# neggles/neurosis

Measured on AMD Instinct MI355X. Metric: train images/sec (node) SDXL 1024^2, higher is better.
Workload: dtype bf16

## Files before the change

include/neurosis_hip.h:

```cpp
#ifndef NEUROSIS_HIP_H
#define NEUROSIS_HIP_H

#ifdef __cplusplus
extern "C" {
#endif

const char* nk_last_error(void);
int nk_abi_version(void);

int nk_linear_fwd(const void* x, const void* w, const float* bias, const void* residual, void* y,
                  int M, int N, int K, long ldx, long ldw, long ldr, long ldy, float alpha, void* stream);
int nk_linear_dgrad(const void* dy, const void* w, const void* dx_add, void* dx, int M, int N, int K,
                    long lddy, long ldw, long ldadd, long lddx, void* stream);
long nk_linear_fwd_geglu_ok(int M, int I, int K);
int nk_linear_fwd_geglu(const void* x, const void* w, const float* bias, void* u, void* h, int M, int I, int K, long ldx, long ldw, long ldu,
                        long ldh, void* stream);
int nk_linear_dgrad_geglu(const void* dy, const void* w, const void* u, void* du, int M, int N, int I, long lddy, long ldw, long ldu,
                          long lddu, void* stream);
int nk_linear_fwd_geglu_s(const void* x, const void* w, const float* bias, void* s, void* h, int M, int I, int K, long ldx, long ldw, long lds,
                          long ldh, void* stream);
int nk_linear_dgrad_geglu_s(const void* dy, const void* w, const void* s, void* du, int M, int N, int I, long lddy, long ldw, long lds,
                            long lddu, void* stream);
int nk_linear_wgrad(const void* dy, const void* x, float* dw, int M, int N, int K, long lddy, long ldx,
                    long lddw, int accumulate, void* stream);
int nk_linear_wgrad_bias(const void* dy, const void* x, float* dw, float* dbias, int M, int N, int K, long lddy, long ldx, long lddw,
                         int accumulate, void* stream);

int nk_gemm_sk_status(void);

int nk_health_status(void);
int nk_health_clear(void);
int nk_health_export(int* dst, void* stream);
int nk_health_import(const int* src, void* stream);
int nk_debug_raise_health(void* stream);
int nk_debug_stamp(unsigned long long* dst, void* stream);
int nk_debug_launch_log(int mode);
long nk_debug_launch_names(char* buf, long cap);

int nk_colsum_batched(const void* dy, float* out, float* ws, long M, int N, long ld, int nbatch, int accumulate, void* stream);

int nk_linear_fwd_batched(const void* const* x, const void* const* w, void* const* y, int count, int M, int N, int K,
                          long ldx, long ldw, long ldy, void* stream);

int nk_linear_wgrad_batched(const void* const* dy, const void* const* x, float* const* dw, float* const* dbias, int count, int M, int N,
                            int K, long lddy, long ldx, long lddw, int accumulate, void* stream);

typedef struct NkConvDesc {
  int N, H, W, Cin;
  int Cout, KH, KW;
  int stride;
  int pad_t, pad_l;
  int Ho, Wo;
  int upsample;
} NkConvDesc;
int nk_conv2d_fwd(const NkConvDesc* d, const void* x, const void* w, const float* bias, const void* rowvec,
                  const void* residual, void* y, void* stream);
long nk_conv2d_stats_tiles(const NkConvDesc* d, int stats_groups);
int nk_conv2d_fwd_stats(const NkConvDesc* d, const void* x, const void* w, const float* bias, const void* rowvec, const void* residual,
                        void* y, float* stats_part, int stats_groups, void* stream);
int nk_conv3x3_few_channels_fwd(const void* x, const void* w, const float* bias, void* y, int N, int H, int W, int Cout, int cin_real,
                                void* stream);
int nk_conv_weight_flip(const void* w, void* wt, int Cout, int Cin, int taps, void* stream);
long nk_conv2d_dgrad_flipped_ok(const NkConvDesc* d);
int nk_conv2d_dgrad_flipped(const NkConvDesc* d, const void* dy, const void* wt, void* dx, void* stream);
int nk_conv2d_dgrad(const NkConvDesc* d, const void* dy, const void* w, void* dx, void* stream);
int nk_conv2d_wgrad(const NkConvDesc* d, const void* dy, const void* x, float* dw, int accumulate, void* stream);
int nk_conv2d_wgrad_bias(const NkConvDesc* d, const void* dy, const void* x, float* dw, float* dbias, int accumulate, void* stream);

typedef struct NkAttnDesc {
  int B, H, Lq, Lk, D;
  long sq, sk, sv, so;
  long bq, bk, bv, bo;
  long sdq, sdk, sdv, sdo;
  long bdq, bdk, bdv, bdo;
  float scale;
  int causal;
} NkAttnDesc;
int nk_attention_fwd(const NkAttnDesc* d, const void* q, const void* k, const void* v, void* o, float* lse,
                     void* stream);
long nk_attention_bwd_ws_floats(const NkAttnDesc* d);
int nk_attention_bwd(const NkAttnDesc* d, const void* q, const void* k, const void* v, const void* o,
                     const float* lse, const void* d_o, void* dq, void* dk, void* dv, float* delta_ws, void* stream);
int nk_attention_bwd_causal(const NkAttnDesc* d, const void* q, const void* k, const void* v, const void* o,
                            const float* lse, const void* d_o, void* dq, void* dk, void* dv, void* stream);
int nk_softmax_rows(void* s, long M, int L, void* stream);

long nk_groupnorm_ws_floats(int N, int HW, int C, int G);
int nk_groupnorm_fwd(const void* x, const float* gamma, const float* beta, void* y, float* mean, float* rstd,
                     float* ws, int N, int HW, int C, int G, float eps, int silu, void* stream);
int nk_groupnorm_sums(const void* x, float* sums, float* ws, int N, int HW, int C, int G, void* stream);
long nk_groupnorm_sums_ws_floats(int N, int nparts, int G);
int nk_groupnorm_sums_from_parts(const float* part, float* sums, float* ws, int N, int nparts, int G, void* stream);
int nk_groupnorm_apply(const void* x, const float* sums, const float* gamma, const float* beta, void* y, float* mean, float* rstd,
                       int N, int HW, int C, int G, float eps, int silu, void* stream);
int nk_groupnorm_bwd(const void* dy, const void* x, const float* gamma, const float* beta, const float* mean,
                     const float* rstd, const void* dx_add, void* dx, float* dgamma, float* dbeta, float* ws,
                     int N, int HW, int C, int G, int silu, int accumulate, void* stream);

int nk_layernorm_fwd(const void* x, const float* gamma, const float* beta, void* y, float* mean, float* rstd,
                     int M, int C, float eps, void* stream);
long nk_layernorm_ws_floats(int M, int C);
int nk_layernorm_bwd(const void* dy, const void* x, const float* gamma, const float* mean, const float* rstd,
                     const void* dx_add, void* dx, float* dgamma, float* dbeta, float* ws, int M, int C, int accumulate, void* stream);
#define NK_COLPART_MAX 32
typedef struct NkColpartBatch {
  const float* part[NK_COLPART_MAX];
  float* dgamma[NK_COLPART_MAX];
  float* dbeta[NK_COLPART_MAX];
  int nrows[NK_COLPART_MAX];
  int C[NK_COLPART_MAX];
  int accumulate[NK_COLPART_MAX];
  int n;
} NkColpartBatch;
long nk_layernorm_part_rows(int M);
int nk_layernorm_bwd_rows(const void* dy, const void* x, const float* gamma, const float* mean, const float* rstd,
                          const void* dx_add, void* dx, float* part, int M, int C, void* stream);
int nk_colpart_reduce_batch(const NkColpartBatch* b, void* stream);
int nk_layernorm_bwd_dx(const void* dy, const void* x, const float* gamma, const float* mean, const float* rstd,
                        const void* dx_add, void* dx, int M, int C, void* stream);
int nk_layernorm_bwd_params(const void* dy, const void* x, const float* mean, const float* rstd, float* dgamma,
                            float* dbeta, float* ws, int M, int C, int accumulate, void* stream);

int nk_geglu_fwd(const void* u, void* y, long M, int I, void* stream);
int nk_geglu_bwd(const void* dy, const void* u, void* du, long M, int I, void* stream);
int nk_geglu_fwd_s(const void* u, void* y, void* s, long M, int I, void* stream);
int nk_geglu_bwd_s(const void* dy, const void* s, void* du, long M, int I, void* stream);

int nk_silu_fwd(const void* x, void* y, long n, void* stream);
int nk_silu_bwd(const void* dy, const void* x, void* dx, long n, void* stream);

int nk_add(const void* a, const void* b, void* out, long n, void* stream);

int nk_cat_channels(const void* a, const void* b, void* out, long rows, int Ca, int Cb, void* stream);
int nk_split_channels(const void* src, void* a, void* b, long rows, int Ca, int Cb, void* stream);

int nk_upsample2x_bwd(const void* dup, void* dx, int N, int H, int W, int C, void* stream);

int nk_nchw_to_nhwc(const void* src, int src_is_f32, void* dst, int N, int C, int HW, int Cpad, float scale,
                    void* stream);
int nk_nhwc_to_nchw(const void* src, void* dst, int dst_is_f32, int N, int C, int HW, int Cpad, void* stream);
int nk_cast_f32_to_bf16(const float* src, void* dst, long n, void* stream);
int nk_cast_bf16_to_f32(const void* src, float* dst, long n, void* stream);

long nk_colsum_ws_floats(long M, int N);
int nk_colsum(const void* dy, float* out, float* ws, long M, int N, long ld, int accumulate, void* stream);

int nk_softmax_rows_bwd(const void* p, void* dp, long M, int L, float scale, void* stream);

int nk_leaky_relu_fwd(const void* x, void* y, long n, float slope, void* stream);
int nk_leaky_relu_bwd(const void* dy, const void* y, void* dx, long n, float slope, void* stream);
long nk_batchnorm_ws_floats(long M, int C);
int nk_batchnorm_fwd(const void* x, const float* gamma, const float* beta, void* y, float* mean, float* rstd, float* running_mean,
                     float* running_var, float* ws, long M, int C, float eps, float momentum, float slope, void* stream);
int nk_batchnorm_bwd(const void* dy, const void* x, const void* y, const float* gamma, const float* mean, const float* rstd, void* dx,
                     float* dgamma, float* dbeta, float* ws, long M, int C, float slope, int accumulate, void* stream);
int nk_batchnorm_eval(const void* x, const float* gamma, const float* beta, const float* running_mean, const float* running_var, void* y,
                      float* ws, long M, int C, float eps, float slope, void* stream);

int nk_maxpool2x2_fwd(const void* x, void* y, int N, int H, int W, int C, void* stream);
int nk_maxpool2x2_bwd(const void* dy, const void* x, void* dx, int N, int H, int W, int C, void* stream);
int nk_maxpool_fwd(const void* x, void* y, int N, int H, int W, int C, int k, int s, void* stream);
int nk_maxpool_bwd(const void* dy, const void* x, void* dx, int N, int H, int W, int C, int k, int s, void* stream);
long nk_lpips_layer_ws_floats(int N, int HW);
int nk_lpips_layer_fwd(const void* f0, const void* f1, const float* w, float* out, float* ws, int N, int HW, int C, float eps,
                       int accumulate, void* stream);
int nk_lpips_layer_bwd(const void* f0, const void* f1, const float* w, const float* upstream, void* df1, int N, int HW, int C,
                       float eps, void* stream);

int nk_gelu_fwd(const void* x, void* y, long n, int mode, void* stream);
int nk_gelu_bwd(const void* dy, const void* x, void* dx, long n, int mode, void* stream);
#define NK_EMBEDDING_BWD_MAX_TOKENS 8192
int nk_embedding_bwd(const long long* ids, const void* dx, long ldx, float* dtable, float* dpos, int B, int L, int V, int P, int C,
                     int accumulate, void* stream);
int nk_gather_rows_bwd(const void* dsel, long ldsel, const long long* idx, void* dx, int B, int L, int C, void* stream);
int nk_wgrad_few_rows(const void* x, long ldx, const void* dy, long lddy, float* dw, long lddw, int M, int K, int N, int accumulate, void* stream);

int nk_timestep_embedding(const float* t, void* out, int B, int dim, float max_period, void* stream);

int nk_edm_prepare(const float* x, const float* eps, const float* sigma, const float* c_in, float* zt, void* net_in,
                   int B, int C, int HW, int Cpad, void* stream);
int nk_edm_loss(const void* net_out, const float* zt, const float* target, const float* c_out, const float* c_skip,
                const float* w, float* loss, void* dnet, int B, int C, int HW, int Cpad, float upstream, void* stream);

int nk_sample_prepare(const float* x, const float* c_in, void* net_in, int B, int C, int HW, int Cpad, int rep, void* stream);
int nk_sample_denoise(const void* net_out, const float* x, const float* c_skip, const float* c_out, float scale,
                      float* denoised, int B, int C, int HW, int Cpad, int rep, void* stream);
int nk_sample_euler_step(const void* net_out, const float* x, const float* c_skip, const float* c_out, const float* sigma_hat,
// ... 56 lines not shown
```

neurosis_amd/csrc/conv_wgrad_halo.h:

```cpp
#pragma once

#define WH_TH 4
#define WH_TW 32
#define WH_HS 48
#define WH_X_BYTES ((WH_TH + 2) * WH_HS * 128)
#define WH_DY_BYTES (WH_TH * WH_TW * 256)
#define WH_STAGE (WH_X_BYTES + WH_DY_BYTES)
#define WH_SMEM (2 * WH_STAGE)
#define WH_BCO 128
#define WH_BCI 64

typedef __attribute__((address_space(3))) char* wh_lds;
typedef __attribute__((address_space(3))) short4_t* wh_lds4;

__device__ __forceinline__ int wh_swz_x(int slot) { return (((slot >> 1) & 1) << 2) | ((slot >> 2) & 3); }
__device__ __forceinline__ int wh_swz_dy(int px) { return ((px & 3) << 2) | ((px >> 2) & 3); }

__device__ __forceinline__ bf16x8_t wh_read(wh_lds lo, wh_lds hi) {
  const short4_t a = __builtin_amdgcn_ds_read_tr16_b64_v4i16((wh_lds4)lo);
  const short4_t b = __builtin_amdgcn_ds_read_tr16_b64_v4i16((wh_lds4)hi);
  short8_t r;
  r[0] = a[0]; r[1] = a[1]; r[2] = a[2]; r[3] = a[3];
  r[4] = b[0]; r[5] = b[1]; r[6] = b[2]; r[7] = b[3];
  return __builtin_bit_cast(bf16x8_t, r);
// ... 99 lines not shown
      if constexpr (BIAS) {
        const short8_t raw = __builtin_bit_cast(short8_t, af);
#pragma unroll
        for (int e = 0; e < 8; ++e) bsum += bf2f((bf16_t)raw[e]);
      }
#pragma unroll
      for (int kh = 0; kh < 3; ++kh)
#pragma unroll
        for (int kw = 0; kw < 3; ++kw) {
          const int off = ((r + kh) * WH_HS + c) * 128;
          const bf16x8_t xf = wh_read(base + xo[kw][0] + off, base + xo[kw][1] + off);
          acc[kh * 3 + kw] = __builtin_amdgcn_mfma_f32_32x32x16_bf16(af, xf, acc[kh * 3 + kw], 0, 0, 0);
        }
    }
  }

  float* dw = (float*)p.C;
  const int ci = ib * WH_BCI + is * 32 + (lane & 31);
  const int co_base = cb * WH_BCO + cs * 32 + 4 * h;
  const bool atomic = gridDim.x > (unsigned)nblk || p.accumulate == 1;
#pragma unroll
  for (int t = 0; t < 9; ++t)
#pragma unroll
    for (int r = 0; r < 16; ++r) {
      const int co = co_base + (r & 3) + 8 * (r >> 2);
      if (co < Cout) {
        float* dst = dw + (long)co * p.ldc + t * Cin + ci;
        const float v = acc[t][r] * p.alpha;
        if (atomic) unsafeAtomicAdd(dst, v);
        else *dst = v;
      }
    }
  if constexpr (BIAS) {
    if (ib == 0 && is == 0) {
      bsum += __shfl_xor(bsum, 32);
      const int co = cb * WH_BCO + cs * 32 + (lane & 31);
      if (lane < 32 && co < Cout) {
        if (atomic) unsafeAtomicAdd(p.dbias + co, bsum * p.alpha);
        else p.dbias[co] = bsum * p.alpha;
      }
    }
  }
}

static bool wgrad_halo_shape_ok(const NkGemmParams& p) {
  const NkGather& g = p.gb;
  if (!p.halo_nb || g.KW != 3 || p.N != 9 * g.C || g.rs != 1 || g.ks != 1 || g.div != 1 || g.off_h != -1 || g.off_w != -1) return false;
  if (g.Ho != g.H || g.Wo != g.W || (g.C % WH_BCI) || (p.M & 7) || p.nbatch || p.ldc != p.N || p.lda != p.M) return false;
  if (p.K != (long)p.halo_nb * g.H * g.W) return false;
  const long cover = (long)((g.W + WH_TW - 1) / WH_TW) * WH_TW * ((g.H + WH_TH - 1) / WH_TH) * WH_TH;
  return cover * 100 <= (long)g.H * g.W * 125;
}
static int wgrad_halo_splits(const NkGemmParams& p, int& per) {
  const NkGather& g = p.gb;
  const long T = (long)p.halo_nb * ((g.W + WH_TW - 1) / WH_TW) * ((g.H + WH_TH - 1) / WH_TH);
  const long nblk = (long)((p.M + WH_BCO - 1) / WH_BCO) * (g.C / WH_BCI);
  const double dw_bytes = (double)p.M * p.N * 4.0;
  double best = 1e30;
  int best_s = 1;
  for (int s = 1; s <= 64 && s <= T; ++s) {
    const long tiles = (T + s - 1) / s;
    const long rounds = (nblk * s + 255) / 256;
    const double cost = (double)rounds * (tiles * 3.0e-6 + 4.0e-6) + (s > 1 ? s * dw_bytes / 1.3e12 : dw_bytes / 4.0e12);
    if (cost < best * 0.97) { best = cost; best_s = s; }
  }
  per = (int)((T + best_s - 1) / best_s);
  return (int)((T + per - 1) / per);
}
static bool use_wgrad_halo(const NkGemmParams& p, int amode, int bmode, int out_f32) {
  if (amode != OP_MC || bmode != OP_MCG || !out_f32) return false;
  int mode = 1;
  if (const char* e = getenv("NK_CONV_WGRAD_HALO")) mode = atoi(e);
  if (!mode || !wgrad_halo_shape_ok(p)) return false;
  if (mode == 2) return true;
  if (p.M < 64) return false;
  const long nblk = (long)((p.M + WH_BCO - 1) / WH_BCO) * (p.gb.C / WH_BCI);
  return p.K >= 16384 || nblk >= 180;
}
static int launch_wgrad_halo(NkGemmParams& p, hipStream_t stream) {
  int per = 0;
  const int S = wgrad_halo_splits(p, per);
  const long nblk = (long)((p.M + WH_BCO - 1) / WH_BCO) * (p.gb.C / WH_BCI);
  if (S > 1 && p.accumulate == 0) {
    const size_t n = (size_t)p.M * p.N;
    const unsigned blocks = (unsigned)((n / 4 + 255) / 256 > 2048 ? 2048 : (n / 4 + 255) / 256);
    hipLaunchKernelGGL(nk_zero_f32_kernel, dim3(blocks ? blocks : 1), dim3(256), 0, stream, (float*)p.C, n);
    if (p.dbias) hipLaunchKernelGGL(nk_zero_f32_kernel, dim3(1), dim3(256), 0, stream, p.dbias, (size_t)p.M);
    if (hipGetLastError() != hipSuccess) return NK_ERR_LAUNCH;
  }
  p.accumulate = p.accumulate == 1 ? 1 : 0;
  p.ksplit_len = per;
  auto kern = p.dbias ? nk_conv3x3_wgrad_halo_kernel<1> : nk_conv3x3_wgrad_halo_kernel<0>;
  nk_optin_lds((const void*)kern, WH_SMEM);
  hipLaunchKernelGGL(kern, dim3((unsigned)(nblk * S)), dim3(512), WH_SMEM, stream, p);
  return nk_check_launch(p.dbias ? "nk_conv3x3_wgrad_halo_kernel<bias=1>" : "nk_conv3x3_wgrad_halo_kernel<bias=0>");
}
```

neurosis_amd/csrc/elementwise.hip:

```cpp
#include "../../include/neurosis_hip.h"
#include "nk_common.h"

#define EW_THREADS 256
static inline int ew_blocks(long work_items) {
  long b = (work_items + EW_THREADS - 1) / EW_THREADS;
  if (b > 8192) b = 8192;
  if (b < 1) b = 1;
  return (int)b;
}

__global__ void geglu_fwd_kernel(const bf16_t* __restrict__ u, bf16_t* __restrict__ y, long M, int I) {
  const int cpr = I >> 3;
  const long total = M * cpr;
  for (long i = blockIdx.x * (long)blockDim.x + threadIdx.x; i < total; i += (long)gridDim.x * blockDim.x) {
    long row = i / cpr;
    int ch = (int)(i - row * cpr);
    float a[8], g[8];
    unpack8(*(const uint4_t*)(u + row * 2 * I + ch * 8), a);
    unpack8(*(const uint4_t*)(u + row * 2 * I + I + ch * 8), g);
#pragma unroll
    for (int e = 0; e < 8; ++e) a[e] *= gelu_erf(g[e]);
    *(uint4_t*)(y + row * I + ch * 8) = pack8(a);
  }
}
// ... 335 lines not shown
  }
}
extern "C" int nk_upsample2x_bwd(const void* dup, void* dx, int N, int H, int W, int C, void* stream) {
  NK_CHECK_ARG(dup && dx && N > 0 && H > 0 && W > 0 && C > 0 && (C & 7) == 0);
  hipLaunchKernelGGL(up2_bwd_kernel, dim3(ew_blocks((long)N * H * W * (C >> 3))), dim3(EW_THREADS), 0,
                     (hipStream_t)stream, (const bf16_t*)dup, (bf16_t*)dx, N, H, W, C);
  return nk_check_launch("upsample2x_bwd");
}

template <typename SrcT>
__global__ void nchw_to_nhwc_kernel(const SrcT* __restrict__ src, bf16_t* __restrict__ dst, int C, int HW, int Cpad,
                                    float scale) {
  __shared__ float tile[32][33];
  const int n = blockIdx.z;
  const int p0 = blockIdx.x * 32, c0 = blockIdx.y * 32;
  const int tx = threadIdx.x & 31, ty = threadIdx.x >> 5;
  for (int j = ty; j < 32; j += 8) {
    int c = c0 + j, p = p0 + tx;
    float v = 0.f;
    if (c < C && p < HW) {
      if constexpr (sizeof(SrcT) == 4) v = src[((long)n * C + c) * HW + p];
      else v = bf2f(src[((long)n * C + c) * HW + p]);
    }
    tile[j][tx] = v * scale;
  }
  __syncthreads();
  for (int j = ty; j < 32; j += 8) {
    int p = p0 + j, c = c0 + tx;
    if (p < HW && c < Cpad) dst[((long)n * HW + p) * Cpad + c] = f2bf(tile[tx][j]);
  }
}
template <typename DstT>
__global__ void nhwc_to_nchw_kernel(const bf16_t* __restrict__ src, DstT* __restrict__ dst, int C, int HW, int Cpad) {
  __shared__ float tile[32][33];
  const int n = blockIdx.z;
  const int p0 = blockIdx.x * 32, c0 = blockIdx.y * 32;
  const int tx = threadIdx.x & 31, ty = threadIdx.x >> 5;
  for (int j = ty; j < 32; j += 8) {
    int p = p0 + j, c = c0 + tx;
    tile[j][tx] = (p < HW && c < C) ? bf2f(src[((long)n * HW + p) * Cpad + c]) : 0.f;
  }
  __syncthreads();
  for (int j = ty; j < 32; j += 8) {
    int c = c0 + j, p = p0 + tx;
    if (c < C && p < HW) {
      float v = tile[tx][j];
      if constexpr (sizeof(DstT) == 4) dst[((long)n * C + c) * HW + p] = v;
      else dst[((long)n * C + c) * HW + p] = f2bf(v);
    }
  }
}
__global__ __launch_bounds__(256) void conv_weight_flip_kernel(const bf16_t* __restrict__ w, bf16_t* __restrict__ wt, int Cout, int Cin, int taps) {
  __shared__ bf16_t tile[64][64 + 8];
  const int tap = blockIdx.z, co0 = blockIdx.y * 64, ci0 = blockIdx.x * 64;
  const int tid = threadIdx.x;
#pragma unroll
  for (int it = 0; it < 2; ++it) {
    const int idx = tid + 256 * it;
    const int r = idx >> 3, ch = idx & 7;
    uint4_t v = {0u, 0u, 0u, 0u};
    if (co0 + r < Cout && ci0 + ch * 8 < Cin) v = *(const uint4_t*)(w + ((long)(co0 + r) * taps + tap) * Cin + ci0 + ch * 8);
    const bf16_t* e = (const bf16_t*)&v;
#pragma unroll
    for (int k = 0; k < 8; ++k) tile[ch * 8 + k][r] = e[k];
  }
  __syncthreads();
  const int tflip = taps - 1 - tap;
#pragma unroll
  for (int it = 0; it < 2; ++it) {
    const int idx = tid + 256 * it;
    const int r = idx >> 3, ch = idx & 7;
    if (ci0 + r < Cin && co0 + ch * 8 < Cout)
      *(uint4_t*)(wt + ((long)(ci0 + r) * taps + tflip) * Cout + co0 + ch * 8) = *(const uint4_t*)&tile[r][ch * 8];
  }
}
extern "C" int nk_conv_weight_flip(const void* w, void* wt, int Cout, int Cin, int taps, void* stream) {
  NK_CHECK_ARG(w && wt && Cout > 0 && Cin > 0 && taps > 0 && taps <= 65535);
  NK_CHECK_ARG((Cout & 7) == 0 && (Cin & 7) == 0);
  hipLaunchKernelGGL(conv_weight_flip_kernel, dim3((Cin + 63) / 64, (Cout + 63) / 64, taps), dim3(256), 0, (hipStream_t)stream, (const bf16_t*)w, (bf16_t*)wt,
                     Cout, Cin, taps);
  return nk_check_launch("conv_weight_flip_kernel");
}

__global__ __launch_bounds__(256) void conv3x3_few_channels_kernel(const bf16_t* __restrict__ x, const bf16_t* __restrict__ w, const float* __restrict__ bias,
                                                                   bf16_t* __restrict__ y, int N, int H, int W, int Cout, int groups_per_wave) {
  const int lane = threadIdx.x & 63, wave = threadIdx.x >> 6;
  const int r = lane & 15, g = lane >> 4;
  const int co_base = blockIdx.y * 128;
  bf16x8_t wf[8][2];
#pragma unroll
  for (int b = 0; b < 8; ++b) {
    const int co = co_base + b * 16 + r;
    uint2_t t0 = {0u, 0u}, t1 = {0u, 0u}, t8 = {0u, 0u};
    if (co < Cout) {
      t0 = *(const uint2_t*)(w + ((long)co * 9 + 2 * g) * 8);
      t1 = *(const uint2_t*)(w + ((long)co * 9 + 2 * g + 1) * 8);
      if (g == 0) t8 = *(const uint2_t*)(w + ((long)co * 9 + 8) * 8);
    }
    wf[b][0] = __builtin_bit_cast(bf16x8_t, (uint4_t){t0.x, t0.y, t1.x, t1.y});
    wf[b][1] = __builtin_bit_cast(bf16x8_t, (uint4_t){t8.x, t8.y, 0u, 0u});
  }
  const int nloc = (g & 1) * 16 + (g >> 1) * 8;
  float bv[4][8];
#pragma unroll
  for (int h = 0; h < 4; ++h)
#pragma unroll
    for (int e = 0; e < 8; ++e) {
      const int co = co_base + h * 32 + nloc + e;
      bv[h][e] = (bias && co < Cout) ? bias[co] : 0.f;
    }
  const long total = (long)N * H * W;
  const long gw = (long)blockIdx.x * 4 + wave;
  const int HW = H * W;
  const int ta = 2 * g, tb = 2 * g + 1;
  const int dya = ta / 3 - 1, dxa = ta % 3 - 1, dyb = tb / 3 - 1, dxb = tb % 3 - 1;

  auto fetch = [&](long grp, uint2_t& a, uint2_t& b, uint2_t& c) {
    a = (uint2_t){0u, 0u}; b = a; c = a;
    const long pix = grp * 16 + r;
    if (pix >= total) return;
    const int n = (int)(pix / HW);
    const int rem = (int)(pix - (long)n * HW);
    const int py = rem / W, px = rem - py * W;
    const bf16_t* img = x + (long)n * HW * 8;
    int yy = py + dya, xx = px + dxa;
    if ((unsigned)yy < (unsigned)H && (unsigned)xx < (unsigned)W) a = *(const uint2_t*)(img + ((long)yy * W + xx) * 8);
    yy = py + dyb; xx = px + dxb;
    if ((unsigned)yy < (unsigned)H && (unsigned)xx < (unsigned)W) b = *(const uint2_t*)(img + ((long)yy * W + xx) * 8);
    if (g == 0) {
      yy = py + 1; xx = px + 1;
      if (yy < H && xx < W) c = *(const uint2_t*)(img + ((long)yy * W + xx) * 8);
    }
  };

  const long gstride = (long)gridDim.x * 4;
  uint2_t na, nb, nc;
  long grp = gw;
  fetch(grp, na, nb, nc);
  for (int it = 0; it < groups_per_wave; ++it, grp += gstride) {
    if (grp * 16 >= total) break;
    const bf16x8_t x0 = __builtin_bit_cast(bf16x8_t, (uint4_t){na.x, na.y, nb.x, nb.y});
    const bf16x8_t x1 = __builtin_bit_cast(bf16x8_t, (uint4_t){nc.x, nc.y, 0u, 0u});
    if (it + 1 < groups_per_wave) fetch(grp + gstride, na, nb, nc);
    float4_t acc[8];
#pragma unroll
    for (int b = 0; b < 8; ++b) {
      acc[b] = __builtin_amdgcn_mfma_f32_16x16x32_bf16(wf[b][0], x0, (float4_t){0.f, 0.f, 0.f, 0.f}, 0, 0, 0);
      acc[b] = __builtin_amdgcn_mfma_f32_16x16x32_bf16(wf[b][1], x1, acc[b], 0, 0, 0);
    }
    const long pix = grp * 16 + r;
#pragma unroll
    for (int h = 0; h < 4; ++h) {
      float v[8];
#pragma unroll
      for (int e = 0; e < 4; ++e) {
        const float a_own = acc[2 * h][e], b_own = acc[2 * h + 1][e];
        auto sw = __builtin_amdgcn_permlane16_swap(__float_as_uint(a_own), __float_as_uint(b_own), false, false);
        v[e] = __uint_as_float(sw[0]) + bv[h][e];
        v[4 + e] = __uint_as_float(sw[1]) + bv[h][4 + e];
      }
      const int co = co_base + h * 32 + nloc;
      if (pix < total && co < Cout) *(uint4_t*)(y + pix * Cout + co) = pack8(v);
    }
  }
}
extern "C" int nk_conv3x3_few_channels_fwd(const void* x, const void* w, const float* bias, void* y, int N, int H, int W, int Cout, int cin_real,
                                           void* stream) {
  NK_CHECK_ARG(x && w && y && N > 0 && H > 0 && W > 0 && Cout > 0 && (Cout & 7) == 0);
  NK_CHECK_ARG(cin_real == 3 || cin_real == 4);
  NK_CHECK_ARG((long)N * H * W < (1l << 31));
  const long groups = ((long)N * H * W + 15) / 16;
  long blocks = (groups + 4 * 32 - 1) / (4 * 32);
  if (blocks > 2048) blocks = 2048;
  const int per_wave = (int)((groups + blocks * 4 - 1) / (blocks * 4));
  dim3 grid((unsigned)blocks, (unsigned)((Cout + 127) / 128));
  hipLaunchKernelGGL(conv3x3_few_channels_kernel, grid, dim3(256), 0, (hipStream_t)stream, (const bf16_t*)x, (const bf16_t*)w, bias, (bf16_t*)y, N, H, W, Cout,
                     per_wave);
  return nk_check_launch("conv3x3_few_channels_kernel");
}

extern "C" int nk_nchw_to_nhwc(const void* src, int src_is_f32, void* dst, int N, int C, int HW, int Cpad, float scale,
                               void* stream) {
  NK_CHECK_ARG(src && dst && N > 0 && C > 0 && HW > 0 && Cpad >= C);
  dim3 grid((HW + 31) / 32, (Cpad + 31) / 32, N);
  if (src_is_f32)
    hipLaunchKernelGGL(nchw_to_nhwc_kernel<float>, grid, dim3(256), 0, (hipStream_t)stream, (const float*)src,
                       (bf16_t*)dst, C, HW, Cpad, scale);
  else
    hipLaunchKernelGGL(nchw_to_nhwc_kernel<bf16_t>, grid, dim3(256), 0, (hipStream_t)stream, (const bf16_t*)src,
                       (bf16_t*)dst, C, HW, Cpad, scale);
  return nk_check_launch("nchw_to_nhwc");
}
extern "C" int nk_nhwc_to_nchw(const void* src, void* dst, int dst_is_f32, int N, int C, int HW, int Cpad,
                               void* stream) {
  NK_CHECK_ARG(src && dst && N > 0 && C > 0 && HW > 0 && Cpad >= C);
  dim3 grid((HW + 31) / 32, (C + 31) / 32, N);
  if (dst_is_f32)
    hipLaunchKernelGGL(nhwc_to_nchw_kernel<float>, grid, dim3(256), 0, (hipStream_t)stream, (const bf16_t*)src,
                       (float*)dst, C, HW, Cpad);
  else
    hipLaunchKernelGGL(nhwc_to_nchw_kernel<bf16_t>, grid, dim3(256), 0, (hipStream_t)stream, (const bf16_t*)src,
                       (bf16_t*)dst, C, HW, Cpad);
  return nk_check_launch("nhwc_to_nchw");
}

__global__ void cast_f32_bf16_kernel(const float* __restrict__ s, bf16_t* __restrict__ d, long n) {
  const long n8 = n >> 3;
  for (long i = blockIdx.x * (long)blockDim.x + threadIdx.x; i < n8; i += (long)gridDim.x * blockDim.x) {
    const float4_t a = *(const float4_t*)(s + i * 8), b = *(const float4_t*)(s + i * 8 + 4);
    float f[8] = {a[0], a[1], a[2], a[3], b[0], b[1], b[2], b[3]};
    *(uint4_t*)(d + i * 8) = pack8(f);
  }
  if (blockIdx.x == 0) for (long i = n8 * 8 + threadIdx.x; i < n; i += blockDim.x) d[i] = f2bf(s[i]);
}
__global__ void cast_bf16_f32_kernel(const bf16_t* __restrict__ s, float* __restrict__ d, long n) {
  for (long i = blockIdx.x * (long)blockDim.x + threadIdx.x; i < n; i += (long)gridDim.x * blockDim.x) d[i] = bf2f(s[i]);
}
extern "C" int nk_cast_f32_to_bf16(const float* src, void* dst, long n, void* stream) {
  NK_CHECK_ARG(src && dst && n > 0 && ((uintptr_t)src & 15) == 0 && ((uintptr_t)dst & 15) == 0);
  hipLaunchKernelGGL(cast_f32_bf16_kernel, dim3(ew_blocks((n >> 3) + 1)), dim3(EW_THREADS), 0, (hipStream_t)stream, src,
                     (bf16_t*)dst, n);
  return nk_check_launch("cast_f32_to_bf16");
}
extern "C" int nk_cast_bf16_to_f32(const void* src, float* dst, long n, void* stream) {
  NK_CHECK_ARG(src && dst && n > 0);
  hipLaunchKernelGGL(cast_bf16_f32_kernel, dim3(ew_blocks(n)), dim3(EW_THREADS), 0, (hipStream_t)stream,
                     (const bf16_t*)src, dst, n);
  return nk_check_launch("cast_bf16_to_f32");
}

#define CS_ROWS 64
static int colsum_rows(long M) {
  long rows = CS_ROWS;
  while ((M + rows - 1) / rows > 1024) rows *= 2;
  return (int)rows;
}
__global__ __launch_bounds__(256) void colsum_partial_kernel(const bf16_t* __restrict__ dy, float* __restrict__ part, long M, int N,
                                                             long ld, int rows_per_block) {
  __shared__ float ps[16][16 * 8 + 4];
  const int tid = threadIdx.x;
  const int cx = tid & 15, ry = tid >> 4;
  const int chunk = blockIdx.y * 16 + cx;
  const bool cok = chunk < (N >> 3);
  dy += (long)blockIdx.z * M * ld;
  part += (long)blockIdx.z * gridDim.x * N;
  const long row_lo = (long)blockIdx.x * rows_per_block;
  const long row_hi = row_lo + rows_per_block < M ? row_lo + rows_per_block : M;
  float s[8];
#pragma unroll
  for (int e = 0; e < 8; ++e) s[e] = 0.f;
  if (cok) {
    for (long base = row_lo + ry; base < row_hi; base += 64) {
      uint4_t v[4];
#pragma unroll
      for (int i = 0; i < 4; ++i) {
        const long r = base + 16 * i;
        v[i] = r < row_hi ? *(const uint4_t*)(dy + r * ld + chunk * 8) : (uint4_t){0u, 0u, 0u, 0u};
      }
#pragma unroll
      for (int i = 0; i < 4; ++i) {
        float f[8];
// ... 325 lines not shown
```

neurosis_amd/csrc/gemm.hip:

```cpp
#include "nk_common.h"
#include "nk_gemm.h"
#include <stdlib.h>

#define BM 128
#define BN 128
#define BK 64
#define NTHREADS 256
#define GROUP_M 8
#define KC_IMAGE_BYTES (128 * 128)
#define MC_ROW_BYTES (128 * 2 + 16)
#define MC_IMAGE_BYTES (BK * MC_ROW_BYTES)
#define OPND_BYTES MC_IMAGE_BYTES
#define STAGE_BYTES (2 * OPND_BYTES)
#define CS_LD 132
#define SMEM_BYTES (2 * STAGE_BYTES)

static_assert(SMEM_BYTES >= BM * CS_LD * 4, "epilogue staging must fit");

enum { OP_KC = 0, OP_KCG = 1, OP_MC = 2, OP_MCT = 3, OP_MCG = 4 };

__device__ __forceinline__ bool is_kc(int mode) { return mode == OP_KC || mode == OP_KCG; }

__device__ __forceinline__ long gather_offset(const NkGather& g, int n, int bh, int bw, int kh, int kw,
                                              int c, bool& valid) {
// ... 1315 lines not shown
    X2_RDA(1);
    X2_BAR();
    X2_MM(4, 2, bc1, X2_NEXT(b0, sb0, p.gb, nb0, kb0); X2_NEXT(b1, sb1, p.gb, nb1, kb1));
    X2_BAR();
    b0.fire(0, sb0[0], cur + 32768);
    b0.fire(1, sb0[1], cur + 32768);
    b1.fire(0, sb1[0], cur + 49152);
    b1.fire(1, sb1[1], cur + 49152);
    asm volatile("s_waitcnt vmcnt(4)" ::: "memory");
    X2_BAR();
    X2_MM(4, 0, bc0, X2_NEXT(a1, sa1, p.ga, na1, ka1));
    X2_BAR();
  }
  if (wm == 0) { X2_BAR(); }
  asm volatile("s_waitcnt vmcnt(0)" ::: "memory");
#undef X2_NEXT
#undef X2_ISSUE
#undef X2_RD1
#undef X2_RDA
#undef X2_RDB
#undef X2_BAR
#undef X2_MM
  if constexpr (GEGLU) {
    const int I = p.N >> 1;
    const int abase = (n0 >> 1) + wn * 32;
    const int cl = (lane >> 4) * 4;
    float4_t ba[2], bg[2];
#pragma unroll
    for (int q = 0; q < 2; ++q) {
      ba[q] = p.bias ? *(const float4_t*)(p.bias + abase + q * 16 + cl) : (float4_t){0.f, 0.f, 0.f, 0.f};
      bg[q] = p.bias ? *(const float4_t*)(p.bias + I + abase + q * 16 + cl) : (float4_t){0.f, 0.f, 0.f, 0.f};
    }
    NkGemmParams ph = p;
    ph.N = I; ph.ldc = p.ld_h; ph.bias = nullptr;
    NkGemmParams ps = p;
    ps.bias = nullptr;
#pragma unroll
    for (int ib = 0; ib < 2; ++ib) {
      float4_t pa[4][2], pg[4][2], phh[4][2];
#pragma unroll
      for (int i = 0; i < 4; ++i)
#pragma unroll
        for (int q = 0; q < 2; ++q) {
          pa[i][q] = acc[ib * 4 + i][2 * q];
          pg[i][q] = acc[ib * 4 + i][2 * q + 1];
#pragma unroll
          for (int r = 0; r < 4; ++r) {
            const float av = bf2f(f2bf(pa[i][q][r] + ba[q][r])), gv = bf2f(f2bf(pg[i][q][r] + bg[q][r]));
            float cdf, pdf;
            normal_cdf_pdf(gv, cdf, pdf);
            const float ge = gv * cdf;
            phh[i][q][r] = av * ge;
            if (p.geglu_save) {
              pa[i][q][r] = ge;
              pg[i][q][r] = av * (cdf + gv * pdf);
            }
          }
        }
      const int mb = m0 + wm * 128 + ib * 64;
      if (p.geglu_save) {
        reg_epilogue_64x32<0>(ps, p.C, pa, mb, abase, lane);
        reg_epilogue_64x32<0>(ps, p.C, pg, mb, I + abase, lane);
      } else {
        reg_epilogue_64x32<0>(p, p.C, pa, mb, abase, lane);
        reg_epilogue_64x32<0>(p, p.C, pg, mb, I + abase, lane);
      }
      reg_epilogue_64x32<0>(ph, p.geglu_h, phh, mb, abase, lane);
    }
    return;
  }
#pragma unroll
  for (int ib = 0; ib < 2; ++ib)
#pragma unroll
    for (int half = 0; half < 2; ++half) {
      float4_t pair[4][2];
#pragma unroll
      for (int i = 0; i < 4; ++i) { pair[i][0] = acc[ib * 4 + i][2 * half]; pair[i][1] = acc[ib * 4 + i][2 * half + 1]; }
      reg_epilogue_64x32<0>(p, p.C, pair, m0 + wm * 128 + ib * 64, n0 + wn * 64 + half * 32, lane);
    }
}

static bool use_xl(const NkGemmParams& p, int amode, int bmode, int out_f32, int splitk);
__global__ void nk_zero_f32_kernel(float* __restrict__ dst, size_t n);
#include "gemm_g2.h"
#include "gemm_w160.h"
#include "conv_halo.h"
#include "conv_wgrad_halo.h"

static bool use_xl(const NkGemmParams& p, int amode, int bmode, int out_f32, int splitk) {
  static int on = -1;
  if (on < 0) { const char* e = getenv("NK_GEMM_XL"); on = (e && e[0] == '0') ? 0 : 1; }
  if (!on || p.nbatch || out_f32 || splitk != 1 || bmode != OP_KC || !(amode == OP_KC || amode == OP_KCG)) return false;
  const long ntn = (p.N + XL_BN - 1) / XL_BN;
  const long tiles = (long)((p.M + XL_BM - 1) / XL_BM) * ntn;
  const long rounds = (tiles + 255) / 256;
  return tiles >= 224 && tiles * 10 >= rounds * 256 * 8 && ntn * XL_BN * 100 <= (long)p.N * 112 && p.K >= 4 * BK;
}
template <int AMODE, int WM, int WN>
static int launch_xl_as(const NkGemmParams& p, hipStream_t stream) {
  auto kern = nk_gemm_xl_kernel<AMODE, WM, WN>;
  nk_optin_lds((const void*)kern, XL_SMEM_BYTES);
  dim3 grid(((p.M + XL_BM - 1) / XL_BM) * ((p.N + XL_BN - 1) / XL_BN), 1, 1);
  hipLaunchKernelGGL(kern, grid, dim3((XL_BM / WM) * (XL_BN / WN) * 64), XL_SMEM_BYTES, stream, p);
  return nk_check_launch("nk_gemm_xl_kernel");
}
template <int AMODE>
static int launch_xl(const NkGemmParams& p_in, hipStream_t stream) {
  if (AMODE == OP_KC) {
    auto kern = nk_gemm_xl2g_kernel<OP_KC, 0>;
    auto kerng = nk_gemm_xl2g_kernel<OP_KC, 1>;
    nk_optin_lds((const void*)kern, XL_SMEM_BYTES);
    nk_optin_lds((const void*)kerng, XL_SMEM_BYTES);
    NkGemmParams p = p_in;
    p.k_rotate = k_rotate_on(p.K) ? 1 : 0;
    dim3 grid(((p.M + XL_BM - 1) / XL_BM) * ((p.N + XL_BN - 1) / XL_BN), 1, 1);
    if (p.geglu_h) hipLaunchKernelGGL(kerng, grid, dim3(512), XL_SMEM_BYTES, stream, p);
    else hipLaunchKernelGGL(kern, grid, dim3(512), XL_SMEM_BYTES, stream, p);
    return nk_check_launch(p.geglu_h ? "nk_gemm_xl2g_kernel<geglu=1>" : "nk_gemm_xl2g_kernel<geglu=0>");
  }
  return launch_xl_as<AMODE, 64, 64>(p_in, stream);
}

template <int AMODE, int BMODE, int OUT_F32>
static int launch(const NkGemmParams& p_in, int splitk, hipStream_t stream) {
  NkGemmParams p2 = p_in;
  const NkGemmParams& p = p2;
  auto kern8 = nk_gemm_dma_kernel<AMODE, BMODE, OUT_F32, 8>;
  auto kernr = nk_gemm_ring_kernel<AMODE, BMODE, OUT_F32>;
  nk_optin_lds((const void*)kern8, V2_SMEM_BYTES);
  nk_optin_lds((const void*)kernr, RING_SMEM_BYTES);
  int ntm = (p.M + BM - 1) / BM, ntn = (p.N + BN - 1) / BN;
  dim3 grid(ntm * ntn, splitk, p.nbatch ? p.nbatch : 1);
  {
    int per_xcd = (ntm * ntn + 7) / 8, g = 1;
    while ((g + 1) * (g + 1) <= per_xcd) ++g;
    p2.group_m = g > GROUP_M ? GROUP_M : g;
  }
  p2.k_rotate = k_rotate_on(splitk > 1 ? p.ksplit_len : p.K) ? 1 : 0;
  if (!p.nbatch && (long)ntm * ntn * splitk <= 256) {
    hipLaunchKernelGGL(kernr, grid, dim3(512), RING_SMEM_BYTES, stream, p);
    return nk_check_launch("nk_gemm_ring_kernel");
  }
  hipLaunchKernelGGL(kern8, grid, dim3(512), V2_SMEM_BYTES, stream, p);
  return nk_check_launch("nk_gemm_dma_kernel");
}


#include <mutex>
#include <unordered_map>
struct SkWorkspace {
  unsigned* counter = nullptr;
  unsigned* flags = nullptr;
  float* ws = nullptr;
};
static std::mutex sk_mutex;
static std::unordered_map<void*, SkWorkspace> sk_spaces;

static bool use_sk(const NkGemmParams& p, int out_f32) {
  int mode = 4;
  if (const char* e = getenv("NK_GEMM_SK")) mode = atoi(e);
  if (mode == 0) return false;
  if (mode == 1) return true;
  if (mode == 2) return out_f32 != 0;
  if (mode == 4 && out_f32) return false;
  const long tiles = (long)((p.M + BM - 1) / BM) * ((p.N + BN - 1) / BN) * (p.nbatch ? p.nbatch : 1);
  const long nk = (p.K + BK - 1) / BK;
// ... 13 lines not shown
      nk_set_error(__FILE__, __LINE__, "stream-K workspace requested while the stream is capturing: run the launch once on this stream before capturing it");
      return NK_ERR_LAUNCH;
    }
    char* raw = nullptr;
    const size_t ws_bytes = (size_t)SK_MAX_GRID * SK_TILE_FLOATS * sizeof(float);
    if (hipMalloc((void**)&raw, ws_bytes + (SK_MAX_GRID + 64) * sizeof(unsigned)) != hipSuccess) {
      nk_set_error(__FILE__, __LINE__, "hipMalloc of the stream-K workspace failed");
      return NK_ERR_LAUNCH;
    }
    w.ws = (float*)raw;
    w.flags = (unsigned*)(raw + ws_bytes);
    w.counter = w.flags + SK_MAX_GRID;
    if (hipMemsetAsync(w.flags, 0, (SK_MAX_GRID + 64) * sizeof(unsigned), stream) != hipSuccess) return NK_ERR_LAUNCH;
  }
  p.sk_health = nk_health_word();
  if (!p.sk_health) { nk_set_error(__FILE__, __LINE__, "health word allocation failed"); return NK_ERR_LAUNCH; }
  p.sk_counter = w.counter;
  p.sk_flags = w.flags;
  p.sk_ws = w.ws;
  p.sk_base = 0;
  p.sk_epoch = 0;
  return NK_OK;
}

int nk_gemm_sk_reset(void) {
  std::lock_guard<std::mutex> lock(sk_mutex);
  for (auto& kv : sk_spaces)
    if (kv.second.flags && hipMemset(kv.second.flags, 0, (SK_MAX_GRID + 64) * sizeof(unsigned)) != hipSuccess) return NK_ERR_LAUNCH;
  return NK_OK;
}

extern "C" int nk_gemm_sk_status(void) {
  std::lock_guard<std::mutex> lock(sk_mutex);
  if (hipDeviceSynchronize() != hipSuccess) return -1;
  int bad = 0;
  for (auto& kv : sk_spaces) {
    unsigned v = 0;
    if (kv.second.flags && hipMemcpy(&v, kv.second.flags + SK_MAX_GRID + 1, sizeof(v), hipMemcpyDeviceToHost) == hipSuccess && v) bad = 1;
  }
  return bad;
}

template <int AMODE, int BMODE, int OUT_F32>
static int launch_sk(NkGemmParams& p, hipStream_t stream) {
  auto kern = nk_gemm_sk_kernel<AMODE, BMODE, OUT_F32>;
  nk_optin_lds((const void*)kern, SK_SMEM_BYTES);
  const long ntm = (p.M + BM - 1) / BM, ntn = (p.N + BN - 1) / BN, nk = (p.K + BK - 1) / BK;
  const long T = ntm * ntn * (p.nbatch ? p.nbatch : 1), W = T * nk;
  const int max_grid = SK_MAX_GRID & ~7, min_iters = 4;
  long grid = (W / min_iters) & ~7l;
  if (grid > max_grid) grid = max_grid;
  if (grid < 8) grid = 8;
  p.sk_chunked = T >= 64;
  { const char* d = getenv("NK_SK_DEBUG"); p.sk_debug = d ? atoi(d) & 2 : 0; }
  if (int e = sk_prepare(p, (int)grid, stream)) return e;
  hipLaunchKernelGGL(kern, dim3((unsigned)grid), dim3(SK_NT), SK_SMEM_BYTES, stream, p);
  return nk_check_launch("nk_gemm_sk_kernel");
}

__global__ __launch_bounds__(256) void nk_zero_f32_kernel(float* __restrict__ dst, size_t n) {
  const size_t n4 = n / 4, stride = (size_t)gridDim.x * 256;
  float4_t* d4 = (float4_t*)dst;
  for (size_t i = (size_t)blockIdx.x * 256 + threadIdx.x; i < n4; i += stride) d4[i] = (float4_t){0.f, 0.f, 0.f, 0.f};
  if (blockIdx.x == 0 && threadIdx.x < (n & 3)) dst[n4 * 4 + threadIdx.x] = 0.f;
}

static int pick_splitk(int M, int N, int K, int max_split) {
  int tiles = ((M + BM - 1) / BM) * ((N + BN - 1) / BN);
  int nk = (K + BK - 1) / BK;
  const int lo = 96, hi = 192;
  if (tiles >= lo && tiles * 2 <= 512 && nk >= 256 && max_split >= 2) return 2;
  if (tiles >= lo) return 1;
  int s = 1;
  while (s < max_split && tiles * s < hi && nk / (s * 2) >= 8) s *= 2;
  return s;
}

static void set_split(NkGemmParams& p, int splitk) {
  int nk = (p.K + BK - 1) / BK;
  int per = (nk + splitk - 1) / splitk;
  p.ksplit_len = per * BK;
}

static int zero_split_outputs(const NkGemmParams& p, hipStream_t stream) {
  for (int z = 0; z < (p.nbatch ? p.nbatch : 1); ++z) {
    const size_t n = (size_t)p.M * p.N;
    float* dst = (float*)(p.nbatch ? p.Cb[z] : p.C);
    const unsigned blocks = (unsigned)((n / 4 + 255) / 256 > 2048 ? 2048 : (n / 4 + 255) / 256);
    hipLaunchKernelGGL(nk_zero_f32_kernel, dim3(blocks ? blocks : 1), dim3(256), 0, stream, dst, n);
    float* db = p.nbatch ? p.dbias_b[z] : p.dbias;
    if (db) hipLaunchKernelGGL(nk_zero_f32_kernel, dim3(1), dim3(256), 0, stream, db, (size_t)p.M);
  }
  return hipGetLastError() != hipSuccess ? NK_ERR_LAUNCH : NK_OK;
}

int nk_gemm_dispatch(NkGemmParams& p, int amode, int bmode, int out_f32, int allow_splitk,
                     hipStream_t stream) {
  NK_CHECK_ARG(p.M > 0 && p.N > 0 && p.K > 0);
  if (!p.nbatch) NK_CHECK_ARG(((uintptr_t)p.A & 15) == 0 && ((uintptr_t)p.B & 15) == 0 && ((uintptr_t)p.C & 15) == 0);
  for (int z = 0; z < p.nbatch; ++z) NK_CHECK_ARG(((uintptr_t)p.Ab[z] & 15) == 0 && ((uintptr_t)p.Bb[z] & 15) == 0 && ((uintptr_t)p.Cb[z] & 15) == 0);
  if (amode == OP_KC) NK_CHECK_ARG((p.K & 7) == 0 && (p.lda & 7) == 0);
  if (bmode == OP_KC) NK_CHECK_ARG((p.K & 7) == 0 && (p.ldb & 7) == 0);
  if (amode == OP_KCG) NK_CHECK_ARG((p.ga.C & 7) == 0);
  if (amode == OP_MC) NK_CHECK_ARG((p.M & 7) == 0 && (p.lda & 7) == 0);
  if (bmode == OP_MC) NK_CHECK_ARG((p.N & 7) == 0 && (p.ldb & 7) == 0);
  if (bmode == OP_MCT) NK_CHECK_ARG((p.N & 7) == 0 && (p.tw.co_stride & 7) == 0 && (p.tw.tap_stride & 7) == 0);
  if (bmode == OP_MCG) NK_CHECK_ARG((p.gb.C & 7) == 0);
  if (p.residual) NK_CHECK_ARG(((uintptr_t)p.residual & 15) == 0 && ((p.ldr & 7) == 0 || (p.N & 7) != 0));
  if (!out_f32) NK_CHECK_ARG((p.ldc & 7) == 0 || (p.N & 7) != 0);
  if (p.fRowsPerBatch.d == 0) p.fRowsPerBatch = make_fastdiv(1);

  if (p.dbias || (p.nbatch && p.dbias_b[0])) NK_CHECK_ARG(amode == OP_MC && out_f32);
  if (p.geglu_h) {
    NK_CHECK_ARG(amode == OP_KC && bmode == OP_KC && !out_f32 && !p.nbatch && (p.N & 255) == 0 && (p.ld_h & 7) == 0 && !p.rowvec && !p.residual && p.alpha == 1.0f);
    NK_CHECK_ARG(((uintptr_t)p.geglu_h & 15) == 0 && (!p.bias || ((uintptr_t)p.bias & 15) == 0));
    if (!use_xl(p, amode, bmode, out_f32, 1)) {
      nk_set_error(__FILE__, __LINE__, "fused GEGLU forward on a shape the 256 x 256 kernel does not take (ask nk_linear_fwd_geglu_ok first)");
      return NK_ERR_ARG;
    }
    set_split(p, 1);
    return launch_xl<OP_KC>(p, stream);
  }
  if (p.geglu_u) {
    NK_CHECK_ARG(amode == OP_KC && bmode == OP_MC && !out_f32 && !p.nbatch && (p.N & 7) == 0 && (p.ld_u & 7) == 0 && !p.bias && !p.rowvec && !p.residual);
    set_split(p, 1);
    return launch<OP_KC, OP_MC, 0>(p, 1, stream);
  }
  if (use_halo(p, amode, bmode, out_f32)) return launch_halo(p, stream);
  if (use_wgrad_halo(p, amode, bmode, out_f32)) return launch_wgrad_halo(p, stream);
  if (p.stats_part) {
    nk_set_error(__FILE__, __LINE__, "statistics epilogue on a convolution the halo-tile kernel does not take (ask nk_conv2d_stats_tiles first)");
    return NK_ERR_ARG;
  }

  {
    const W160Plan wp = w160_plan(p, amode, bmode, out_f32, allow_splitk);
    if (wp.bn) {
      set_split(p, wp.splitk);
      if (wp.splitk > 1 && p.accumulate == 0) {
        NK_CHECK_ARG(p.ldc == p.N);
        if (int rc = zero_split_outputs(p, stream)) return rc;
        p.accumulate = 1;
      } else if (p.accumulate == 2) {
        p.accumulate = wp.splitk > 1 ? 1 : 0;
      }
      p.k_rotate = k_rotate_on(wp.splitk > 1 ? p.ksplit_len : p.K) ? 1 : 0;
      return wp.bn == 160 ? launch_w160_as<160>(p, wp.splitk, stream) : launch_w160_as<128>(p, wp.splitk, stream);
    }
  }
  if (use_ring64(p, amode, bmode, out_f32)) return launch_ring64(p, stream);
  if ((!p.nbatch || p.nbatch <= NK_MAX_BATCH) && use_g2(p, amode, bmode, out_f32, 1) && (g2_mode() == 2 || !use_xl(p, amode, bmode, out_f32, 1))) {
    if (p.accumulate == 2) p.accumulate = 0;
    if (amode == OP_KC && bmode == OP_KC) return out_f32 ? launch_g2<OP_KC, OP_KC, 1>(p, stream) : launch_g2<OP_KC, OP_KC, 0>(p, stream);
    if (amode == OP_KC && bmode == OP_MC) return out_f32 ? launch_g2<OP_KC, OP_MC, 1>(p, stream) : launch_g2<OP_KC, OP_MC, 0>(p, stream);
    if (amode == OP_KCG && bmode == OP_KC) return out_f32 ? launch_g2<OP_KCG, OP_KC, 1>(p, stream) : launch_g2<OP_KCG, OP_KC, 0>(p, stream);
    if (amode == OP_KCG && bmode == OP_MCT) return out_f32 ? launch_g2<OP_KCG, OP_MCT, 1>(p, stream) : launch_g2<OP_KCG, OP_MCT, 0>(p, stream);
    return out_f32 ? launch_g2<OP_MC, OP_MC, 1>(p, stream) : launch_g2<OP_MC, OP_MC, 0>(p, stream);
  }

  bool has_dbias = p.dbias != nullptr;
  for (int z = 0; z < p.nbatch && z < NK_MAX_BATCH; ++z) has_dbias = has_dbias || p.dbias_b[z] != nullptr;
  if (!has_dbias && use_sk(p, out_f32)) {
    const long ntm_ = (p.M + BM - 1) / BM, ntn_ = (p.N + BN - 1) / BN, nk_ = (p.K + BK - 1) / BK;
    if (ntm_ * ntn_ * (p.nbatch ? p.nbatch : 1) * nk_ < (1l << 22)) {
      if (p.accumulate == 2) p.accumulate = 0;
#define NK_SK_CASE(A_, B_)                                                        \
      if (amode == A_ && bmode == B_) return out_f32 ? launch_sk<A_, B_, 1>(p, stream) : launch_sk<A_, B_, 0>(p, stream);
      NK_SK_CASE(OP_KC, OP_KC)
      NK_SK_CASE(OP_KC, OP_MC)
      NK_SK_CASE(OP_MC, OP_MC)
      NK_SK_CASE(OP_KCG, OP_KC)
// ... 46 lines not shown
```

neurosis_amd/csrc/nk_common.h:

```cpp
#pragma once
#include <hip/hip_runtime.h>
#include <stdint.h>

typedef unsigned short bf16_t;
typedef __attribute__((ext_vector_type(8))) short short8_t;
typedef __attribute__((ext_vector_type(4))) short short4_t;
typedef __attribute__((ext_vector_type(8))) __bf16 bf16x8_t;
typedef __attribute__((ext_vector_type(4))) float float4_t;
typedef __attribute__((ext_vector_type(16))) float float16_t;
typedef __attribute__((ext_vector_type(4))) unsigned int uint4_t;
typedef __attribute__((ext_vector_type(2))) unsigned int uint2_t;

#define NK_OK 0
#define NK_ERR_ARG 1
#define NK_ERR_LAUNCH 2
#define NK_ERR_HEALTH 3

#define NK_CHECK_ARG(cond)                                                        \
  do {                                                                            \
    if (!(cond)) {                                                                \
      nk_set_error(__FILE__, __LINE__, #cond);                                    \
      return NK_ERR_ARG;                                                          \
    }                                                                             \
  } while (0)

void nk_set_error(const char* file, int line, const char* what);
int nk_check_launch(const char* what);
void nk_optin_lds(const void* kernel, int bytes);
unsigned* nk_health_word(void);
int nk_health_poll(void);
void nk_health_snapshot(hipStream_t stream);

__device__ __forceinline__ float bf2f(bf16_t v) { return __uint_as_float(((unsigned)v) << 16); }
__device__ __forceinline__ bf16_t f2bf(float f) {
  __bf16 b = (__bf16)f;
  return __builtin_bit_cast(unsigned short, b);
}
typedef __attribute__((ext_vector_type(2))) float float2_t;
typedef __attribute__((ext_vector_type(2))) __bf16 bf16x2_t;
__device__ __forceinline__ unsigned pack2bf(float lo, float hi) {
  float2_t v = {lo, hi};
  return __builtin_bit_cast(unsigned, __builtin_convertvector(v, bf16x2_t));
}
__device__ __forceinline__ void unpack8(const uint4_t& v, float* f) {
  f[0] = __uint_as_float(v.x << 16); f[1] = __uint_as_float(v.x & 0xffff0000u);
  f[2] = __uint_as_float(v.y << 16); f[3] = __uint_as_float(v.y & 0xffff0000u);
  f[4] = __uint_as_float(v.z << 16); f[5] = __uint_as_float(v.z & 0xffff0000u);
  f[6] = __uint_as_float(v.w << 16); f[7] = __uint_as_float(v.w & 0xffff0000u);
}
__device__ __forceinline__ uint4_t pack8(const float* f) {
  uint4_t v;
  v.x = pack2bf(f[0], f[1]); v.y = pack2bf(f[2], f[3]);
  v.z = pack2bf(f[4], f[5]); v.w = pack2bf(f[6], f[7]);
  return v;
}
__device__ __forceinline__ void unpack4(const uint2_t& v, float* f) {
  f[0] = __uint_as_float(v.x << 16); f[1] = __uint_as_float(v.x & 0xffff0000u);
  f[2] = __uint_as_float(v.y << 16); f[3] = __uint_as_float(v.y & 0xffff0000u);
}

__device__ __forceinline__ float wave_sum(float v) {
#pragma unroll
  for (int o = 32; o > 0; o >>= 1) v += __shfl_xor(v, o, 64);
  return v;
}
__device__ __forceinline__ float wave_max(float v) {
#pragma unroll
  for (int o = 32; o > 0; o >>= 1) v = fmaxf(v, __shfl_xor(v, o, 64));
  return v;
}

struct FastDiv {
  unsigned d, m, s;
};
static inline FastDiv make_fastdiv(unsigned d) {
  FastDiv f;
  f.d = d;
  if (d <= 1) { f.m = 0; f.s = 0; return f; }
  unsigned l = 0;
  while ((1ull << l) < d) ++l;
  f.m = (unsigned)(((1ull << 32) * ((1ull << l) - d)) / d + 1);
  f.s = l;
  return f;
}
__device__ __forceinline__ unsigned fdiv(unsigned n, const FastDiv& f) {
  return (__umulhi(n, f.m) + n) >> f.s;
}

__device__ __forceinline__ float silu_f(float x) { return x / (1.0f + __expf(-x)); }
__device__ __forceinline__ float dsilu_f(float x) {
  float s = 1.0f / (1.0f + __expf(-x));
  return s * (1.0f + x * (1.0f - s));
}

__device__ __forceinline__ void normal_cdf_pdf(float x, float& cdf, float& pdf) {
  const float e = __expf(-0.5f * x * x);
  const float t = __builtin_amdgcn_rcpf(1.0f + 0.3275911f * 0.70710678118654752f * fabsf(x));
  const float poly = t * (0.254829592f + t * (-0.284496736f + t * (1.421413741f + t * (-1.453152027f + t * 1.061405429f))));
  cdf = 0.5f * (1.0f + copysignf(1.0f - poly * e, x));
  pdf = 0.3989422804014327f * e;
}
__device__ __forceinline__ float gelu_erf(float x) {
  float cdf, pdf;
  normal_cdf_pdf(x, cdf, pdf);
  return x * cdf;
}
__device__ __forceinline__ float dgelu_erf(float x) {
  float cdf, pdf;
  normal_cdf_pdf(x, cdf, pdf);
  return cdf + x * pdf;
}
// ... 1 lines not shown
```

neurosis_amd/csrc/norm.hip:

```cpp
#include "../../include/neurosis_hip.h"
#include "nk_common.h"

#define GN_THREADS 256
#define GN_MAXC 4096

__global__ __launch_bounds__(GN_THREADS) void gn_stats_kernel(const bf16_t* __restrict__ x, float* __restrict__ stats,
                                                              int HW, int C, int G, int rows_per) {
  __shared__ float ps[GN_THREADS * 8], pss[GN_THREADS * 8];
  const int n = blockIdx.y;
  const int cpr = (C >> 3) / gridDim.z;
  const int ch0 = blockIdx.z * cpr;
  const int rows_par = GN_THREADS / cpr;
  const int tid = threadIdx.x;
  const int cpg = C / G;
  const int row_lo = blockIdx.x * rows_per;
  const int row_hi = min(HW, row_lo + rows_per);
  float s[8], ss[8];
#pragma unroll
  for (int e = 0; e < 8; ++e) { s[e] = 0.f; ss[e] = 0.f; }
  const int chunk = tid % cpr, rsub = tid / cpr;
  if (rsub < rows_par) {
    const bf16_t* base = x + ((long)n * HW) * C + (ch0 + chunk) * 8;
    int r = row_lo + rsub;
    for (; r + 3 * rows_par < row_hi; r += 4 * rows_par) {
      uint4_t v[4];
#pragma unroll
      for (int u = 0; u < 4; ++u) v[u] = *(const uint4_t*)(base + (long)(r + u * rows_par) * C);
#pragma unroll
      for (int u = 0; u < 4; ++u) {
        float f[8];
        unpack8(v[u], f);
#pragma unroll
        for (int e = 0; e < 8; ++e) { s[e] += f[e]; ss[e] += f[e] * f[e]; }
      }
    }
    for (; r < row_hi; r += rows_par) {
      float f[8];
      unpack8(*(const uint4_t*)(base + (long)r * C), f);
#pragma unroll
      for (int e = 0; e < 8; ++e) { s[e] += f[e]; ss[e] += f[e] * f[e]; }
    }
#pragma unroll
    for (int e = 0; e < 8; ++e) {
      ps[(rsub * cpr + chunk) * 8 + e] = s[e];
      pss[(rsub * cpr + chunk) * 8 + e] = ss[e];
    }
  }
  __syncthreads();
  float* part = stats + (((long)n * gridDim.x + blockIdx.x) * gridDim.z + blockIdx.z) * 2 * G;
  for (int i = tid; i < 2 * G; i += GN_THREADS) {
    const int g = i >> 1;
    const float* src = (i & 1) ? pss : ps;
    const int c_lo = max(g * cpg, ch0 * 8), c_hi = min((g + 1) * cpg, (ch0 + cpr) * 8);
    float a = 0.f;
    for (int c = c_lo; c < c_hi; ++c)
      for (int r = 0; r < rows_par; ++r) a += src[r * cpr * 8 + (c - ch0 * 8)];
    part[i] = a;
  }
}

__global__ __launch_bounds__(1024) void gn_reduce_partials_kernel(const float* __restrict__ part, float* __restrict__ out,
                                                                 int nparts, int G2) {
  __shared__ float sm[8][128];
  const int n = blockIdx.x;
  const int tx = threadIdx.x & 127, ty = threadIdx.x >> 7;
  float a = 0.f;
  if (tx < G2)
    for (int p = ty; p < nparts; p += 8) a += part[((long)n * nparts + p) * G2 + tx];
  sm[ty][tx] = a;
  __syncthreads();
  if (ty == 0 && tx < G2) {
#pragma unroll
    for (int j = 1; j < 8; ++j) a += sm[j][tx];
    out[(long)n * G2 + tx] = a;
  }
}

__global__ __launch_bounds__(GN_THREADS) void gn_apply_kernel(const bf16_t* __restrict__ x, const float* __restrict__ stats,
                                                              const float* __restrict__ gamma, const float* __restrict__ beta,
                                                              bf16_t* __restrict__ y, float* __restrict__ mean_out,
                                                              float* __restrict__ rstd_out, int HW, int C, int G,
                                                              float eps, int silu, int rows_per) {
  extern __shared__ __attribute__((aligned(16))) char smem_raw[];
  float* sc = (float*)smem_raw;
  float* sh = sc + C;
  const int n = blockIdx.y;
  const int tid = threadIdx.x;
  const int cpg = C / G;
  const float inv_cnt = 1.0f / ((float)HW * (float)cpg);
  for (int c = tid; c < C; c += GN_THREADS) {
    int g = c / cpg;
    float m = stats[(long)n * 2 * G + 2 * g] * inv_cnt;
    float var = fmaxf(stats[(long)n * 2 * G + 2 * g + 1] * inv_cnt - m * m, 0.f);
    float rs = rsqrtf(var + eps);
    float a = rs * gamma[c];
    sc[c] = a;
    sh[c] = beta[c] - m * a;
    if (blockIdx.x == 0 && (c % cpg) == 0) { mean_out[n * G + g] = m; rstd_out[n * G + g] = rs; }
  }
  __syncthreads();
  const int cpr = C >> 3;
  const int row_lo = blockIdx.x * rows_per;
  const int row_hi = min(HW, row_lo + rows_per);
  const unsigned total = (unsigned)(row_hi - row_lo) * (unsigned)cpr;
  const bf16_t* xb = x + ((long)n * HW + row_lo) * C;
  bf16_t* yb = y + ((long)n * HW + row_lo) * C;
  auto one = [&](unsigned i, const uint4_t& raw) {
    const unsigned chunk = i % (unsigned)cpr;
    float f[8];
    unpack8(raw, f);
    const float4_t a0 = *(const float4_t*)(sc + chunk * 8), a1 = *(const float4_t*)(sc + chunk * 8 + 4);
    const float4_t b0 = *(const float4_t*)(sh + chunk * 8), b1 = *(const float4_t*)(sh + chunk * 8 + 4);
    f[0] = f[0] * a0[0] + b0[0]; f[1] = f[1] * a0[1] + b0[1]; f[2] = f[2] * a0[2] + b0[2]; f[3] = f[3] * a0[3] + b0[3];
    f[4] = f[4] * a1[0] + b1[0]; f[5] = f[5] * a1[1] + b1[1]; f[6] = f[6] * a1[2] + b1[2]; f[7] = f[7] * a1[3] + b1[3];
    if (silu) {
#pragma unroll
      for (int e = 0; e < 8; ++e) f[e] = silu_f(f[e]);
    }
    *(uint4_t*)(yb + (size_t)i * 8) = pack8(f);
  };
  unsigned i = tid;
  for (; i + 3 * GN_THREADS < total; i += 4 * GN_THREADS) {
    uint4_t v[4];
#pragma unroll
    for (int u = 0; u < 4; ++u) v[u] = *(const uint4_t*)(xb + (size_t)(i + u * GN_THREADS) * 8);
#pragma unroll
    for (int u = 0; u < 4; ++u) one(i + u * GN_THREADS, v[u]);
  }
  for (; i < total; i += GN_THREADS) one(i, *(const uint4_t*)(xb + (size_t)i * 8));
}

__global__ __launch_bounds__(GN_THREADS, 4) void gn_bwd_stats_kernel(const bf16_t* __restrict__ dy, const bf16_t* __restrict__ x,
                                                                  const float* __restrict__ gamma, const float* __restrict__ beta,
                                                                  const float* __restrict__ mean, const float* __restrict__ rstd,
                                                                  float* __restrict__ gsum, float* __restrict__ chan_part,
                                                                  int HW, int C, int G, int silu, int rows_per) {
  __shared__ float pa[GN_THREADS * 8], pb[GN_THREADS * 8];
  extern __shared__ __attribute__((aligned(16))) char smem_raw[];
  float* ca = (float*)smem_raw;
  float* cb = ca + C;
  const int n = blockIdx.y;
  const int tid = threadIdx.x;
  const int cpg = C / G;
  const int cpr = (C >> 3) / gridDim.z;
  const int ch0 = blockIdx.z * cpr;
  const int rows_par = GN_THREADS / cpr;
  const int row_lo = blockIdx.x * rows_per;
  const int row_hi = min(HW, row_lo + rows_per);
  const int chunk = tid % cpr, rsub = tid / cpr;
  if (rsub < rows_par) {
    float a[8], b[8], mu[8], rs[8], ga[8], be[8];
#pragma unroll
    for (int e = 0; e < 8; ++e) {
      int c = (ch0 + chunk) * 8 + e;
      int g = c / cpg;
      a[e] = 0.f; b[e] = 0.f;
      mu[e] = mean[n * G + g]; rs[e] = rstd[n * G + g];
      ga[e] = gamma[c]; be[e] = beta[c];
    }
    const long base = ((long)n * HW) * C + (ch0 + chunk) * 8;
    auto one = [&](const uint4_t& rx, const uint4_t& rd) {
      float fx[8], fd[8];
      unpack8(rx, fx);
      unpack8(rd, fd);
#pragma unroll
      for (int e = 0; e < 8; ++e) {
        float xh = (fx[e] - mu[e]) * rs[e];
        float dz = fd[e];
        if (silu) dz *= dsilu_f(xh * ga[e] + be[e]);
        a[e] += dz;
        b[e] += dz * xh;
      }
    };
    int r = row_lo + rsub;
    for (; r + 3 * rows_par < row_hi; r += 4 * rows_par) {
      uint4_t vx[4], vd[4];
#pragma unroll
      for (int u = 0; u < 4; ++u) {
        vx[u] = *(const uint4_t*)(x + base + (long)(r + u * rows_par) * C);
        vd[u] = *(const uint4_t*)(dy + base + (long)(r + u * rows_par) * C);
      }
#pragma unroll
      for (int u = 0; u < 4; ++u) one(vx[u], vd[u]);
    }
    for (; r < row_hi; r += rows_par) one(*(const uint4_t*)(x + base + (long)r * C), *(const uint4_t*)(dy + base + (long)r * C));
#pragma unroll
    for (int e = 0; e < 8; ++e) {
      pa[(rsub * cpr + chunk) * 8 + e] = a[e];
      pb[(rsub * cpr + chunk) * 8 + e] = b[e];
    }
  }
  __syncthreads();
  float* cp = chan_part + ((long)n * gridDim.x + blockIdx.x) * 2 * C;
  for (int cl = tid; cl < cpr * 8; cl += GN_THREADS) {
    float av = 0.f, bv = 0.f;
    for (int r = 0; r < rows_par; ++r) { av += pa[r * cpr * 8 + cl]; bv += pb[r * cpr * 8 + cl]; }
    const int c = ch0 * 8 + cl;
    ca[cl] = av;
    cb[cl] = bv;
    cp[c] = bv;
    cp[C + c] = av;
  }
  __syncthreads();
  float* part = gsum + (((long)n * gridDim.x + blockIdx.x) * gridDim.z + blockIdx.z) * 2 * G;
  for (int i = tid; i < 2 * G; i += GN_THREADS) {
    const int g = i >> 1;
    const float* src = (i & 1) ? cb : ca;
    const int c_lo = max(g * cpg, ch0 * 8), c_hi = min((g + 1) * cpg, (ch0 + cpr) * 8);
    float acc = 0.f;
    for (int c = c_lo; c < c_hi; ++c) acc += gamma[c] * src[c - ch0 * 8];
    part[i] = acc;
  }
}

__global__ __launch_bounds__(1024) void colpart_reduce_kernel(const float* __restrict__ part, float* __restrict__ dgamma,
                                                              float* __restrict__ dbeta, int nrows, int C, int accumulate) {
  __shared__ float sa[16][64], sb[16][64];
  const int tx = threadIdx.x & 63, ty = threadIdx.x >> 6;
  const int c = blockIdx.x * 64 + tx;
  float a = 0.f, b = 0.f;
  if (c < C) {
#pragma unroll 4
    for (int r = ty; r < nrows; r += 16) {
      a += part[(long)r * 2 * C + c];
      b += part[(long)r * 2 * C + C + c];
    }
  }
  sa[ty][tx] = a;
  sb[ty][tx] = b;
  __syncthreads();
  if (ty == 0 && c < C) {
#pragma unroll
    for (int j = 1; j < 16; ++j) { a += sa[j][tx]; b += sb[j][tx]; }
    dgamma[c] = accumulate ? dgamma[c] + a : a;
    dbeta[c] = accumulate ? dbeta[c] + b : b;
  }
}

__global__ __launch_bounds__(GN_THREADS) void gn_bwd_apply_kernel(const bf16_t* __restrict__ dy, const bf16_t* __restrict__ x,
                                                                  const float* __restrict__ gamma, const float* __restrict__ beta,
                                                                  const float* __restrict__ mean, const float* __restrict__ rstd,
                                                                  const float* __restrict__ gsum, const bf16_t* __restrict__ dx_add,
                                                                  bf16_t* __restrict__ dx, int HW, int C, int G, int silu,
                                                                  int rows_per) {
  extern __shared__ __attribute__((aligned(16))) char smem_raw[];
  float* p_a = (float*)smem_raw;
  float* p_b = p_a + C;
  float* p_c = p_b + C;
  float* p_d = p_c + C;
  const int n = blockIdx.y;
  const int tid = threadIdx.x;
  const int cpg = C / G;
  const float inv_cnt = 1.0f / ((float)HW * (float)cpg);
  for (int c = tid; c < C; c += GN_THREADS) {
    const int g = c / cpg;
    const float mu = mean[n * G + g], rs = rstd[n * G + g];
    const float s1 = gsum[(long)n * 2 * G + 2 * g] * inv_cnt, s2 = gsum[(long)n * 2 * G + 2 * g + 1] * inv_cnt;
    const float a = rs * gamma[c];
    p_a[c] = a;
    p_b[c] = beta[c] - mu * a;
    p_c[c] = -rs * rs * s2;
    p_d[c] = -rs * s1 + mu * rs * rs * s2;
  }
  __syncthreads();
  const int cpr = C >> 3;
  const int row_lo = blockIdx.x * rows_per;
  const int row_hi = min(HW, row_lo + rows_per);
  const unsigned total = (unsigned)(row_hi - row_lo) * (unsigned)cpr;
  const long off0 = ((long)n * HW + row_lo) * C;
  auto one = [&](unsigned i, const uint4_t& rx, const uint4_t& rd, const uint4_t& ra) {
    const int c0 = (int)(i % (unsigned)cpr) * 8;
    float fx[8], fd[8], fa[8], ca[8], cb[8], cc[8], cd[8];
    unpack8(rx, fx);
    unpack8(rd, fd);
    unpack8(ra, fa);
    *(float4_t*)ca = *(const float4_t*)(p_a + c0); *(float4_t*)(ca + 4) = *(const float4_t*)(p_a + c0 + 4);
    *(float4_t*)cc = *(const float4_t*)(p_c + c0); *(float4_t*)(cc + 4) = *(const float4_t*)(p_c + c0 + 4);
    *(float4_t*)cd = *(const float4_t*)(p_d + c0); *(float4_t*)(cd + 4) = *(const float4_t*)(p_d + c0 + 4);
    if (silu) {
      *(float4_t*)cb = *(const float4_t*)(p_b + c0); *(float4_t*)(cb + 4) = *(const float4_t*)(p_b + c0 + 4);
#pragma unroll
      for (int e = 0; e < 8; ++e) fd[e] *= dsilu_f(fx[e] * ca[e] + cb[e]);
    }
#pragma unroll
    for (int e = 0; e < 8; ++e) fx[e] = ca[e] * fd[e] + (fx[e] * cc[e] + cd[e]) + fa[e];
    *(uint4_t*)(dx + off0 + (size_t)i * 8) = pack8(fx);
  };
  const uint4_t zero4 = {0u, 0u, 0u, 0u};
  unsigned i = tid;
  for (; i + GN_THREADS < total; i += 2 * GN_THREADS) {
    uint4_t vx[2], vd[2], va[2];
#pragma unroll
    for (int u = 0; u < 2; ++u) {
      const size_t o = off0 + (size_t)(i + u * GN_THREADS) * 8;
      vx[u] = *(const uint4_t*)(x + o);
      vd[u] = *(const uint4_t*)(dy + o);
      va[u] = dx_add ? *(const uint4_t*)(dx_add + o) : zero4;
    }
#pragma unroll
    for (int u = 0; u < 2; ++u) one(i + u * GN_THREADS, vx[u], vd[u], va[u]);
  }
  for (; i < total; i += GN_THREADS) {
    const size_t o = off0 + (size_t)i * 8;
    one(i, *(const uint4_t*)(x + o), *(const uint4_t*)(dy + o), dx_add ? *(const uint4_t*)(dx_add + o) : zero4);
  }
}

static int gn_nz(int C) {
  int cpr = C >> 3, nz = (cpr + GN_THREADS - 1) / GN_THREADS;
  while (cpr % nz) ++nz;
  return nz;
}

static int gn_rows_per(int N, int HW, int* nsplit) {
  int want = (1024 + N - 1) / N;
  int rows_per = (HW + want - 1) / want;
  if (rows_per < 32) rows_per = 32;
  *nsplit = (HW + rows_per - 1) / rows_per;
  return rows_per;
}

extern "C" long nk_groupnorm_ws_floats(int N, int HW, int C, int G) {
  int nsplit;
  gn_rows_per(N, HW, &nsplit);
  long parts = (long)N * nsplit * gn_nz(C) * 2 * G;
  long chan = (long)N * nsplit * 2 * C;
  return parts + chan + (long)N * 2 * G + 64;
}

extern "C" int nk_groupnorm_fwd(const void* x, const float* gamma, const float* beta, void* y, float* mean,
                                float* rstd, float* ws, int N, int HW, int C, int G, float eps, int silu,
                                void* stream_) {
  hipStream_t stream = (hipStream_t)stream_;
  NK_CHECK_ARG(N > 0 && HW > 0 && C > 0 && G > 0 && G <= 64);
  NK_CHECK_ARG((C & 7) == 0 && C % G == 0 && C <= GN_MAXC);
  NK_CHECK_ARG(x && gamma && beta && y && mean && rstd && ws);
  int nsplit;
  int rows_per = gn_rows_per(N, HW, &nsplit);
  const int nz = gn_nz(C);
  float* part = ws;
  float* stats = ws + (long)N * nsplit * nz * 2 * G;
  hipLaunchKernelGGL(gn_stats_kernel, dim3(nsplit, N, nz), dim3(GN_THREADS), 0, stream, (const bf16_t*)x, part, HW, C,
                     G, rows_per);
  if (int e = nk_check_launch("gn_stats_kernel")) return e;
  hipLaunchKernelGGL(gn_reduce_partials_kernel, dim3(N), dim3(1024), 0, stream, part, stats, nsplit * nz, 2 * G);
  if (int e = nk_check_launch("gn_reduce_partials_kernel")) return e;
  hipLaunchKernelGGL(gn_apply_kernel, dim3(nsplit, N), dim3(GN_THREADS), 2 * C * sizeof(float), stream,
                     (const bf16_t*)x, stats, gamma, beta, (bf16_t*)y, mean, rstd, HW, C, G, eps, silu, rows_per);
  return nk_check_launch("gn_apply_kernel");
}

__global__ __launch_bounds__(256) void gn_reduce_partials_l1_kernel(const float* __restrict__ part, float* __restrict__ out, int nparts, int G2, int nchunks) {
  __shared__ float sm[4][64];
  const int n = blockIdx.y, chunk = blockIdx.x;
  const int tx = threadIdx.x & 63, ty = threadIdx.x >> 6;
  float a = 0.f;
  if (tx < G2)
    for (int p = chunk + ty * nchunks; p < nparts; p += 4 * nchunks) a += part[((long)n * nparts + p) * G2 + tx];
  sm[ty][tx] = a;
  __syncthreads();
  if (ty == 0 && tx < G2) out[((long)n * nchunks + chunk) * G2 + tx] = (a + sm[1][tx]) + (sm[2][tx] + sm[3][tx]);
}

extern "C" long nk_groupnorm_sums_ws_floats(int N, int nparts, int G) {
  (void)nparts;
  return (long)N * 64 * 2 * G + 64;
}
extern "C" int nk_groupnorm_sums_from_parts(const float* part, float* sums, float* ws, int N, int nparts, int G, void* stream_) {
  hipStream_t stream = (hipStream_t)stream_;
  NK_CHECK_ARG(part && sums && N > 0 && nparts > 0 && G > 0 && G <= 32);
  if (nparts > 128) {
    NK_CHECK_ARG(ws != nullptr);
    const int nchunks = 64;
    hipLaunchKernelGGL(gn_reduce_partials_l1_kernel, dim3(nchunks, N), dim3(256), 0, stream, part, ws, nparts, 2 * G, nchunks);
    if (int e = nk_check_launch("gn_reduce_partials_l1_kernel")) return e;
    part = ws;
    nparts = nchunks;
  }
  hipLaunchKernelGGL(gn_reduce_partials_kernel, dim3(N), dim3(1024), 0, stream, part, sums, nparts, 2 * G);
  return nk_check_launch("gn_reduce_partials_kernel");
}

extern "C" int nk_groupnorm_sums(const void* x, float* sums, float* ws, int N, int HW, int C, int G, void* stream_) {
  hipStream_t stream = (hipStream_t)stream_;
  NK_CHECK_ARG(N > 0 && HW > 0 && C > 0 && G > 0 && G <= 64);
  NK_CHECK_ARG((C & 7) == 0 && C % G == 0 && C <= GN_MAXC);
  NK_CHECK_ARG(x && sums && ws);
  int nsplit;
  int rows_per = gn_rows_per(N, HW, &nsplit);
  const int nz = gn_nz(C);
  hipLaunchKernelGGL(gn_stats_kernel, dim3(nsplit, N, nz), dim3(GN_THREADS), 0, stream, (const bf16_t*)x, ws, HW, C, G, rows_per);
  if (int e = nk_check_launch("gn_stats_kernel")) return e;
  hipLaunchKernelGGL(gn_reduce_partials_kernel, dim3(N), dim3(1024), 0, stream, ws, sums, nsplit * nz, 2 * G);
  return nk_check_launch("gn_reduce_partials_kernel");
}

extern "C" int nk_groupnorm_apply(const void* x, const float* sums, const float* gamma, const float* beta, void* y, float* mean,
                                  float* rstd, int N, int HW, int C, int G, float eps, int silu, void* stream_) {
  hipStream_t stream = (hipStream_t)stream_;
  NK_CHECK_ARG(N > 0 && HW > 0 && C > 0 && G > 0 && G <= 64);
  NK_CHECK_ARG((C & 7) == 0 && C % G == 0 && C <= GN_MAXC);
  NK_CHECK_ARG(x && sums && gamma && beta && y && mean && rstd);
  int nsplit;
  int rows_per = gn_rows_per(N, HW, &nsplit);
  hipLaunchKernelGGL(gn_apply_kernel, dim3(nsplit, N), dim3(GN_THREADS), 2 * C * sizeof(float), stream, (const bf16_t*)x, sums, gamma, beta,
                     (bf16_t*)y, mean, rstd, HW, C, G, eps, silu, rows_per);
  return nk_check_launch("gn_apply_kernel");
}

extern "C" int nk_groupnorm_bwd(const void* dy, const void* x, const float* gamma, const float* beta,
                                const float* mean, const float* rstd, const void* dx_add, void* dx, float* dgamma,
                                float* dbeta, float* ws, int N, int HW, int C, int G, int silu, int accumulate, void* stream_) {
  hipStream_t stream = (hipStream_t)stream_;
  NK_CHECK_ARG(N > 0 && HW > 0 && C > 0 && G > 0 && G <= 64);
  NK_CHECK_ARG((C & 7) == 0 && C % G == 0 && C <= GN_MAXC);
  NK_CHECK_ARG(dy && x && gamma && beta && mean && rstd && dx && dgamma && dbeta && ws);
  int nsplit;
  int rows_per = gn_rows_per(N, HW, &nsplit);
  const int nz = gn_nz(C);
  float* part = ws;
  float* gsum = part + (long)N * nsplit * nz * 2 * G;
  float* chan = gsum + (long)N * 2 * G;
  hipLaunchKernelGGL(gn_bwd_stats_kernel, dim3(nsplit, N, nz), dim3(GN_THREADS), 2 * C * sizeof(float), stream,
                     (const bf16_t*)dy, (const bf16_t*)x, gamma, beta, mean, rstd, part, chan, HW, C, G, silu, rows_per);
  if (int e = nk_check_launch("gn_bwd_stats_kernel")) return e;
  hipLaunchKernelGGL(gn_reduce_partials_kernel, dim3(N), dim3(1024), 0, stream, part, gsum, nsplit * nz, 2 * G);
  if (int e = nk_check_launch("gn_reduce_partials_kernel")) return e;
  hipLaunchKernelGGL(colpart_reduce_kernel, dim3((C + 63) / 64), dim3(1024), 0, stream, chan, dgamma, dbeta, N * nsplit, C, accumulate);
  if (int e = nk_check_launch("colpart_reduce_kernel")) return e;
  hipLaunchKernelGGL(gn_bwd_apply_kernel, dim3(nsplit, N), dim3(GN_THREADS), 4 * C * sizeof(float), stream,
                     (const bf16_t*)dy, (const bf16_t*)x, gamma, beta, mean, rstd, gsum, (const bf16_t*)dx_add,
                     (bf16_t*)dx, HW, C, G, silu, rows_per);
  return nk_check_launch("gn_bwd_apply_kernel");
}

#define LN_MAXCH 4

template <int NCH>
__global__ __launch_bounds__(256) void ln_fwd_kernel(const bf16_t* __restrict__ x, const float* __restrict__ gamma,
                                                     const float* __restrict__ beta, bf16_t* __restrict__ y,
                                                     float* __restrict__ mean, float* __restrict__ rstd, int M, int C,
                                                     float eps) {
  const int lane = threadIdx.x & 63;
  const int wave = (blockIdx.x * blockDim.x + threadIdx.x) >> 6;
  const int nwaves = (gridDim.x * blockDim.x) >> 6;
  const int cpr = C >> 3;
  const float invC = 1.0f / (float)C;
  for (int row = wave; row < M; row += nwaves) {
    float f[NCH][8];
    float s = 0.f;
#pragma unroll
    for (int j = 0; j < NCH; ++j) {
      int ch = lane + 64 * j;
      if (ch < cpr) {
        unpack8(*(const uint4_t*)(x + (long)row * C + ch * 8), f[j]);
#pragma unroll
        for (int e = 0; e < 8; ++e) s += f[j][e];
      }
    }
    const float mu = wave_sum(s) * invC;
    float v = 0.f;
#pragma unroll
    for (int j = 0; j < NCH; ++j) {
      int ch = lane + 64 * j;
      if (ch < cpr) {
#pragma unroll
        for (int e = 0; e < 8; ++e) { float d = f[j][e] - mu; v += d * d; }
      }
    }
    const float rs = rsqrtf(wave_sum(v) * invC + eps);
    if (lane == 0) { mean[row] = mu; rstd[row] = rs; }
#pragma unroll
    for (int j = 0; j < NCH; ++j) {
      int ch = lane + 64 * j;
      if (ch < cpr) {
        const float4_t g0 = *(const float4_t*)(gamma + ch * 8), g1 = *(const float4_t*)(gamma + ch * 8 + 4);
        const float4_t b0 = *(const float4_t*)(beta + ch * 8), b1 = *(const float4_t*)(beta + ch * 8 + 4);
        float o[8];
#pragma unroll
        for (int e = 0; e < 4; ++e) {
          o[e] = (f[j][e] - mu) * rs * g0[e] + b0[e];
          o[4 + e] = (f[j][4 + e] - mu) * rs * g1[e] + b1[e];
        }
        *(uint4_t*)(y + (long)row * C + ch * 8) = pack8(o);
      }
    }
  }
}

template <int NCH>
__global__ __launch_bounds__(256, 4) void ln_bwd_dx_kernel(const bf16_t* __restrict__ dy, const bf16_t* __restrict__ x,
                                                        const float* __restrict__ gamma, const float* __restrict__ mean,
                                                        const float* __restrict__ rstd, const bf16_t* __restrict__ dx_add,
                                                        bf16_t* __restrict__ dx, int M, int C) {
  const int lane = threadIdx.x & 63;
  const int wave = (blockIdx.x * blockDim.x + threadIdx.x) >> 6;
  const int nwaves = (gridDim.x * blockDim.x) >> 6;
  const int cpr = C >> 3;
  const float invC = 1.0f / (float)C;
  float gm[NCH][8];
#pragma unroll
  for (int j = 0; j < NCH; ++j) {
    int ch = lane + 64 * j;
#pragma unroll
    for (int e = 0; e < 8; ++e) gm[j][e] = 0.f;
    if (ch < cpr) {
      const float4_t g0 = *(const float4_t*)(gamma + ch * 8), g1 = *(const float4_t*)(gamma + ch * 8 + 4);
#pragma unroll
      for (int e = 0; e < 4; ++e) { gm[j][e] = g0[e]; gm[j][4 + e] = g1[e]; }
    }
  }
  for (int row = wave; row < M; row += nwaves) {
    const float mu = mean[row], rs = rstd[row];
    uint4_t rx[NCH], rd[NCH], ra[NCH];
#pragma unroll
// ... 136 lines not shown
  };
  constexpr bool AHEAD = NCH < 4;
  if (AHEAD) fetch(wave, rx, rd, ra, mu, rs);
  for (int row = wave; row < M; row += nwaves) {
    uint4_t nx[NCH], nd[NCH], na[NCH];
    float nmu = 0.f, nrs = 0.f;
    if (AHEAD) fetch(row + nwaves, nx, nd, na, nmu, nrs);
    else fetch(row, rx, rd, ra, mu, rs);
    float s1 = 0.f, s2 = 0.f;
#pragma unroll
    for (int j = 0; j < NCH; ++j) {
      float fx[8], fd[8];
      unpack8(rx[j], fx);
      unpack8(rd[j], fd);
#pragma unroll
      for (int e = 0; e < 8; ++e) {
        const float xh = (fx[e] - mu) * rs;
        const float d = fd[e] * gm[j][e];
        s1 += d;
        s2 += d * xh;
        sb[j][e] += fd[e];
        sg[j][e] += fd[e] * xh;
      }
    }
    s1 = wave_sum(s1) * invC;
    s2 = wave_sum(s2) * invC;
#pragma unroll
    for (int j = 0; j < NCH; ++j) {
      int ch = lane + 64 * j;
      if (ch < cpr) {
        float fx[8], fd[8], o[8];
        unpack8(rx[j], fx);
        unpack8(rd[j], fd);
        unpack8(ra[j], o);
#pragma unroll
        for (int e = 0; e < 8; ++e) o[e] += rs * (fd[e] * gm[j][e] - s1 - (fx[e] - mu) * rs * s2);
        *(uint4_t*)(dx + (long)row * C + ch * 8) = pack8(o);
      }
    }
    if (AHEAD) {
#pragma unroll
      for (int j = 0; j < NCH; ++j) { rx[j] = nx[j]; rd[j] = nd[j]; ra[j] = na[j]; }
      mu = nmu;
      rs = nrs;
    }
  }
#pragma unroll
  for (int round = 0; round < LNR_WAVES / 2; ++round) {
    if ((wv >> 1) == round) {
      float* gbase = red + ((long)(wv & 1) * 2) * C;
#pragma unroll
      for (int j = 0; j < NCH; ++j) {
        int ch = lane + 64 * j;
        if (ch < cpr) {
          float* g = gbase + ch * 8;
          float4_t g0 = {sg[j][0], sg[j][1], sg[j][2], sg[j][3]}, g1 = {sg[j][4], sg[j][5], sg[j][6], sg[j][7]};
          float4_t b0 = {sb[j][0], sb[j][1], sb[j][2], sb[j][3]}, b1 = {sb[j][4], sb[j][5], sb[j][6], sb[j][7]};
          if (round) { g0 += *(const float4_t*)g; g1 += *(const float4_t*)(g + 4); b0 += *(const float4_t*)(g + C); b1 += *(const float4_t*)(g + C + 4); }
          *(float4_t*)g = g0;
          *(float4_t*)(g + 4) = g1;
          *(float4_t*)(g + C) = b0;
          *(float4_t*)(g + C + 4) = b1;
        }
      }
    }
    __syncthreads();
  }
  float* out = part + (long)blockIdx.x * 2 * C;
  for (int c = threadIdx.x; c < 2 * C; c += LNR_WAVES * 64) out[c] = red[c] + red[2 * C + c];
}
static int ln_rows_blocks(int M) {
  int b = (M + 4 * LNR_WAVES - 1) / (4 * LNR_WAVES);
  return b < 1 ? 1 : (b > LNR_MAX_BLOCKS ? LNR_MAX_BLOCKS : b);
}

__global__ __launch_bounds__(1024) void colpart_reduce_batch_kernel(const NkColpartBatch b) {
  __shared__ float sa[32][33], sb[32][33];
  const int z = blockIdx.y;
  const int C = b.C[z], nrows = b.nrows[z];
  if ((int)blockIdx.x * 32 >= C) return;
  const float* __restrict__ part = b.part[z];
  const int tx = threadIdx.x & 31, ty = threadIdx.x >> 5;
  const int c = blockIdx.x * 32 + tx;
  float a = 0.f, v = 0.f;
  if (c < C) {
#pragma unroll 8
    for (int r = ty; r < nrows; r += 32) {
      a += part[(long)r * 2 * C + c];
      v += part[(long)r * 2 * C + C + c];
    }
  }
  sa[ty][tx] = a;
  sb[ty][tx] = v;
  __syncthreads();
  if (ty == 0 && c < C) {
#pragma unroll
    for (int j = 1; j < 32; ++j) { a += sa[j][tx]; v += sb[j][tx]; }
    float* dgamma = b.dgamma[z];
    float* dbeta = b.dbeta[z];
    dgamma[c] = b.accumulate[z] ? dgamma[c] + a : a;
    dbeta[c] = b.accumulate[z] ? dbeta[c] + v : v;
  }
}

extern "C" int nk_colpart_reduce_batch(const NkColpartBatch* b, void* stream_) {
  NK_CHECK_ARG(b && b->n > 0 && b->n <= NK_COLPART_MAX);
  int maxC = 0;
  for (int z = 0; z < b->n; ++z) {
    NK_CHECK_ARG(b->part[z] && b->dgamma[z] && b->dbeta[z] && b->nrows[z] > 0 && b->C[z] > 0);
    maxC = b->C[z] > maxC ? b->C[z] : maxC;
  }
  hipLaunchKernelGGL(colpart_reduce_batch_kernel, dim3((maxC + 31) / 32, b->n), dim3(1024), 0, (hipStream_t)stream_, *b);
  return nk_check_launch("colpart_reduce_batch_kernel");
}

extern "C" int nk_layernorm_fwd(const void* x, const float* gamma, const float* beta, void* y, float* mean,
                                float* rstd, int M, int C, float eps, void* stream) {
  NK_CHECK_ARG(M > 0 && C > 0 && (C & 7) == 0 && (C >> 3) <= 64 * LN_MAXCH);
  NK_CHECK_ARG(x && gamma && beta && y && mean && rstd);
  int blocks = min((M + 3) / 4, 4096);
  const int nch = ((C >> 3) + 63) / 64;
#define NK_LN_FWD(NCH_) hipLaunchKernelGGL(ln_fwd_kernel<NCH_>, dim3(blocks), dim3(256), 0, (hipStream_t)stream, (const bf16_t*)x, gamma, beta, (bf16_t*)y, mean, rstd, M, C, eps)
  if (nch <= 2) NK_LN_FWD(2); else if (nch == 3) NK_LN_FWD(3); else NK_LN_FWD(4);
#undef NK_LN_FWD
  return nk_check_launch("ln_fwd_kernel");
}

extern "C" long nk_layernorm_ws_floats(int M, int C) {
  const long a = (long)ln_param_split(M), b = LNR_MAX_BLOCKS;
  return (a > b ? a : b) * 2 * C + 64;
}

extern "C" long nk_layernorm_part_rows(int M) { return ln_rows_blocks(M); }

extern "C" int nk_layernorm_bwd_dx(const void* dy, const void* x, const float* gamma, const float* mean, const float* rstd,
                                   const void* dx_add, void* dx, int M, int C, void* stream_) {
  hipStream_t stream = (hipStream_t)stream_;
  NK_CHECK_ARG(M > 0 && C > 0 && (C & 7) == 0 && (C >> 3) <= 64 * LN_MAXCH);
  NK_CHECK_ARG(dy && x && gamma && mean && rstd && dx);
  const int blocks = min((M + 3) / 4, 4096);
  const int nch = ((C >> 3) + 63) / 64;
#define NK_LN_DX(NCH_) hipLaunchKernelGGL(ln_bwd_dx_kernel<NCH_>, dim3(blocks), dim3(256), 0, stream, (const bf16_t*)dy, (const bf16_t*)x, gamma, mean, rstd, (const bf16_t*)dx_add, (bf16_t*)dx, M, C)
  if (nch <= 2) NK_LN_DX(2); else if (nch == 3) NK_LN_DX(3); else NK_LN_DX(4);
#undef NK_LN_DX
  return nk_check_launch("ln_bwd_dx_kernel");
}

extern "C" int nk_layernorm_bwd_params(const void* dy, const void* x, const float* mean, const float* rstd, float* dgamma,
                                       float* dbeta, float* ws, int M, int C, int accumulate, void* stream_) {
  hipStream_t stream = (hipStream_t)stream_;
  NK_CHECK_ARG(M > 0 && C > 0 && (C & 7) == 0);
  NK_CHECK_ARG(dy && x && mean && rstd && dgamma && dbeta && ws);
  const int nsplit = ln_param_split(M);
  hipLaunchKernelGGL(ln_bwd_param_kernel, dim3(nsplit, (C + 127) / 128), dim3(256), 0, stream, (const bf16_t*)dy, (const bf16_t*)x,
                     mean, rstd, ws, M, C);
  if (int e = nk_check_launch("ln_bwd_param_kernel")) return e;
  hipLaunchKernelGGL(colpart_reduce_kernel, dim3((C + 63) / 64), dim3(1024), 0, stream, ws, dgamma, dbeta, nsplit, C, accumulate);
  return nk_check_launch("colpart_reduce_kernel");
}

static int launch_ln_rows(const void* dy, const void* x, const float* gamma, const float* mean, const float* rstd, const void* dx_add,
                          void* dx, float* part, int M, int C, hipStream_t stream) {
  const int blocks = ln_rows_blocks(M);
  const int nch = ((C >> 3) + 63) / 64;
  const int smem = 2 * 2 * C * (int)sizeof(float);
#define NK_LN_ROWS(NCH_)                                                                                                       \
  do {                                                                                                                          \
    nk_optin_lds((const void*)ln_bwd_rows_kernel<NCH_>, 2 * 2 * 2048 * 4);                                                      \
    hipLaunchKernelGGL(ln_bwd_rows_kernel<NCH_>, dim3(blocks), dim3(LNR_WAVES * 64), smem, stream, (const bf16_t*)dy, (const bf16_t*)x, gamma, mean, rstd,   \
                       (const bf16_t*)dx_add, (bf16_t*)dx, part, M, C);                                                        \
  } while (0)
  if (nch <= 2) NK_LN_ROWS(2); else if (nch == 3) NK_LN_ROWS(3); else NK_LN_ROWS(4);
#undef NK_LN_ROWS
  return nk_check_launch("ln_bwd_rows_kernel");
}

extern "C" int nk_layernorm_bwd_rows(const void* dy, const void* x, const float* gamma, const float* mean, const float* rstd,
                                     const void* dx_add, void* dx, float* part, int M, int C, void* stream_) {
  NK_CHECK_ARG(M > 0 && C > 0 && (C & 7) == 0 && (C >> 3) <= 64 * LN_MAXCH);
  NK_CHECK_ARG(dy && x && gamma && mean && rstd && dx && part);
  return launch_ln_rows(dy, x, gamma, mean, rstd, dx_add, dx, part, M, C, (hipStream_t)stream_);
}

extern "C" int nk_layernorm_bwd(const void* dy, const void* x, const float* gamma, const float* mean,
// ... 10 lines not shown
```

neurosis_amd/lib.py:

```python
from __future__ import annotations

import ctypes as C
import os
from pathlib import Path

import torch

CSRC = Path(__file__).resolve().parent / "csrc"
LIB_PATH = CSRC / "libneurosis_hip.so"

vp, i32, i64, f32 = C.c_void_p, C.c_int, C.c_long, C.c_float


class NkConvDesc(C.Structure):
    _fields_ = [(n, i32) for n in ("N", "H", "W", "Cin", "Cout", "KH", "KW", "stride", "pad_t", "pad_l", "Ho", "Wo", "upsample")]


class NkAttnDesc(C.Structure):
    _fields_ = (
        [(n, i32) for n in ("B", "H", "Lq", "Lk", "D")]
        + [(n, i64) for n in ("sq", "sk", "sv", "so", "bq", "bk", "bv", "bo", "sdq", "sdk", "sdv", "sdo", "bdq", "bdk", "bdv", "bdo")]
        + [("scale", f32), ("causal", i32)]
    )


NK_COLPART_MAX = 32


class NkColpartBatch(C.Structure):
    _fields_ = [("part", vp * NK_COLPART_MAX), ("dgamma", vp * NK_COLPART_MAX), ("dbeta", vp * NK_COLPART_MAX), ("nrows", i32 * NK_COLPART_MAX),
                ("C", i32 * NK_COLPART_MAX), ("accumulate", i32 * NK_COLPART_MAX), ("n", i32)]


cdp, adp = C.POINTER(NkConvDesc), C.POINTER(NkAttnDesc)

SIGNATURES: dict[str, list] = {
    "nk_linear_fwd": [vp, vp, vp, vp, vp, i32, i32, i32, i64, i64, i64, i64, f32, vp],
    "nk_linear_dgrad": [vp, vp, vp, vp, i32, i32, i32, i64, i64, i64, i64, vp],
    "nk_linear_dgrad_geglu": [vp, vp, vp, vp, i32, i32, i32, i64, i64, i64, i64, vp],
    "nk_linear_fwd_geglu": [vp, vp, vp, vp, vp, i32, i32, i32, i64, i64, i64, i64, vp],
    "nk_linear_fwd_geglu_s": [vp, vp, vp, vp, vp, i32, i32, i32, i64, i64, i64, i64, vp],
    "nk_linear_dgrad_geglu_s": [vp, vp, vp, vp, i32, i32, i32, i64, i64, i64, i64, vp],
    "nk_linear_wgrad": [vp, vp, vp, i32, i32, i32, i64, i64, i64, i32, vp],
    "nk_linear_fwd_batched": [C.POINTER(vp), C.POINTER(vp), C.POINTER(vp), i32, i32, i32, i32, i64, i64, i64, vp],
    "nk_linear_wgrad_batched": [C.POINTER(vp), C.POINTER(vp), C.POINTER(vp), C.POINTER(vp), i32, i32, i32, i32, i64, i64, i64, i32, vp],
    "nk_linear_wgrad_bias": [vp, vp, vp, vp, i32, i32, i32, i64, i64, i64, i32, vp],
    "nk_conv2d_wgrad_bias": [cdp, vp, vp, vp, vp, i32, vp],
    "nk_conv2d_fwd": [cdp, vp, vp, vp, vp, vp, vp, vp],
    "nk_conv2d_fwd_stats": [cdp, vp, vp, vp, vp, vp, vp, vp, i32, vp],
    "nk_conv_weight_flip": [vp, vp, i32, i32, i32, vp],
    "nk_conv3x3_few_channels_fwd": [vp, vp, vp, vp, i32, i32, i32, i32, i32, vp],
    "nk_conv2d_dgrad": [cdp, vp, vp, vp, vp],
    "nk_conv2d_dgrad_flipped": [cdp, vp, vp, vp, vp],
    "nk_conv2d_wgrad": [cdp, vp, vp, vp, i32, vp],
    "nk_attention_fwd": [adp, vp, vp, vp, vp, vp, vp],
    "nk_attention_bwd": [adp, vp, vp, vp, vp, vp, vp, vp, vp, vp, vp, vp],
    "nk_attention_bwd_causal": [adp, vp, vp, vp, vp, vp, vp, vp, vp, vp, vp],
    "nk_softmax_rows": [vp, i64, i32, vp],
    "nk_softmax_rows_bwd": [vp, vp, i64, i32, f32, vp],
    "nk_groupnorm_fwd": [vp, vp, vp, vp, vp, vp, vp, i32, i32, i32, i32, f32, i32, vp],
    "nk_groupnorm_sums": [vp, vp, vp, i32, i32, i32, i32, vp],
    "nk_groupnorm_sums_from_parts": [vp, vp, vp, i32, i32, i32, vp],
    "nk_groupnorm_apply": [vp, vp, vp, vp, vp, vp, vp, i32, i32, i32, i32, f32, i32, vp],
    "nk_groupnorm_bwd": [vp, vp, vp, vp, vp, vp, vp, vp, vp, vp, vp, i32, i32, i32, i32, i32, i32, vp],
    "nk_layernorm_fwd": [vp, vp, vp, vp, vp, vp, i32, i32, f32, vp],
    "nk_layernorm_bwd": [vp, vp, vp, vp, vp, vp, vp, vp, vp, vp, i32, i32, i32, vp],
    "nk_layernorm_bwd_dx": [vp, vp, vp, vp, vp, vp, vp, i32, i32, vp],
    "nk_layernorm_bwd_rows": [vp, vp, vp, vp, vp, vp, vp, vp, i32, i32, vp],
    "nk_colpart_reduce_batch": [C.POINTER(NkColpartBatch), vp],
    "nk_layernorm_bwd_params": [vp, vp, vp, vp, vp, vp, vp, i32, i32, i32, vp],
    "nk_geglu_fwd": [vp, vp, i64, i32, vp],
    "nk_geglu_bwd": [vp, vp, vp, i64, i32, vp],
    "nk_geglu_fwd_s": [vp, vp, vp, i64, i32, vp],
    "nk_geglu_bwd_s": [vp, vp, vp, i64, i32, vp],
    "nk_silu_fwd": [vp, vp, i64, vp],
    "nk_gelu_fwd": [vp, vp, i64, i32, vp],
    "nk_gelu_bwd": [vp, vp, vp, i64, i32, vp],
    "nk_embedding_bwd": [vp, vp, i64, vp, vp, i32, i32, i32, i32, i32, i32, vp],
    "nk_gather_rows_bwd": [vp, i64, vp, vp, i32, i32, i32, vp],
    "nk_wgrad_few_rows": [vp, i64, vp, i64, vp, i64, i32, i32, i32, i32, vp],
    "nk_leaky_relu_fwd": [vp, vp, i64, f32, vp],
    "nk_leaky_relu_bwd": [vp, vp, vp, i64, f32, vp],
    "nk_maxpool2x2_fwd": [vp, vp, i32, i32, i32, i32, vp],
    "nk_maxpool2x2_bwd": [vp, vp, vp, i32, i32, i32, i32, vp],
    "nk_maxpool_fwd": [vp, vp, i32, i32, i32, i32, i32, i32, vp],
    "nk_maxpool_bwd": [vp, vp, vp, i32, i32, i32, i32, i32, i32, vp],
    "nk_lpips_layer_fwd": [vp, vp, vp, vp, vp, i32, i32, i32, f32, i32, vp],
    "nk_lpips_layer_bwd": [vp, vp, vp, vp, vp, i32, i32, i32, f32, vp],
    "nk_batchnorm_fwd": [vp, vp, vp, vp, vp, vp, vp, vp, vp, i64, i32, f32, f32, f32, vp],
    "nk_batchnorm_bwd": [vp, vp, vp, vp, vp, vp, vp, vp, vp, vp, i64, i32, f32, i32, vp],
    "nk_batchnorm_eval": [vp, vp, vp, vp, vp, vp, vp, i64, i32, f32, f32, vp],
    "nk_silu_bwd": [vp, vp, vp, i64, vp],
    "nk_add": [vp, vp, vp, i64, vp],
    "nk_cat_channels": [vp, vp, vp, i64, i32, i32, vp],
    "nk_split_channels": [vp, vp, vp, i64, i32, i32, vp],
    "nk_upsample2x_bwd": [vp, vp, i32, i32, i32, i32, vp],
    "nk_nchw_to_nhwc": [vp, i32, vp, i32, i32, i32, i32, f32, vp],
    "nk_nhwc_to_nchw": [vp, vp, i32, i32, i32, i32, i32, vp],
    "nk_cast_f32_to_bf16": [vp, vp, i64, vp],
    "nk_cast_bf16_to_f32": [vp, vp, i64, vp],
    "nk_colsum": [vp, vp, vp, i64, i32, i64, i32, vp],
    "nk_colsum_batched": [vp, vp, vp, i64, i32, i64, i32, i32, vp],
    "nk_timestep_embedding": [vp, vp, i32, i32, f32, vp],
    "nk_edm_prepare": [vp, vp, vp, vp, vp, vp, i32, i32, i32, i32, vp],
    "nk_edm_loss": [vp, vp, vp, vp, vp, vp, vp, vp, i32, i32, i32, i32, f32, vp],
    "nk_sample_prepare": [vp, vp, vp, i32, i32, i32, i32, i32, vp],
    "nk_sample_denoise": [vp, vp, vp, vp, f32, vp, i32, i32, i32, i32, i32, vp],
    "nk_sample_euler_step": [vp, vp, vp, vp, vp, vp, f32, vp, vp, i32, i32, i32, i32, i32, vp],
    "nk_adamw_flat": [vp, vp, vp, vp, vp, i64, f32, f32, f32, f32, f32, i32, f32, vp],
    "nk_ema_flat": [vp, vp, i64, f32, vp],
    "nk_debug_raise_health": [vp],
    "nk_debug_stamp": [vp, vp],
    "nk_debug_launch_log": [i32],
    "nk_health_clear": [],
    "nk_health_export": [vp, vp],
    "nk_health_import": [vp, vp],
    "nk_adafactor_init": [vp, vp],
    "nk_adafactor_chunk": [vp, vp],
    "nk_came_chunk": [vp, vp],
    "nk_adamw8bit_step": [vp, vp],
}

SIZE_QUERIES: dict[str, list] = {
    "nk_groupnorm_ws_floats": [i32, i32, i32, i32],
    "nk_groupnorm_sums_ws_floats": [i32, i32, i32],
    "nk_conv2d_stats_tiles": [cdp, i32],
    "nk_conv2d_dgrad_flipped_ok": [cdp],
    "nk_linear_fwd_geglu_ok": [i32, i32, i32],
    "nk_layernorm_ws_floats": [i32, i32],
    "nk_layernorm_part_rows": [i32],
    "nk_colsum_ws_floats": [i64, i32],
    "nk_batchnorm_ws_floats": [i64, i32],
    "nk_lpips_layer_ws_floats": [i32, i32],
    "nk_attention_bwd_ws_floats": [adp],
    "nk_adafactor_tensor_bytes": [],
    "nk_came_tensor_bytes": [],
    "nk_adamw8bit_tensor_bytes": [],
    "nk_gemm_sk_status": [],
    "nk_health_status": [],
    "nk_debug_launch_names": [C.c_char_p, i64],
}

_lib = None


class NkError(RuntimeError):
    pass


def load() -> C.CDLL:
    global _lib
    if _lib is not None:
        return _lib
    path = Path(os.environ.get("NEUROSIS_HIP_LIB", LIB_PATH))
    if not path.exists():
        raise NkError(
            f"{path} not found: the HIP extension is not built. Run `python -c 'import __graft_entry__ as g; g.build()'` "
            "(or `make -C neurosis_amd/csrc`). There is no CPU fallback for the product path."
        )
    lib = C.CDLL(str(path))
    lib.nk_last_error.restype = C.c_char_p
    lib.nk_last_error.argtypes = []
    lib.nk_abi_version.restype = i32
    lib.nk_abi_version.argtypes = []
    for name, argtypes in SIGNATURES.items():
        fn = getattr(lib, name)
        fn.argtypes = argtypes
        fn.restype = i32
    for name, argtypes in SIZE_QUERIES.items():
        fn = getattr(lib, name)
        fn.argtypes = argtypes
        fn.restype = i64
    _lib = lib
    return lib


def launch_log(mode: int) -> None:
    call("nk_debug_launch_log", int(mode))


def launched() -> list[str]:
    buf = C.create_string_buffer(8192)
    n = query("nk_debug_launch_names", buf, len(buf))
    if n < 0:
        raise NkError("nk_debug_launch_names failed")
    return buf.value.decode().split("\n")[:-1]


def query(name: str, *args) -> int:
    return int(getattr(load(), name)(*args))


def call(name: str, *args) -> None:
    lib = load()
    rc = getattr(lib, name)(*args)
    if rc != 0:
        raise NkError(f"{name} failed (rc={rc}): {lib.nk_last_error().decode()}")
```

neurosis_amd/modules/diffusion/model.py:

```python
from __future__ import annotations

import os
import math
from typing import Optional, Sequence

import torch
from torch import Tensor, nn

from ... import ops
from ...graphs import ForwardGraphs, frozen_stamp, graphs_enabled
from ...nn import Conv2d
from ...ops import BF16, Img


def Normalize(in_channels: int, num_groups: int = 32) -> nn.GroupNorm:
    return nn.GroupNorm(num_groups=num_groups, num_channels=in_channels, eps=1e-6, affine=True)


def _gn(x: Img, norm: nn.GroupNorm, silu: bool) -> Img:
    return ops.groupnorm_fwd(x, norm.weight, norm.bias, norm.num_groups, norm.eps, silu)[0]


def _conv_fwdb(conv: Conv2d, x: Img, **kw):
    y, b = conv.fwd(x, **kw)
# ... 113 lines not shown
        hn, b_n = ops.groupnorm_fwd(x, n.weight, n.bias, n.num_groups, n.eps, False)
        (q, b_q), (k, b_k), (v, b_v) = (m.fwd(hn) for m in (self.q, self.k, self.v))
        if self.in_channels <= 160:
            o, b_att = ops.attention_fwd(q.t, k.t, v.t, x.N, 1, self.in_channels)
        elif self.in_channels == 512:
            o, b_att = ops.attention512_fwd(q.t, k.t, v.t, x.N)
        else:
            o, b_att = ops.attention_anydim_fwd(q.t, k.t, v.t, x.N)
        y, b_p = self.proj_out.fwd(Img(o, x.N, x.H, x.W), residual=x.t)

        def bwd(dy: Tensor) -> Tensor:
            dq, dk, dv = b_att(b_p(dy)[0].t)
            dhn = ops.add(ops.add(b_q(dq)[0].t, b_k(dk)[0].t), b_v(dv)[0].t)
            return b_n(dhn, dx_add=dy)

        return y, bwd


MemoryEfficientAttnBlock = AttnBlock


def make_attn(in_channels: int, attn_type: str = "vanilla", attn_kwargs=None) -> nn.Module:
    if attn_type in ("vanilla", "vanilla-xformers"):
        return AttnBlock(in_channels)
    if attn_type == "none":
        return nn.Identity()
    if attn_type == "torch-sdp":
        raise ValueError("attn_type 'torch-sdp' (TorchSDPAttnBlock) scrambles tokens in the reference; use 'vanilla' or 'vanilla-xformers'")
    raise ValueError(f"attn_type {attn_type} unknown or outside the SD/SDXL path")


class Encoder(nn.Module):

    def __init__(self, *, ch: int, out_ch: int, ch_mult: Sequence[int] = (1, 2, 4, 8), num_res_blocks: int, attn_resolutions: Sequence[int],
                 dropout: float = 0.0, resamp_with_conv: bool = True, in_channels: int, resolution: int, z_channels: int, double_z: bool = True,
                 use_linear_attn: bool = False, attn_type: str = "vanilla", embed_dim: int = 256, standalone: bool = False, **kwargs):
        super().__init__()
        self.ch = ch
        self.temb_ch = 0
        self.num_resolutions = len(ch_mult)
        self.num_res_blocks = num_res_blocks
        self.resolution = resolution
        self.in_channels = in_channels
        self.z_channels = z_channels
        self.double_z = double_z
        self.conv_in = Conv2d(in_channels, self.ch, kernel_size=3, stride=1, padding=1)
        curr_res = resolution
        in_ch_mult = (1,) + tuple(ch_mult)
        self.in_ch_mult = in_ch_mult
        self.down = nn.ModuleList()
        block_in = ch
        for i_level in range(self.num_resolutions):
            block = nn.ModuleList()
            attn = nn.ModuleList()
            block_in = ch * in_ch_mult[i_level]
            block_out = ch * ch_mult[i_level]
            for _ in range(self.num_res_blocks):
                block.append(ResnetBlock(in_channels=block_in, out_channels=block_out, temb_channels=self.temb_ch, dropout=dropout))
                block_in = block_out
                if curr_res in attn_resolutions:
                    attn.append(make_attn(block_in, attn_type=attn_type))
            down = nn.Module()
            down.block = block
            down.attn = attn
            if i_level != self.num_resolutions - 1:
                down.downsample = Downsample(block_in, resamp_with_conv)
                curr_res = curr_res // 2
            self.down.append(down)
        self.mid = nn.Module()
        self.mid.block_1 = ResnetBlock(in_channels=block_in, out_channels=block_in, temb_channels=self.temb_ch, dropout=dropout)
        self.mid.attn_1 = make_attn(block_in, attn_type=attn_type)
        self.mid.block_2 = ResnetBlock(in_channels=block_in, out_channels=block_in, temb_channels=self.temb_ch, dropout=dropout)
        self.norm_out = Normalize(block_in)
        self.conv_out = Conv2d(block_in, 2 * z_channels if double_z else z_channels, kernel_size=3, stride=1, padding=1)
        self.max_batch_size = None
        self.standalone = standalone
        if self.standalone:
            qc = (1 + double_z) * z_channels
            self.quant_conv = Conv2d(qc, (1 + double_z) * embed_dim, 1)
        else:
            self.quant_conv = nn.Identity()

    def fwd(self, x: Img) -> Img:
        h = self.conv_in.fwd(x, need_dx=False)[0]
        last_level = self.num_resolutions - 1
        for i_level in range(self.num_resolutions):
            level = self.down[i_level]
            for i_block in range(self.num_res_blocks):
                to_norm = i_block + 1 < self.num_res_blocks or len(level.attn) > 0 or i_level == last_level
                h = level.block[i_block].fwd(h, want_sums=to_norm)
                if len(level.attn) > 0:
                    h = level.attn[i_block].fwd(h)
            if i_level != last_level:
                h = level.downsample.fwd(h)
        h = self.mid.block_1.fwd(h, want_sums=True)
        if not isinstance(self.mid.attn_1, nn.Identity):
            h = self.mid.attn_1.fwd(h)
        h = self.mid.block_2.fwd(h, want_sums=True)
        h = self.conv_out.fwd(_gn(h, self.norm_out, True), need_dx=False)[0]
        if self.standalone:
            h = self.quant_conv.fwd(h, need_dx=False)[0]
        return h

    def fwdb(self, x: Img):
        tape = []

        def run(pair):
            tape.append(pair[1])
            return pair[0]

        h, b_in = self.conv_in.fwd(x, need_dx=False)
        for i_level in range(self.num_resolutions):
            level = self.down[i_level]
            for i_block in range(self.num_res_blocks):
                h = run(level.block[i_block].fwdb(h))
                if len(level.attn) > 0:
                    h = run(level.attn[i_block].fwdb(h))
            if i_level != self.num_resolutions - 1:
                h = run(level.downsample.fwdb(h))
        h = run(self.mid.block_1.fwdb(h))
        if not isinstance(self.mid.attn_1, nn.Identity):
            h = run(self.mid.attn_1.fwdb(h))
        h = run(self.mid.block_2.fwdb(h))
        no = self.norm_out
        hn, b_no = ops.groupnorm_fwd(h, no.weight, no.bias, no.num_groups, no.eps, True)
        h, b_out = self.conv_out.fwd(hn)
        b_quant = None
        if self.standalone:
            h, b_quant = self.quant_conv.fwd(h)

        def bwd(dh: Tensor) -> None:
            if b_quant is not None:
                dh = b_quant(dh)[0].t
            dh = b_no(b_out(dh)[0].t)
            for b in reversed(tape):
                dh = b(dh)
            tape.clear()
            b_in(dh)

        return h, bwd

    @torch.no_grad()
    def forward(self, x: Tensor, regularize: bool = False) -> Tensor:
        N, Cin, H, W = x.shape
        bs = self.max_batch_size or N
        outs = []
        for i in range(0, N, bs):
            xb = x[i:i + bs]
            n = xb.shape[0]
            xb = xb.float() if xb.dtype not in (torch.float32, BF16) else xb
            if xb.is_cuda and graphs_enabled("vae") and not any(p.requires_grad for p in self.parameters()):
                fg = self.__dict__.get("_nk_fgraphs")
                if fg is None:
                    fg = self.__dict__["_nk_fgraphs"] = ForwardGraphs(xb.device)
                outs.append(fg.run(lambda t: self._encode_chunk(t, regularize), [xb.contiguous()], extra_key=(regularize, frozen_stamp(self))))
            else:
                outs.append(self._encode_chunk(xb, regularize))
        return outs[0] if len(outs) == 1 else torch.cat(outs, 0)

    def _encode_chunk(self, xb: Tensor, regularize: bool) -> Tensor:
        n, Cin, H, W = xb.shape
        img = Img(ops.nchw_to_tokens(xb, (Cin + 7) // 8 * 8), n, H, W)
        h = self.fwd(img)
        zc_real = self.conv_out.out_channels if not self.standalone else self.quant_conv.out_channels
        keep = zc_real // 2 if (regularize and self.double_z) else zc_real
        return ops.tokens_to_nchw(h.t, n, keep, h.H, h.W, dtype=torch.float32)

# ... 126 lines not shown
```

neurosis_amd/nn.py:

```python
from __future__ import annotations

import math
from typing import Callable, Iterable, Optional, Sequence

import torch
from torch import Tensor, nn

from . import ops
from .lib import call
from .ops import BF16, Img


class NkFunction(torch.autograd.Function):

    @staticmethod
    def forward(ctx, run: Callable, n_in: int, *args):
        with ops.recording_backward():
            out, bwd = run(*args[:n_in])
        ctx.bwd = bwd
        ctx.n_in = n_in
        ctx.n_args = len(args)
        ctx.in_meta = [(a.dtype, a.shape) if isinstance(a, Tensor) else None for a in args[:n_in]]
        return out

# ... 32 lines not shown
        return ops.cast_bf16(x2.contiguous())
    if x2.dtype == BF16:
        return x2.contiguous()
    raise ValueError(f"unsupported dtype {x2.dtype}")


def grad_to_tokens(g: Tensor, C: int) -> Tensor:
    return Img.from_nchw(g).t if g.dim() == 4 else as_tokens(g)


def _pad8(c: int) -> int:
    return (c + 7) // 8 * 8


class Conv2d(nn.Module):

    def __init__(self, in_channels: int, out_channels: int, kernel_size: int, stride: int = 1, padding: int = 0, bias: bool = True, asym_pad: bool = False):
        super().__init__()
        self.in_channels, self.out_channels = in_channels, out_channels
        self.kernel_size, self.stride, self.padding, self.asym_pad = kernel_size, stride, padding, asym_pad
        self.weight = ops.conv_weight_param(out_channels, in_channels, kernel_size, kernel_size)
        self.bias = nn.Parameter(torch.empty(out_channels)) if bias else None
        self.reset_parameters()
        self._pad_cache = None

    def reset_parameters(self):
        nn.init.kaiming_uniform_(self.weight, a=math.sqrt(5))
        if self.bias is not None:
            fan_in = self.in_channels * self.kernel_size * self.kernel_size
            bound = 1 / math.sqrt(fan_in) if fan_in > 0 else 0
            nn.init.uniform_(self.bias, -bound, bound)

    @property
    def padded(self) -> bool:
        return self.in_channels % 8 != 0 or self.out_channels % 8 != 0

    def _padded_params(self):
        stamp = (ops._param_stamp(self.weight), None if self.bias is None else ops._param_stamp(self.bias), self.weight.requires_grad)
        cache = self._pad_cache
        same = cache is not None and cache[1].device == self.weight.device and cache[0][2] == stamp[2]
        if same and cache[0] == stamp and not ops.capturing():
            return cache[1], cache[2]
        if same:
            wp, bp = cache[1], cache[2]
            with torch.no_grad():
                wv = wp.data.permute(0, 2, 3, 1)
                wv.zero_()
                wv[: self.out_channels, :, :, : self.in_channels].copy_(self.weight.detach().permute(0, 2, 3, 1))
                if bp is not None:
                    bp.data.zero_()
                    bp.data[: self.out_channels].copy_(self.bias.detach())
            wp._nk_shadow_stamp = None
            if bp is not None:
                bp._nk_shadow_stamp = None
            self._pad_cache = (stamp, wp, bp)
            return wp, bp
        ci, co, k = _pad8(self.in_channels), _pad8(self.out_channels), self.kernel_size
        with torch.no_grad():
            w = torch.zeros(co, k, k, ci, device=self.weight.device)
            w[: self.out_channels, :, :, : self.in_channels] = self.weight.detach().permute(0, 2, 3, 1)
            wp = nn.Parameter(w.permute(0, 3, 1, 2), requires_grad=self.weight.requires_grad)
            bp = None
            if self.bias is not None:
                b = torch.zeros(co, device=self.weight.device)
                b[: self.out_channels] = self.bias.detach()
                bp = nn.Parameter(b, requires_grad=self.weight.requires_grad)
        st = ops.state_of(self.weight).derived()
        wp._nk_state = st
        if bp is not None:
            bp._nk_state = st
        self._pad_cache = (stamp, wp, bp)
        return wp, bp

    def fwd(self, x: Img, rowvec: Optional[Tensor] = None, residual: Optional[Tensor] = None, upsample: bool = False, need_dx: bool = True,
            stats_groups: Optional[int] = None):
        if not self.padded:
            return ops.conv2d_fwd(x, self.weight, self.bias, self.stride, self.padding, upsample, rowvec, residual, need_dx, self.asym_pad,
                                  stats_groups=stats_groups)
        wp, bp = self._padded_params()
        wp.grad = None
        if bp is not None:
            bp.grad = None
        out, b = ops.conv2d_fwd(x, wp, bp, self.stride, self.padding, upsample, rowvec, residual, need_dx, self.asym_pad,
                                cin_real=self.in_channels if self.in_channels in (3, 4) else None)

        def bwd(dy: Tensor):
            acc = ops.state_of(self.weight).grad_accumulate
            res = b(dy)
            if not self.weight.requires_grad:
                return res
            ops.join_wgrad_stream(wp)
            with torch.no_grad():
                g = wp.grad[: self.out_channels, : self.in_channels]
                ops.grad_flat(self.weight)
                ops.grad_flat(self.bias) if self.bias is not None else None
                if acc:
                    self.weight.grad.add_(g)
                    if self.bias is not None:
                        self.bias.grad.add_(bp.grad[: self.out_channels])
                else:
                    self.weight.grad.copy_(g)
                    if self.bias is not None:
                        self.bias.grad.copy_(bp.grad[: self.out_channels])
            return res

        return out, bwd

    def forward(self, x: Tensor) -> Tensor:
        def run(x):
            N, _, H, W = x.shape
            if self.in_channels % 8:
                img = Img(ops.nchw_to_tokens(x, _pad8(self.in_channels)), N, H, W)
            else:
                img = Img.from_nchw(x)
            out, bwd = self.fwd(img)

            def bwd2(g):
                gt = grad_to_tokens(g, out.C)
                if out.C != self.out_channels:
                    raise NotImplementedError("backward through a channel-padded conv output is only supported inside UNetModel")
                dx, _ = bwd(gt)
                if self.in_channels % 8:
                    return ops.tokens_to_nchw(dx.t, N, self.in_channels, H, W, dtype=x.dtype)
                return dx.to_nchw()

            y = out.to_nchw()
            if out.C != self.out_channels:
                y = ops.tokens_to_nchw(out.t, N, self.out_channels, out.H, out.W, dtype=BF16)
            return y, bwd2

        return apply_module(run, [x], self)


def linear_module_fwd(lin: nn.Linear, x: Tensor, residual: Optional[Tensor] = None, need_dx: bool = True, x_saved=None):
    return ops.linear_fwd(x, lin.weight, lin.bias, residual, need_dx, x_saved)


class FlatParamStore:

    ALIGN = 64

    def __init__(self, params: Iterable[nn.Parameter]):
        self.params = [p for p in params]
        if not self.params:
            raise ValueError("FlatParamStore: no parameters")
        dev = self.params[0].device
        self.offsets, total = [], 0
        for p in self.params:
            self.offsets.append(total)
            total += (p.numel() + self.ALIGN - 1) // self.ALIGN * self.ALIGN
        self.numel = total
        self.master = torch.zeros(total, dtype=torch.float32, device=dev)
        self.shadow = torch.zeros(total, dtype=BF16, device=dev)
        self.grad = torch.zeros(total, dtype=torch.float32, device=dev)
        self.exp_avg: Optional[Tensor] = None
        self.exp_avg_sq: Optional[Tensor] = None
        self.step_count = 0
        self.epoch = 0
        self.listeners = []
        self.state = ops.EngineState()
        with torch.no_grad():
            for i, (p, off) in enumerate(zip(self.params, self.offsets)):
                n = p.numel()
                p._nk_index = i
                self.master[off:off + n].copy_(ops._phys_flat(p))
                p.data = self._view(self.master, off, p)
# ... 89 lines not shown
```

neurosis_amd/ops.py:

```python
from __future__ import annotations

import ctypes as C
import os
import threading
import weakref
from dataclasses import dataclass
from typing import Callable, Optional

import torch
from torch import Tensor

from . import lib
from .lib import NkAttnDesc, NkConvDesc, call, query

BF16 = torch.bfloat16


class EngineState:

    _live = weakref.WeakSet()

    def __init__(self, wgrad_stream=None):
        self.grad_accumulate = False
        self.assume_zeroed = False
# ... 63 lines not shown
    return getattr(_recording, "depth", 0) > 0


def on_wgrad_stream(fn: Callable[[], None], *reads: Tensor, owner=None) -> None:
    st = state_of(owner)
    side = st.wgrad_stream
    if side is None:
        fn()
        return
    if st.deferred is not None:
        st.deferred.append((fn, reads))
        return
    side.wait_stream(torch.cuda.current_stream())
    with torch.cuda.stream(side):
        fn()
    for t in reads:
        if t is not None:
            t.record_stream(side)


class WgradQueue:

    def __init__(self, owner=None):
        self.items = []
        self.colparts = []
        self.owner = owner

    MAX_ELEMS = 2 << 20

    @classmethod
    def takes(cls, weight: Tensor) -> bool:
        return weight.numel() <= cls.MAX_ELEMS

    def add(self, dy: Tensor, x: Tensor, dw: Tensor, db: Optional[Tensor] = None) -> None:
        self.items.append((dy, x, dw, db))

    def add_colpart(self, part: Tensor, dgamma: Tensor, dbeta: Tensor, nrows: int, Cc: int, accumulate: bool) -> None:
        self.colparts.append((part, dgamma, dbeta, nrows, Cc, accumulate))

    def flush(self) -> None:
        colparts, self.colparts = self.colparts, []
        if colparts:
            on_wgrad_stream(lambda: colpart_reduce(colparts), *[c[0] for c in colparts], owner=self.owner)
        items, self.items = self.items, []
        if not items:
            return
        groups = {}
        for it in items:
            dy, x, dw, _db = it
            key = (dy.shape[0], dy.shape[1], x.shape[1], dy.stride(0), x.stride(0), dw.stride(0))
            groups.setdefault(key, []).append(it)
        mode = wgrad_mode(self.owner)

        def run():
            for (M, N, K, lddy, ldx, lddw), its in groups.items():
                for i in range(0, len(its), 8):
                    chunk = its[i:i + 8]
                    if len(chunk) == 1:
                        gemm_tn_f32(chunk[0][0], chunk[0][1], chunk[0][2], mode, dbias=chunk[0][3])
                        continue
                    n = len(chunk)
                    arr = C.c_void_p * n
                    call("nk_linear_wgrad_batched", arr(*[c[0].data_ptr() for c in chunk]), arr(*[c[1].data_ptr() for c in chunk]),
                         arr(*[c[2].data_ptr() for c in chunk]), arr(*[None if c[3] is None else c[3].data_ptr() for c in chunk]), n, M, N, K,
                         lddy, ldx, lddw, mode, _stream())

        on_wgrad_stream(run, *[t for it in items for t in it[:2]], owner=self.owner)


def colpart_reduce(entries) -> None:
    for i in range(0, len(entries), lib.NK_COLPART_MAX):
        chunk = entries[i:i + lib.NK_COLPART_MAX]
        b = lib.NkColpartBatch()
        for z, (part, dgamma, dbeta, nrows, Cc, acc) in enumerate(chunk):
            b.part[z], b.dgamma[z], b.dbeta[z] = part.data_ptr(), dgamma.data_ptr(), dbeta.data_ptr()
            b.nrows[z], b.C[z], b.accumulate[z] = nrows, Cc, int(acc)
        b.n = len(chunk)
        call("nk_colpart_reduce_batch", C.byref(b), _stream())


_wgrad_queue: Optional[WgradQueue] = None


class batched_wgrads:

    def __init__(self, owner=None):
        self.owner = owner

    def __enter__(self):
        global _wgrad_queue
        self.prev = _wgrad_queue
        _wgrad_queue = WgradQueue(self.owner) if state_of(self.owner).batch_wgrads else None
        return _wgrad_queue

    def __exit__(self, *exc):
        global _wgrad_queue
        q, _wgrad_queue = _wgrad_queue, self.prev
        if exc[0] is None and q is not None:
            q.flush()
        return False


def join_wgrad_stream(owner=None) -> None:
    if owner is not None:
        st = state_of(owner)
        side = st.wgrad_stream
        if side is not None and st.deferred is None:
            torch.cuda.current_stream().wait_stream(side)
        return
    seen = set()
    for st in list(EngineState._live):
        side = st.wgrad_stream
        if side is not None and st.deferred is None and id(side) not in seen:
            seen.add(id(side))
            torch.cuda.current_stream().wait_stream(side)


def _ws(n_floats: int, device) -> Tensor:
    return torch.empty(n_floats, dtype=torch.float32, device=device)


def _p(t: Optional[Tensor]):
    return None if t is None else t.data_ptr()


def _stream():
    return torch.cuda.current_stream().cuda_stream


def _check2d(t: Tensor, name: str):
    if t.dim() != 2 or t.stride(1) != 1 or t.dtype != BF16 or not t.is_cuda:
        raise ValueError(f"{name}: expected a 2-D bf16 CUDA tensor with unit inner stride, got {tuple(t.shape)} {t.dtype} {t.stride()} {t.device}")


@dataclass
class Img:

    t: Tensor
    N: int
    H: int
    W: int
    sums: Optional[Tensor] = None

    @property
    def C(self) -> int:
        return self.t.shape[1]

    @staticmethod
    def from_nchw(x: Tensor) -> "Img":
        N, Cc, H, W = x.shape
        if x.dtype == BF16 and x.permute(0, 2, 3, 1).is_contiguous():
            return Img(x.permute(0, 2, 3, 1).reshape(N * H * W, Cc), N, H, W)
        return Img(nchw_to_tokens(x, Cc), N, H, W)

    def to_nchw(self) -> Tensor:
        return self.t.view(self.N, self.H, self.W, self.C).permute(0, 3, 1, 2)


def _param_stamp(p: Tensor):
    st = getattr(p, "_nk_store", None)
    if st is not None:
        return ("epoch", id(st), st.epoch)
    return ("version", p._version, p.data_ptr())


def shadow(p: Tensor) -> Tensor:
    if getattr(p, "_nk_store", None) is not None:
        return p._nk_shadow
    s = getattr(p, "_nk_shadow", None)
    stamp = _param_stamp(p)
    if s is not None and getattr(p, "_nk_shadow_stamp", None) == stamp:
        return s
    flat = _phys_flat(p)
    n = flat.numel()
    if s is not None and n % 8 == 0 and s.numel() == n and s.device == p.device:
        call("nk_cast_f32_to_bf16", flat.data_ptr(), s.data_ptr(), n, _stream())
        p._nk_shadow_stamp = stamp
        return s
    s = torch.empty(flat.numel(), dtype=BF16, device=p.device)
    if n % 8 == 0:
        call("nk_cast_f32_to_bf16", flat.data_ptr(), s.data_ptr(), n, _stream())
    else:
        pad = torch.zeros((n + 7) // 8 * 8, dtype=torch.float32, device=p.device)
        pad[:n] = flat
        s8 = torch.empty(pad.numel(), dtype=BF16, device=p.device)
        call("nk_cast_f32_to_bf16", pad.data_ptr(), s8.data_ptr(), pad.numel(), _stream())
        s = s8[:n]
    p._nk_shadow = s
    p._nk_shadow_stamp = stamp
    return s


def _phys_flat(p: Tensor) -> Tensor:
    d = p.detach()
    if d.dim() == 4:
        d = d.permute(0, 2, 3, 1)
    if not d.is_contiguous():
        raise ValueError("parameter storage must be dense (conv weights in channels_last memory format)")
    return d.reshape(-1)


def grad_flat(p: Tensor) -> Tensor:
    if p.grad is None:
        g = torch.zeros_like(p, memory_format=torch.preserve_format)
        p.grad = g
    g = p.grad
    if g.dim() == 4:
        g = g.permute(0, 2, 3, 1)
    if not g.is_contiguous():
        raise ValueError("parameter .grad must share the parameter's physical layout")
    return g.reshape(-1)


def w2d(p: Tensor) -> Tensor:
    return shadow(p).view(p.shape[0], -1)


def g2d(p: Tensor) -> Tensor:
    return grad_flat(p).view(p.shape[0], -1)


def conv_weight_param(out_ch: int, in_ch: int, kh: int, kw: int) -> torch.nn.Parameter:
    base = torch.empty(out_ch, kh, kw, in_ch)
    return torch.nn.Parameter(base.permute(0, 3, 1, 2))

# ... 105 lines not shown
    _check2d(dy, "dy")
    M, N = dy.shape
    ws = _ws(query("nk_colsum_ws_floats", M, N), dy.device)
    call("nk_colsum", dy.data_ptr(), out.data_ptr(), ws.data_ptr(), M, N, dy.stride(0), int(accumulate), _stream())


def linear_fwd(x: Tensor, weight: Tensor, bias: Optional[Tensor], residual: Optional[Tensor] = None, need_dx: bool = True, x_saved=None):
    y = gemm_nt(x, w2d(weight), bias, residual)
    return y, _linear_bwd(x if x_saved is None else x_saved, weight, bias, need_dx)


def geglu_save_enabled() -> bool:
    return os.environ.get("NK_GEGLU_SAVE", "1") != "0"


def linear_geglu_fwd(x: Tensor, weight: Tensor, bias: Optional[Tensor], x_saved=None, save_derivative: bool = False):
    _check2d(x, "x")
    M, K = x.shape
    I2 = weight.shape[0]
    I = I2 // 2
    wq = w2d(weight)
    if I2 % 2 == 0 and x.is_contiguous() and query("nk_linear_fwd_geglu_ok", M, I, K):
        u = torch.empty(M, I2, dtype=BF16, device=x.device)
        h = torch.empty(M, I, dtype=BF16, device=x.device)
        call("nk_linear_fwd_geglu_s" if save_derivative else "nk_linear_fwd_geglu", x.data_ptr(), wq.data_ptr(), _p(bias), u.data_ptr(), h.data_ptr(), M, I, K,
             x.stride(0), wq.stride(0), u.stride(0), h.stride(0), _stream())
    else:
        u = gemm_nt(x, wq, bias, None)
        if save_derivative:
            h = torch.empty(M, I, dtype=BF16, device=x.device)
            call("nk_geglu_fwd_s", u.data_ptr(), h.data_ptr(), u.data_ptr(), M, I, _stream())
        else:
            h = geglu_fwd(u)[0]
    return u, h, _linear_bwd(x if x_saved is None else x_saved, weight, bias, True)


def _linear_bwd(x_in, weight: Tensor, bias: Optional[Tensor], need_dx: bool):
    def bwd(dy: Tensor, dx_add: Optional[Tensor] = None, geglu_u: Optional[Tensor] = None, geglu_s: Optional[Tensor] = None):
        entry = "nk_linear_dgrad_geglu"
        if geglu_s is not None:
            if geglu_u is not None:
                raise ValueError("linear bwd: geglu_u and geglu_s are exclusive")
            geglu_u, entry = geglu_s, "nk_linear_dgrad_geglu_s"
        x = x_in() if callable(x_in) else x_in
        queued = _wgrad_queue is not None and _wgrad_queue.takes(weight) and dy.is_contiguous() and x.is_contiguous()
        db = grad_flat(bias) if bias is not None else None
        if queued:
            _wgrad_queue.add(dy, x, g2d(weight), db)
        else:
            on_wgrad_stream(lambda: gemm_tn_f32(dy, x, g2d(weight), wgrad_mode(weight), dbias=db), dy, x, owner=weight)
        if not need_dx:
            return None
        if geglu_u is not None:
            if dx_add is not None:
                raise ValueError("linear bwd: geglu_u and dx_add are exclusive")
            M, N = dy.shape
            K = weight.shape[1]
            _check2d(geglu_u, "geglu_u")
            if geglu_u.shape != (M, 2 * K):
                raise ValueError(f"linear bwd: geglu_u must be [{M}, {2 * K}], got {tuple(geglu_u.shape)}")
            du = torch.empty(M, 2 * K, dtype=BF16, device=dy.device)
            wq = w2d(weight)
            call(entry, dy.data_ptr(), wq.data_ptr(), geglu_u.data_ptr(), du.data_ptr(), M, N, K, dy.stride(0), wq.stride(0),
                 geglu_u.stride(0), du.stride(0), _stream())
            return du
        return gemm_nn(dy, w2d(weight), dx_add)

    return bwd


def _conv_desc(N, H, W, Cin, Cout, KH, KW, stride, pad_t, pad_l, Ho, Wo, upsample) -> NkConvDesc:
    return NkConvDesc(N, H, W, Cin, Cout, KH, KW, stride, pad_t, pad_l, Ho, Wo, int(upsample))


def groupnorm_sums(x: Img, groups: int) -> Tensor:
    if x.sums is not None and x.sums.shape == (x.N, 2 * groups):
        return x.sums
    sums = torch.empty(x.N, 2 * groups, dtype=torch.float32, device=x.t.device)
    ws = _ws(query("nk_groupnorm_ws_floats", x.N, x.H * x.W, x.C, groups), x.t.device)
    call("nk_groupnorm_sums", x.t.data_ptr(), sums.data_ptr(), ws.data_ptr(), x.N, x.H * x.W, x.C, groups, _stream())
    return sums


def conv2d_fwd(x: Img, weight: Tensor, bias: Optional[Tensor], stride: int = 1, padding=1, upsample: bool = False,
               rowvec: Optional[Tensor] = None, residual: Optional[Tensor] = None, need_dx: bool = True,
               asym_pad: bool = False, stats_groups: Optional[int] = None, cin_real: Optional[int] = None):
    Cout, Cin, KH, KW = weight.shape
    if x.C != Cin:
        raise ValueError(f"conv2d: input has {x.C} channels, weight expects {Cin}")
    Hin, Win = (2 * x.H, 2 * x.W) if upsample else (x.H, x.W)
    if asym_pad:
        pad_t = pad_l = 0
        Ho = (Hin + 1 - KH) // stride + 1
        Wo = (Win + 1 - KW) // stride + 1
    else:
        pad_t = pad_l = int(padding)
        Ho = (Hin + 2 * pad_t - KH) // stride + 1
        Wo = (Win + 2 * pad_l - KW) // stride + 1
    d = _conv_desc(x.N, x.H, x.W, Cin, Cout, KH, KW, stride, pad_t, pad_l, Ho, Wo, upsample)
    y = torch.empty(x.N * Ho * Wo, Cout, dtype=BF16, device=x.t.device)
    _check2d(x.t, "x")
    if not x.t.is_contiguous():
        raise ValueError("conv2d: x must be dense channels-last")
    tiles = query("nk_conv2d_stats_tiles", C.byref(d), stats_groups) if stats_groups else 0
    sums_out = None
    if tiles:
        dev = x.t.device
        part = torch.empty(x.N, tiles, 2 * stats_groups, dtype=torch.float32, device=dev)
        call("nk_conv2d_fwd_stats", C.byref(d), x.t.data_ptr(), w2d(weight).data_ptr(), _p(bias), _p(rowvec), _p(residual), y.data_ptr(),
             part.data_ptr(), stats_groups, _stream())
        sums_out = torch.empty(x.N, 2 * stats_groups, dtype=torch.float32, device=dev)
        ws = _ws(query("nk_groupnorm_sums_ws_floats", x.N, tiles, stats_groups), dev)
        call("nk_groupnorm_sums_from_parts", part.data_ptr(), sums_out.data_ptr(), ws.data_ptr(), x.N, tiles, stats_groups, _stream())
    elif (cin_real in (3, 4) and Cin == 8 and KH == 3 and KW == 3 and stride == 1 and pad_t == 1 and not asym_pad and not upsample and rowvec is None
          and residual is None and Cout % 8 == 0):
        call("nk_conv3x3_few_channels_fwd", x.t.data_ptr(), w2d(weight).data_ptr(), _p(bias), y.data_ptr(), x.N, x.H, x.W, Cout, cin_real, _stream())
    else:
        call("nk_conv2d_fwd", C.byref(d), x.t.data_ptr(), w2d(weight).data_ptr(), _p(bias), _p(rowvec), _p(residual), y.data_ptr(), _stream())
    out = Img(y, x.N, Ho, Wo, sums_out)

    def bwd(dy: Tensor):
        _check2d(dy, "dy")
        if not dy.is_contiguous():
            raise ValueError("conv2d bwd: dy must be dense")
        acc = state_of(weight).grad_accumulate

        if weight.requires_grad:
            if bias is not None:
                on_wgrad_stream(lambda: call("nk_conv2d_wgrad_bias", C.byref(d), dy.data_ptr(), x.t.data_ptr(), g2d(weight).data_ptr(), grad_flat(bias).data_ptr(),
                                             wgrad_mode(weight), _stream()), dy, x.t, owner=weight)
            else:
                on_wgrad_stream(lambda: call("nk_conv2d_wgrad", C.byref(d), dy.data_ptr(), x.t.data_ptr(), g2d(weight).data_ptr(), wgrad_mode(weight), _stream()),
                                dy, x.t, owner=weight)
        drow = None
        if rowvec is not None:
            drow32 = torch.empty(x.N, Cout, dtype=torch.float32, device=dy.device)
            ws = _ws(x.N * query("nk_colsum_ws_floats", Ho * Wo, Cout), dy.device)
            call("nk_colsum_batched", dy.data_ptr(), drow32.data_ptr(), ws.data_ptr(), Ho * Wo, Cout, dy.stride(0), x.N, 0, _stream())
            drow = cast_bf16(drow32)
        dx = None
        if need_dx:
            dxt = torch.empty(x.N * Hin * Win, Cin, dtype=BF16, device=dy.device)
            if query("nk_conv2d_dgrad_flipped_ok", C.byref(d)):
                wt = torch.empty(Cin * 9 * Cout, dtype=BF16, device=dy.device)
                call("nk_conv_weight_flip", w2d(weight).data_ptr(), wt.data_ptr(), Cout, Cin, 9, _stream())
                call("nk_conv2d_dgrad_flipped", C.byref(d), dy.data_ptr(), wt.data_ptr(), dxt.data_ptr(), _stream())
            else:
                call("nk_conv2d_dgrad", C.byref(d), dy.data_ptr(), w2d(weight).data_ptr(), dxt.data_ptr(), _stream())
            if upsample:
                dsm = torch.empty(x.N * x.H * x.W, Cin, dtype=BF16, device=dy.device)
                call("nk_upsample2x_bwd", dxt.data_ptr(), dsm.data_ptr(), x.N, x.H, x.W, Cin, _stream())
                dxt = dsm
            dx = Img(dxt, x.N, x.H, x.W)
        return dx, drow

    return out, bwd


def groupnorm_fwd(x: Img, weight: Tensor, bias: Tensor, groups: int, eps: float, silu: bool):
    if not x.t.is_contiguous():
        raise ValueError("groupnorm: x must be dense channels-last")
    N, HW, Cc = x.N, x.H * x.W, x.C
    y = torch.empty_like(x.t)
    mean = torch.empty(N, groups, dtype=torch.float32, device=x.t.device)
    rstd = torch.empty_like(mean)
    nws = query("nk_groupnorm_ws_floats", N, HW, Cc, groups)
    if x.sums is not None and x.sums.shape == (N, 2 * groups):
        call("nk_groupnorm_apply", x.t.data_ptr(), x.sums.data_ptr(), weight.data_ptr(), bias.data_ptr(), y.data_ptr(), mean.data_ptr(),
             rstd.data_ptr(), N, HW, Cc, groups, float(eps), int(silu), _stream())
    else:
        ws = _ws(nws, x.t.device)
        call("nk_groupnorm_fwd", x.t.data_ptr(), weight.data_ptr(), bias.data_ptr(), y.data_ptr(), mean.data_ptr(), rstd.data_ptr(),
             ws.data_ptr(), N, HW, Cc, groups, float(eps), int(silu), _stream())

    def bwd(dy: Tensor, dx_add: Optional[Tensor] = None):
        dx = torch.empty_like(x.t)
        ws2 = _ws(nws, dy.device)
        call("nk_groupnorm_bwd", dy.data_ptr(), x.t.data_ptr(), weight.data_ptr(), bias.data_ptr(), mean.data_ptr(), rstd.data_ptr(),
             _p(dx_add), dx.data_ptr(), grad_flat(weight).data_ptr(), grad_flat(bias).data_ptr(), ws2.data_ptr(), N, HW, Cc, groups,
             int(silu), int(state_of(weight).grad_accumulate), _stream())
        return dx

    return Img(y, x.N, x.H, x.W), bwd


def layernorm_fwd(x: Tensor, weight: Tensor, bias: Tensor, eps: float = 1e-5):
    _check2d(x, "x")
    if not x.is_contiguous():
        raise ValueError("layernorm: x must be dense")
    M, Cc = x.shape
    y = torch.empty_like(x)
    mean = torch.empty(M, dtype=torch.float32, device=x.device)
    rstd = torch.empty_like(mean)
    call("nk_layernorm_fwd", x.data_ptr(), weight.data_ptr(), bias.data_ptr(), y.data_ptr(), mean.data_ptr(), rstd.data_ptr(), M, Cc, float(eps), _stream())

    def bwd(dy: Tensor, dx_add: Optional[Tensor] = None):
        dx = torch.empty_like(x)
        acc = state_of(weight).grad_accumulate
        if os.environ.get("NK_LN_FUSED", "1") != "0":
            rows = query("nk_layernorm_part_rows", M)
            part = torch.empty(rows * 2 * Cc, dtype=torch.float32, device=dy.device)
            call("nk_layernorm_bwd_rows", dy.data_ptr(), x.data_ptr(), weight.data_ptr(), mean.data_ptr(), rstd.data_ptr(), _p(dx_add),
                 dx.data_ptr(), part.data_ptr(), M, Cc, _stream())
            entry = (part, grad_flat(weight), grad_flat(bias), rows, Cc, bool(acc))
            if _wgrad_queue is not None:
                _wgrad_queue.add_colpart(*entry)
            else:
                on_wgrad_stream(lambda: colpart_reduce([entry]), part, owner=weight)
            return dx
        ws = _ws(query("nk_layernorm_ws_floats", M, Cc), dy.device)
        call("nk_layernorm_bwd_dx", dy.data_ptr(), x.data_ptr(), weight.data_ptr(), mean.data_ptr(), rstd.data_ptr(), _p(dx_add),
             dx.data_ptr(), M, Cc, _stream())

        def params():
            call("nk_layernorm_bwd_params", dy.data_ptr(), x.data_ptr(), mean.data_ptr(), rstd.data_ptr(),
                 grad_flat(weight).data_ptr(), grad_flat(bias).data_ptr(), ws.data_ptr(), M, Cc, int(acc), _stream())

        st_ = state_of(weight)
        if st_.norm_params_on_side_stream if st_.norm_params_on_side_stream is not None else st_.deferred is not None:
            on_wgrad_stream(params, dy, x, mean, rstd, ws, owner=weight)
        else:
            params()
        return dx

    return y, bwd


def geglu_fwd(u: Tensor):
    _check2d(u, "u")
    M, I2 = u.shape
    inner = I2 // 2
    y = torch.empty(M, inner, dtype=BF16, device=u.device)
    call("nk_geglu_fwd", u.data_ptr(), y.data_ptr(), M, inner, _stream())

    def bwd(dy: Tensor):
        du = torch.empty_like(u)
        call("nk_geglu_bwd", dy.data_ptr(), u.data_ptr(), du.data_ptr(), M, inner, _stream())
        return du

    return y, bwd


def gelu(x: Tensor, quick: bool = False) -> Tensor:
    y = torch.empty_like(x)
    call("nk_gelu_fwd", x.data_ptr(), y.data_ptr(), x.numel(), int(quick), _stream())
    return y


def gelu_fwd(x: Tensor, quick: bool = False):
    if not x.is_contiguous():
        raise ValueError("gelu_fwd: x must be dense")
    y = gelu(x, quick)

    def bwd(dy: Tensor) -> Tensor:
        if dy.shape != x.shape or dy.dtype != BF16 or not dy.is_contiguous():
            raise ValueError("gelu bwd: dy must be a dense bf16 tensor of x's shape")
        dx = torch.empty_like(x)
        call("nk_gelu_bwd", dy.data_ptr(), x.data_ptr(), dx.data_ptr(), x.numel(), int(quick), _stream())
        return dx

# ... 304 lines not shown
```

Before: 26.68.

## Fold groupnorm partial-sum reductions into consumers and batch split-K zeroing

Conv forward-with-stats now hands per-tile partial sums straight to groupnorm apply, which folds them in-kernel instead of running a separate sums-from-parts reduction. The few-channel 3x3 conv_in kernel gains a stats variant so the first groupnorm can skip its own statistics pass. Groupnorm backward writes per-row channel partials that are reduced later on the wgrad stream through the batched colpart path. Split-K output zeroing becomes a single batched list kernel instead of per-output launches. The aim is fewer launches and reduction passes, at the cost of extra partial buffers and more in-kernel fold work, all gated by an env var that defaults to on.

New measurement: 26.67. About the same (-0.0%).

```diff
diff --git a/include/neurosis_hip.h b/include/neurosis_hip.h
--- a/include/neurosis_hip.h
+++ b/include/neurosis_hip.h
@@ -60,6 +60,9 @@
                         void* y, float* stats_part, int stats_groups, void* stream);
 int nk_conv3x3_few_channels_fwd(const void* x, const void* w, const float* bias, void* y, int N, int H, int W, int Cout, int cin_real,
                                 void* stream);
+long nk_conv3x3_few_channels_stats_rows(int N, int H, int W, int Cout, int stats_groups);
+int nk_conv3x3_few_channels_fwd_stats(const void* x, const void* w, const float* bias, void* y, float* stats_part, int N, int H, int W, int Cout,
+                                      int cin_real, int stats_groups, void* stream);
 int nk_conv_weight_flip(const void* w, void* wt, int Cout, int Cin, int taps, void* stream);
 long nk_conv2d_dgrad_flipped_ok(const NkConvDesc* d);
 int nk_conv2d_dgrad_flipped(const NkConvDesc* d, const void* dy, const void* wt, void* dx, void* stream);
@@ -93,9 +96,16 @@
 int nk_groupnorm_sums_from_parts(const float* part, float* sums, float* ws, int N, int nparts, int G, void* stream);
 int nk_groupnorm_apply(const void* x, const float* sums, const float* gamma, const float* beta, void* y, float* mean, float* rstd,
                        int N, int HW, int C, int G, float eps, int silu, void* stream);
+long nk_groupnorm_parts_rows(int nparts);
+int nk_groupnorm_parts_l1(const float* part, float* out, int N, int nparts, int G, void* stream);
+int nk_groupnorm_apply_parts(const void* x, const float* part, int nparts, float* sums_out, const float* gamma, const float* beta, void* y,
+                             float* mean, float* rstd, int N, int HW, int C, int G, float eps, int silu, void* stream);
 int nk_groupnorm_bwd(const void* dy, const void* x, const float* gamma, const float* beta, const float* mean,
                      const float* rstd, const void* dx_add, void* dx, float* dgamma, float* dbeta, float* ws,
                      int N, int HW, int C, int G, int silu, int accumulate, void* stream);
+long nk_groupnorm_part_rows(int N, int HW);
+int nk_groupnorm_bwd_rows(const void* dy, const void* x, const float* gamma, const float* beta, const float* mean, const float* rstd,
+                          const void* dx_add, void* dx, float* chan_part, float* ws, int N, int HW, int C, int G, int silu, void* stream);
 
 int nk_layernorm_fwd(const void* x, const float* gamma, const float* beta, void* y, float* mean, float* rstd,
                      int M, int C, float eps, void* stream);
@@ -103,6 +113,7 @@
 int nk_layernorm_bwd(const void* dy, const void* x, const float* gamma, const float* mean, const float* rstd,
                      const void* dx_add, void* dx, float* dgamma, float* dbeta, float* ws, int M, int C, int accumulate, void* stream);
 #define NK_COLPART_MAX 32
+#define NK_COLPART_ORDER16 2
 typedef struct NkColpartBatch {
   const float* part[NK_COLPART_MAX];
   float* dgamma[NK_COLPART_MAX];
diff --git a/neurosis_amd/csrc/conv_wgrad_halo.h b/neurosis_amd/csrc/conv_wgrad_halo.h
--- a/neurosis_amd/csrc/conv_wgrad_halo.h
+++ b/neurosis_amd/csrc/conv_wgrad_halo.h
@@ -205,11 +205,7 @@
   const int S = wgrad_halo_splits(p, per);
   const long nblk = (long)((p.M + WH_BCO - 1) / WH_BCO) * (p.gb.C / WH_BCI);
   if (S > 1 && p.accumulate == 0) {
-    const size_t n = (size_t)p.M * p.N;
-    const unsigned blocks = (unsigned)((n / 4 + 255) / 256 > 2048 ? 2048 : (n / 4 + 255) / 256);
-    hipLaunchKernelGGL(nk_zero_f32_kernel, dim3(blocks ? blocks : 1), dim3(256), 0, stream, (float*)p.C, n);
-    if (p.dbias) hipLaunchKernelGGL(nk_zero_f32_kernel, dim3(1), dim3(256), 0, stream, p.dbias, (size_t)p.M);
-    if (hipGetLastError() != hipSuccess) return NK_ERR_LAUNCH;
+    if (int rc = zero_split_outputs(p, stream)) return rc;
   }
   p.accumulate = p.accumulate == 1 ? 1 : 0;
   p.ksplit_len = per;
diff --git a/neurosis_amd/csrc/elementwise.hip b/neurosis_amd/csrc/elementwise.hip
--- a/neurosis_amd/csrc/elementwise.hip
+++ b/neurosis_amd/csrc/elementwise.hip
@@ -441,8 +441,10 @@
   return nk_check_launch("conv_weight_flip_kernel");
 }
 
+template <int CPG>
 __global__ __launch_bounds__(256) void conv3x3_few_channels_kernel(const bf16_t* __restrict__ x, const bf16_t* __restrict__ w, const float* __restrict__ bias,
-                                                                   bf16_t* __restrict__ y, int N, int H, int W, int Cout, int groups_per_wave) {
+                                                                   bf16_t* __restrict__ y, int N, int H, int W, int Cout, int groups_per_wave,
+                                                                   float* __restrict__ stats_part, int G) {
   const int lane = threadIdx.x & 63, wave = threadIdx.x >> 6;
   const int r = lane & 15, g = lane >> 4;
   const int co_base = blockIdx.y * 128;
@@ -493,11 +495,49 @@
   };
 
   const long gstride = (long)gridDim.x * 4;
+  constexpr bool STATS = CPG != 0;
+  constexpr int NSUB = STATS ? 8 / CPG : 1;
+  float st[4][NSUB][2];
+  int cur = -1;
+  auto lane16_sum = [](float v) {
+    v += __builtin_bit_cast(float, __builtin_amdgcn_update_dpp(0, __builtin_bit_cast(int, v), 0xB1, 0xF, 0xF, true));
+    v += __builtin_bit_cast(float, __builtin_amdgcn_update_dpp(0, __builtin_bit_cast(int, v), 0x4E, 0xF, 0xF, true));
+    v += __builtin_bit_cast(float, __builtin_amdgcn_update_dpp(0, __builtin_bit_cast(int, v), 0x141, 0xF, 0xF, true));
+    v += __builtin_bit_cast(float, __builtin_amdgcn_update_dpp(0, __builtin_bit_cast(int, v), 0x140, 0xF, 0xF, true));
+    return v;
+  };
+  auto emit = [&](int img, bool have) {
+    float* row = stats_part + ((long)img * gstride + gw) * 2 * G;
+#pragma unroll
+    for (int h = 0; h < 4; ++h) {
+      const int co = co_base + h * 32 + nloc;
+#pragma unroll
+      for (int j = 0; j < NSUB; ++j) {
+        const float a = have ? lane16_sum(st[h][j][0]) : 0.f, q = have ? lane16_sum(st[h][j][1]) : 0.f;
+        if (r == 0 && co < Cout) {
+          row[2 * ((co + j * CPG) / (STATS ? CPG : 1))] = a;
+          row[2 * ((co + j * CPG) / (STATS ? CPG : 1)) + 1] = q;
+        }
+      }
+    }
+  };
   uint2_t na, nb, nc;
   long grp = gw;
   fetch(grp, na, nb, nc);
   for (int it = 0; it < groups_per_wave; ++it, grp += gstride) {
     if (grp * 16 >= total) break;
+    if constexpr (STATS) {
+      const int img = (int)(grp * 16 / HW);
+      if (img != cur) {
+        if (cur >= 0) emit(cur, true);
+        for (int z = cur + 1; z < img; ++z) emit(z, false);
+        cur = img;
+#pragma unroll
+        for (int h = 0; h < 4; ++h)
+#pragma unroll
+          for (int j = 0; j < NSUB; ++j) { st[h][j][0] = 0.f; st[h][j][1] = 0.f; }
+      }
+    }
     const bf16x8_t x0 = __builtin_bit_cast(bf16x8_t, (uint4_t){na.x, na.y, nb.x, nb.y});
     const bf16x8_t x1 = __builtin_bit_cast(bf16x8_t, (uint4_t){nc.x, nc.y, 0u, 0u});
     if (it + 1 < groups_per_wave) fetch(grp + gstride, na, nb, nc);
@@ -519,23 +559,67 @@
         v[4 + e] = __uint_as_float(sw[1]) + bv[h][4 + e];
       }
       const int co = co_base + h * 32 + nloc;
-      if (pix < total && co < Cout) *(uint4_t*)(y + pix * Cout + co) = pack8(v);
-    }
-  }
+      const uint4_t o = pack8(v);
+      const bool ok = pix < total && co < Cout;
+      if (ok) *(uint4_t*)(y + pix * Cout + co) = o;
+      if constexpr (STATS) {
+        float q[8];
+        unpack8(o, q);
+#pragma unroll
+        for (int j = 0; j < NSUB; ++j) {
+          float a = 0.f, b = 0.f;
+#pragma unroll
+          for (int e = j * CPG; e < (j + 1) * CPG; ++e) { a += q[e]; b += q[e] * q[e]; }
+          st[h][j][0] += ok ? a : 0.f;
+          st[h][j][1] += ok ? b : 0.f;
+        }
+      }
+    }
+  }
+  if constexpr (STATS) {
+    if (cur >= 0) emit(cur, true);
+    for (int z = cur + 1; z < N; ++z) emit(z, false);
+  }
+}
+static long few_channels_blocks(int N, int H, int W, int* per_wave) {
+  const long groups = ((long)N * H * W + 15) / 16;
+  long blocks = (groups + 4 * 32 - 1) / (4 * 32);
+  if (blocks > 2048) blocks = 2048;
+  *per_wave = (int)((groups + blocks * 4 - 1) / (blocks * 4));
+  return blocks;
 }
 extern "C" int nk_conv3x3_few_channels_fwd(const void* x, const void* w, const float* bias, void* y, int N, int H, int W, int Cout, int cin_real,
                                            void* stream) {
   NK_CHECK_ARG(x && w && y && N > 0 && H > 0 && W > 0 && Cout > 0 && (Cout & 7) == 0);
   NK_CHECK_ARG(cin_real == 3 || cin_real == 4);
   NK_CHECK_ARG((long)N * H * W < (1l << 31));
-  const long groups = ((long)N * H * W + 15) / 16;
-  long blocks = (groups + 4 * 32 - 1) / (4 * 32);
-  if (blocks > 2048) blocks = 2048;
-  const int per_wave = (int)((groups + blocks * 4 - 1) / (blocks * 4));
+  int per_wave;
+  const long blocks = few_channels_blocks(N, H, W, &per_wave);
   dim3 grid((unsigned)blocks, (unsigned)((Cout + 127) / 128));
-  hipLaunchKernelGGL(conv3x3_few_channels_kernel, grid, dim3(256), 0, (hipStream_t)stream, (const bf16_t*)x, (const bf16_t*)w, bias, (bf16_t*)y, N, H, W, Cout,
-                     per_wave);
+  hipLaunchKernelGGL(conv3x3_few_channels_kernel<0>, grid, dim3(256), 0, (hipStream_t)stream, (const bf16_t*)x, (const bf16_t*)w, bias, (bf16_t*)y, N, H, W,
+                     Cout, per_wave, (float*)nullptr, 1);
   return nk_check_launch("conv3x3_few_channels_kernel");
+}
+extern "C" long nk_conv3x3_few_channels_stats_rows(int N, int H, int W, int Cout, int G) {
+  if (N <= 0 || H <= 0 || W <= 0 || Cout <= 0 || G <= 0 || G > 32 || Cout % G || (Cout & 7) || ((long)H * W & 15) || (long)N * H * W >= (1l << 31)) return 0;
+  const int cpg = Cout / G;
+  if (cpg != 2 && cpg != 4 && cpg != 8) return 0;
+  int per_wave;
+  return few_channels_blocks(N, H, W, &per_wave) * 4;
+}
+extern "C" int nk_conv3x3_few_channels_fwd_stats(const void* x, const void* w, const float* bias, void* y, float* part, int N, int H, int W, int Cout,
+                                                 int cin_real, int G, void* stream) {
+  NK_CHECK_ARG(x && w && y && part && N > 0 && H > 0 && W > 0 && Cout > 0 && (Cout & 7) == 0);
+  NK_CHECK_ARG(cin_real == 3 || cin_real == 4);
+  NK_CHECK_ARG(nk_conv3x3_few_channels_stats_rows(N, H, W, Cout, G) > 0);
+  int per_wave;
+  const long blocks = few_channels_blocks(N, H, W, &per_wave);
+  dim3 grid((unsigned)blocks, (unsigned)((Cout + 127) / 128));
+#define NK_FEW_STATS(CPG_) hipLaunchKernelGGL(conv3x3_few_channels_kernel<CPG_>, grid, dim3(256), 0, (hipStream_t)stream, (const bf16_t*)x, (const bf16_t*)w, \
+                                              bias, (bf16_t*)y, N, H, W, Cout, per_wave, part, G)
+  switch (Cout / G) { case 2: NK_FEW_STATS(2); break; case 4: NK_FEW_STATS(4); break; default: NK_FEW_STATS(8); }
+#undef NK_FEW_STATS
+  return nk_check_launch("conv3x3_few_channels_kernel<stats>");
 }
 
 extern "C" int nk_nchw_to_nhwc(const void* src, int src_is_f32, void* dst, int N, int C, int HW, int Cpad, float scale,
diff --git a/neurosis_amd/csrc/gemm.hip b/neurosis_amd/csrc/gemm.hip
--- a/neurosis_amd/csrc/gemm.hip
+++ b/neurosis_amd/csrc/gemm.hip
@@ -1421,6 +1421,7 @@
 
 static bool use_xl(const NkGemmParams& p, int amode, int bmode, int out_f32, int splitk);
 __global__ void nk_zero_f32_kernel(float* __restrict__ dst, size_t n);
+static int zero_split_outputs(const NkGemmParams& p, hipStream_t stream);
 #include "gemm_g2.h"
 #include "gemm_w160.h"
 #include "conv_halo.h"
@@ -1600,11 +1601,36 @@
   p.ksplit_len = per * BK;
 }
 
+struct NkZeroList {
+  float* c[NK_MAX_BATCH];
+  float* dbias[NK_MAX_BATCH];
+};
+__global__ __launch_bounds__(256) void nk_zero_f32_list_kernel(const NkZeroList l, size_t n, unsigned m) {
+  const size_t n4 = n / 4, stride = (size_t)gridDim.x * 256;
+  float* dst = l.c[blockIdx.y];
+  float4_t* d4 = (float4_t*)dst;
+  for (size_t i = (size_t)blockIdx.x * 256 + threadIdx.x; i < n4; i += stride) d4[i] = (float4_t){0.f, 0.f, 0.f, 0.f};
+  if (blockIdx.x == 0 && threadIdx.x < (n & 3)) dst[n4 * 4 + threadIdx.x] = 0.f;
+  if (float* db = l.dbias[blockIdx.y])
+    for (size_t i = (size_t)blockIdx.x * 256 + threadIdx.x; i < m; i += stride) db[i] = 0.f;
+}
+
 static int zero_split_outputs(const NkGemmParams& p, hipStream_t stream) {
-  for (int z = 0; z < (p.nbatch ? p.nbatch : 1); ++z) {
-    const size_t n = (size_t)p.M * p.N;
+  const size_t n = (size_t)p.M * p.N;
+  const unsigned blocks = (unsigned)((n / 4 + 255) / 256 > 2048 ? 2048 : (n / 4 + 255) / 256);
+  const int nb = p.nbatch ? p.nbatch : 1;
+  if (nk_fold_reduce(NK_FOLD_ZERO)) {
+    NK_CHECK_ARG(nb <= NK_MAX_BATCH);
+    NkZeroList l = {};
+    for (int z = 0; z < nb; ++z) {
+      l.c[z] = (float*)(p.nbatch ? p.Cb[z] : p.C);
+      l.dbias[z] = p.nbatch ? p.dbias_b[z] : p.dbias;
+    }
+    hipLaunchKernelGGL(nk_zero_f32_list_kernel, dim3(blocks ? blocks : 1, nb), dim3(256), 0, stream, l, n, (unsigned)p.M);
+    return hipGetLastError() != hipSuccess ? NK_ERR_LAUNCH : NK_OK;
+  }
+  for (int z = 0; z < nb; ++z) {
     float* dst = (float*)(p.nbatch ? p.Cb[z] : p.C);
-    const unsigned blocks = (unsigned)((n / 4 + 255) / 256 > 2048 ? 2048 : (n / 4 + 255) / 256);
     hipLaunchKernelGGL(nk_zero_f32_kernel, dim3(blocks ? blocks : 1), dim3(256), 0, stream, dst, n);
     float* db = p.nbatch ? p.dbias_b[z] : p.dbias;
     if (db) hipLaunchKernelGGL(nk_zero_f32_kernel, dim3(1), dim3(256), 0, stream, db, (size_t)p.M);
diff --git a/neurosis_amd/csrc/nk_common.h b/neurosis_amd/csrc/nk_common.h
--- a/neurosis_amd/csrc/nk_common.h
+++ b/neurosis_amd/csrc/nk_common.h
@@ -1,6 +1,7 @@
 #pragma once
 #include <hip/hip_runtime.h>
 #include <stdint.h>
+#include <stdlib.h>
 
 typedef unsigned short bf16_t;
 typedef __attribute__((ext_vector_type(8))) short short8_t;
@@ -27,6 +28,11 @@
 void nk_set_error(const char* file, int line, const char* what);
 int nk_check_launch(const char* what);
 void nk_optin_lds(const void* kernel, int bytes);
+enum { NK_FOLD_GN = 1, NK_FOLD_ZERO = 2 };
+static inline bool nk_fold_reduce(int which) {
+  const char* e = getenv("NK_FOLD_REDUCE");
+  return !e || (atoi(e) & which) != 0;
+}
 unsigned* nk_health_word(void);
 int nk_health_poll(void);
 void nk_health_snapshot(hipStream_t stream);
diff --git a/neurosis_amd/csrc/norm.hip b/neurosis_amd/csrc/norm.hip
--- a/neurosis_amd/csrc/norm.hip
+++ b/neurosis_amd/csrc/norm.hip
@@ -76,22 +76,53 @@
   }
 }
 
+#define GN_FOLD_MAX 128
+__device__ __forceinline__ void gn_fold_partials(const float* __restrict__ part_n, int nparts, int G2, float (*sm)[128], float* out) {
+  const int tx = threadIdx.x & 127, h = threadIdx.x >> 7;
+  if (tx < G2) {
+    float a[4] = {0.f, 0.f, 0.f, 0.f};
+    for (int p0 = h; p0 < nparts; p0 += 8) {
+#pragma unroll
+      for (int k = 0; k < 4; ++k)
+        if (p0 + 2 * k < nparts) a[k] += part_n[(long)(p0 + 2 * k) * G2 + tx];
+    }
+#pragma unroll
+    for (int k = 0; k < 4; ++k) sm[h + 2 * k][tx] = a[k];
+  }
+  __syncthreads();
+  if ((int)threadIdx.x < G2) {
+    float v = sm[0][threadIdx.x];
+#pragma unroll
+    for (int j = 1; j < 8; ++j) v += sm[j][threadIdx.x];
+    out[threadIdx.x] = v;
+  }
+  __syncthreads();
+}
+
 __global__ __launch_bounds__(GN_THREADS) void gn_apply_kernel(const bf16_t* __restrict__ x, const float* __restrict__ stats,
                                                               const float* __restrict__ gamma, const float* __restrict__ beta,
                                                               bf16_t* __restrict__ y, float* __restrict__ mean_out,
                                                               float* __restrict__ rstd_out, int HW, int C, int G,
-                                                              float eps, int silu, int rows_per) {
+                                                              float eps, int silu, int rows_per,
+                                                              const float* __restrict__ part, int nparts, float* __restrict__ sums_out) {
   extern __shared__ __attribute__((aligned(16))) char smem_raw[];
+  __shared__ float fold_sm[8][128], fold_out[128];
   float* sc = (float*)smem_raw;
   float* sh = sc + C;
   const int n = blockIdx.y;
   const int tid = threadIdx.x;
   const int cpg = C / G;
   const float inv_cnt = 1.0f / ((float)HW * (float)cpg);
+  const float* st = stats + (long)n * 2 * G;
+  if (part) {
+    gn_fold_partials(part + (long)n * nparts * 2 * G, nparts, 2 * G, fold_sm, fold_out);
+    st = fold_out;
+    if (sums_out && blockIdx.x == 0 && tid < 2 * G) sums_out[(long)n * 2 * G + tid] = fold_out[tid];
+  }
   for (int c = tid; c < C; c += GN_THREADS) {
     int g = c / cpg;
-    float m = stats[(long)n * 2 * G + 2 * g] * inv_cnt;
-    float var = fmaxf(stats[(long)n * 2 * G + 2 * g + 1] * inv_cnt - m * m, 0.f);
+    float m = st[2 * g] * inv_cnt;
+    float var = fmaxf(st[2 * g + 1] * inv_cnt - m * m, 0.f);
     float rs = rsqrtf(var + eps);
     float a = rs * gamma[c];
     sc[c] = a;
@@ -242,20 +273,26 @@
                                                                   const float* __restrict__ mean, const float* __restrict__ rstd,
                                                                   const float* __restrict__ gsum, const bf16_t* __restrict__ dx_add,
                                                                   bf16_t* __restrict__ dx, int HW, int C, int G, int silu,
-                                                                  int rows_per) {
+                                                                  int rows_per, const float* __restrict__ part, int nparts) {
   extern __shared__ __attribute__((aligned(16))) char smem_raw[];
   float* p_a = (float*)smem_raw;
   float* p_b = p_a + C;
   float* p_c = p_b + C;
   float* p_d = p_c + C;
+  __shared__ float fold_sm[8][128], fold_out[128];
   const int n = blockIdx.y;
   const int tid = threadIdx.x;
   const int cpg = C / G;
   const float inv_cnt = 1.0f / ((float)HW * (float)cpg);
+  const float* gs = gsum + (long)n * 2 * G;
+  if (part) {
+    gn_fold_partials(part + (long)n * nparts * 2 * G, nparts, 2 * G, fold_sm, fold_out);
+    gs = fold_out;
+  }
   for (int c = tid; c < C; c += GN_THREADS) {
     const int g = c / cpg;
     const float mu = mean[n * G + g], rs = rstd[n * G + g];
-    const float s1 = gsum[(long)n * 2 * G + 2 * g] * inv_cnt, s2 = gsum[(long)n * 2 * G + 2 * g + 1] * inv_cnt;
+    const float s1 = gs[2 * g] * inv_cnt, s2 = gs[2 * g + 1] * inv_cnt;
     const float a = rs * gamma[c];
     p_a[c] = a;
     p_b[c] = beta[c] - mu * a;
@@ -343,10 +380,14 @@
   hipLaunchKernelGGL(gn_stats_kernel, dim3(nsplit, N, nz), dim3(GN_THREADS), 0, stream, (const bf16_t*)x, part, HW, C,
                      G, rows_per);
   if (int e = nk_check_launch("gn_stats_kernel")) return e;
-  hipLaunchKernelGGL(gn_reduce_partials_kernel, dim3(N), dim3(1024), 0, stream, part, stats, nsplit * nz, 2 * G);
-  if (int e = nk_check_launch("gn_reduce_partials_kernel")) return e;
+  const bool fold = nk_fold_reduce(NK_FOLD_GN) && nsplit * nz <= GN_FOLD_MAX;
+  if (!fold) {
+    hipLaunchKernelGGL(gn_reduce_partials_kernel, dim3(N), dim3(1024), 0, stream, part, stats, nsplit * nz, 2 * G);
+    if (int e = nk_check_launch("gn_reduce_partials_kernel")) return e;
+  }
   hipLaunchKernelGGL(gn_apply_kernel, dim3(nsplit, N), dim3(GN_THREADS), 2 * C * sizeof(float), stream,
-                     (const bf16_t*)x, stats, gamma, beta, (bf16_t*)y, mean, rstd, HW, C, G, eps, silu, rows_per);
+                     (const bf16_t*)x, stats, gamma, beta, (bf16_t*)y, mean, rstd, HW, C, G, eps, silu, rows_per,
+                     fold ? part : (const float*)nullptr, nsplit * nz, (float*)nullptr);
   return nk_check_launch("gn_apply_kernel");
 }
 
@@ -379,6 +420,14 @@
   }
   hipLaunchKernelGGL(gn_reduce_partials_kernel, dim3(N), dim3(1024), 0, stream, part, sums, nparts, 2 * G);
   return nk_check_launch("gn_reduce_partials_kernel");
+}
+
+extern "C" long nk_groupnorm_parts_rows(int nparts) { return nparts > GN_FOLD_MAX ? 64 : nparts; }
+extern "C" int nk_groupnorm_parts_l1(const float* part, float* out, int N, int nparts, int G, void* stream_) {
+  NK_CHECK_ARG(part && out && N > 0 && nparts > GN_FOLD_MAX && G > 0 && G <= 32);
+  const int nchunks = 64;
+  hipLaunchKernelGGL(gn_reduce_partials_l1_kernel, dim3(nchunks, N), dim3(256), 0, (hipStream_t)stream_, part, out, nparts, 2 * G, nchunks);
+  return nk_check_launch("gn_reduce_partials_l1_kernel");
 }
 
 extern "C" int nk_groupnorm_sums(const void* x, float* sums, float* ws, int N, int HW, int C, int G, void* stream_) {
@@ -404,7 +453,20 @@
   int nsplit;
   int rows_per = gn_rows_per(N, HW, &nsplit);
   hipLaunchKernelGGL(gn_apply_kernel, dim3(nsplit, N), dim3(GN_THREADS), 2 * C * sizeof(float), stream, (const bf16_t*)x, sums, gamma, beta,
-                     (bf16_t*)y, mean, rstd, HW, C, G, eps, silu, rows_per);
+                     (bf16_t*)y, mean, rstd, HW, C, G, eps, silu, rows_per, (const float*)nullptr, 0, (float*)nullptr);
+  return nk_check_launch("gn_apply_kernel");
+}
+
+extern "C" int nk_groupnorm_apply_parts(const void* x, const float* part, int nparts, float* sums_out, const float* gamma, const float* beta,
+                                        void* y, float* mean, float* rstd, int N, int HW, int C, int G, float eps, int silu, void* stream_) {
+  hipStream_t stream = (hipStream_t)stream_;
+  NK_CHECK_ARG(N > 0 && HW > 0 && C > 0 && G > 0 && G <= 64);
+  NK_CHECK_ARG((C & 7) == 0 && C % G == 0 && C <= GN_MAXC);
+  NK_CHECK_ARG(x && part && nparts > 0 && nparts <= GN_FOLD_MAX && gamma && beta && y && mean && rstd);
+  int nsplit;
+  int rows_per = gn_rows_per(N, HW, &nsplit);
+  hipLaunchKernelGGL(gn_apply_kernel, dim3(nsplit, N), dim3(GN_THREADS), 2 * C * sizeof(float), stream, (const bf16_t*)x, part, gamma, beta,
+                     (bf16_t*)y, mean, rstd, HW, C, G, eps, silu, rows_per, part, nparts, sums_out);
   return nk_check_launch("gn_apply_kernel");
 }
 
@@ -424,13 +486,47 @@
   hipLaunchKernelGGL(gn_bwd_stats_kernel, dim3(nsplit, N, nz), dim3(GN_THREADS), 2 * C * sizeof(float), stream,
                      (const bf16_t*)dy, (const bf16_t*)x, gamma, beta, mean, rstd, part, chan, HW, C, G, silu, rows_per);
   if (int e = nk_check_launch("gn_bwd_stats_kernel")) return e;
-  hipLaunchKernelGGL(gn_reduce_partials_kernel, dim3(N), dim3(1024), 0, stream, part, gsum, nsplit * nz, 2 * G);
-  if (int e = nk_check_launch("gn_reduce_partials_kernel")) return e;
+  const bool fold = nk_fold_reduce(NK_FOLD_GN) && nsplit * nz <= GN_FOLD_MAX;
+  if (!fold) {
+    hipLaunchKernelGGL(gn_reduce_partials_kernel, dim3(N), dim3(1024), 0, stream, part, gsum, nsplit * nz, 2 * G);
+    if (int e = nk_check_launch("gn_reduce_partials_kernel")) return e;
+  }
   hipLaunchKernelGGL(colpart_reduce_kernel, dim3((C + 63) / 64), dim3(1024), 0, stream, chan, dgamma, dbeta, N * nsplit, C, accumulate);
   if (int e = nk_check_launch("colpart_reduce_kernel")) return e;
   hipLaunchKernelGGL(gn_bwd_apply_kernel, dim3(nsplit, N), dim3(GN_THREADS), 4 * C * sizeof(float), stream,
                      (const bf16_t*)dy, (const bf16_t*)x, gamma, beta, mean, rstd, gsum, (const bf16_t*)dx_add,
-                     (bf16_t*)dx, HW, C, G, silu, rows_per);
+                     (bf16_t*)dx, HW, C, G, silu, rows_per, fold ? part : (const float*)nullptr, nsplit * nz);
+  return nk_check_launch("gn_bwd_apply_kernel");
+}
+
+extern "C" long nk_groupnorm_part_rows(int N, int HW) {
+  int nsplit;
+  gn_rows_per(N, HW, &nsplit);
+  return (long)N * nsplit;
+}
+extern "C" int nk_groupnorm_bwd_rows(const void* dy, const void* x, const float* gamma, const float* beta, const float* mean, const float* rstd,
+                                     const void* dx_add, void* dx, float* chan_part, float* ws, int N, int HW, int C, int G, int silu,
+                                     void* stream_) {
+  hipStream_t stream = (hipStream_t)stream_;
+  NK_CHECK_ARG(N > 0 && HW > 0 && C > 0 && G > 0 && G <= 64);
+  NK_CHECK_ARG((C & 7) == 0 && C % G == 0 && C <= GN_MAXC);
+  NK_CHECK_ARG(dy && x && gamma && beta && mean && rstd && dx && chan_part && ws);
+  int nsplit;
+  int rows_per = gn_rows_per(N, HW, &nsplit);
+  const int nz = gn_nz(C);
+  float* part = ws;
+  float* gsum = part + (long)N * nsplit * nz * 2 * G;
+  hipLaunchKernelGGL(gn_bwd_stats_kernel, dim3(nsplit, N, nz), dim3(GN_THREADS), 2 * C * sizeof(float), stream,
+                     (const bf16_t*)dy, (const bf16_t*)x, gamma, beta, mean, rstd, part, chan_part, HW, C, G, silu, rows_per);
+  if (int e = nk_check_launch("gn_bwd_stats_kernel")) return e;
+  const bool fold = nsplit * nz <= GN_FOLD_MAX;
+  if (!fold) {
+    hipLaunchKernelGGL(gn_reduce_partials_kernel, dim3(N), dim3(1024), 0, stream, part, gsum, nsplit * nz, 2 * G);
+    if (int e = nk_check_launch("gn_reduce_partials_kernel")) return e;
+  }
+  hipLaunchKernelGGL(gn_bwd_apply_kernel, dim3(nsplit, N), dim3(GN_THREADS), 4 * C * sizeof(float), stream,
+                     (const bf16_t*)dy, (const bf16_t*)x, gamma, beta, mean, rstd, gsum, (const bf16_t*)dx_add,
+                     (bf16_t*)dx, HW, C, G, silu, rows_per, fold ? part : (const float*)nullptr, nsplit * nz);
   return nk_check_launch("gn_bwd_apply_kernel");
 }
 
@@ -733,10 +829,11 @@
   const float* __restrict__ part = b.part[z];
   const int tx = threadIdx.x & 31, ty = threadIdx.x >> 5;
   const int c = blockIdx.x * 32 + tx;
+  const int ng = (b.accumulate[z] & NK_COLPART_ORDER16) ? 16 : 32;
   float a = 0.f, v = 0.f;
-  if (c < C) {
+  if (c < C && ty < ng) {
 #pragma unroll 8
-    for (int r = ty; r < nrows; r += 32) {
+    for (int r = ty; r < nrows; r += ng) {
       a += part[(long)r * 2 * C + c];
       v += part[(long)r * 2 * C + C + c];
     }
@@ -745,12 +842,11 @@
   sb[ty][tx] = v;
   __syncthreads();
   if (ty == 0 && c < C) {
-#pragma unroll
-    for (int j = 1; j < 32; ++j) { a += sa[j][tx]; v += sb[j][tx]; }
+    for (int j = 1; j < ng; ++j) { a += sa[j][tx]; v += sb[j][tx]; }
     float* dgamma = b.dgamma[z];
     float* dbeta = b.dbeta[z];
-    dgamma[c] = b.accumulate[z] ? dgamma[c] + a : a;
-    dbeta[c] = b.accumulate[z] ? dbeta[c] + v : v;
+    dgamma[c] = (b.accumulate[z] & 1) ? dgamma[c] + a : a;
+    dbeta[c] = (b.accumulate[z] & 1) ? dbeta[c] + v : v;
   }
 }
 
diff --git a/neurosis_amd/lib.py b/neurosis_amd/lib.py
--- a/neurosis_amd/lib.py
+++ b/neurosis_amd/lib.py
@@ -25,6 +25,7 @@
 
 
 NK_COLPART_MAX = 32
+NK_COLPART_ORDER16 = 2
 
 
 class NkColpartBatch(C.Structure):
@@ -50,6 +51,7 @@
     "nk_conv2d_fwd_stats": [cdp, vp, vp, vp, vp, vp, vp, vp, i32, vp],
     "nk_conv_weight_flip": [vp, vp, i32, i32, i32, vp],
     "nk_conv3x3_few_channels_fwd": [vp, vp, vp, vp, i32, i32, i32, i32, i32, vp],
+    "nk_conv3x3_few_channels_fwd_stats": [vp, vp, vp, vp, vp, i32, i32, i32, i32, i32, i32, vp],
     "nk_conv2d_dgrad": [cdp, vp, vp, vp, vp],
     "nk_conv2d_dgrad_flipped": [cdp, vp, vp, vp, vp],
     "nk_conv2d_wgrad": [cdp, vp, vp, vp, i32, vp],
@@ -63,6 +65,9 @@
     "nk_groupnorm_sums_from_parts": [vp, vp, vp, i32, i32, i32, vp],
     "nk_groupnorm_apply": [vp, vp, vp, vp, vp, vp, vp, i32, i32, i32, i32, f32, i32, vp],
     "nk_groupnorm_bwd": [vp, vp, vp, vp, vp, vp, vp, vp, vp, vp, vp, i32, i32, i32, i32, i32, i32, vp],
+    "nk_groupnorm_parts_l1": [vp, vp, i32, i32, i32, vp],
+    "nk_groupnorm_apply_parts": [vp, vp, i32, vp, vp, vp, vp, vp, vp, i32, i32, i32, i32, f32, i32, vp],
+    "nk_groupnorm_bwd_rows": [vp, vp, vp, vp, vp, vp, vp, vp, vp, vp, i32, i32, i32, i32, i32, vp],
     "nk_layernorm_fwd": [vp, vp, vp, vp, vp, vp, i32, i32, f32, vp],
     "nk_layernorm_bwd": [vp, vp, vp, vp, vp, vp, vp, vp, vp, vp, i32, i32, i32, vp],
     "nk_layernorm_bwd_dx": [vp, vp, vp, vp, vp, vp, vp, i32, i32, vp],
@@ -124,7 +129,10 @@
 SIZE_QUERIES: dict[str, list] = {
     "nk_groupnorm_ws_floats": [i32, i32, i32, i32],
     "nk_groupnorm_sums_ws_floats": [i32, i32, i32],
+    "nk_groupnorm_parts_rows": [i32],
+    "nk_groupnorm_part_rows": [i32, i32],
     "nk_conv2d_stats_tiles": [cdp, i32],
+    "nk_conv3x3_few_channels_stats_rows": [i32, i32, i32, i32, i32],
     "nk_conv2d_dgrad_flipped_ok": [cdp],
     "nk_linear_fwd_geglu_ok": [i32, i32, i32],
     "nk_layernorm_ws_floats": [i32, i32],
diff --git a/neurosis_amd/modules/diffusion/model.py b/neurosis_amd/modules/diffusion/model.py
--- a/neurosis_amd/modules/diffusion/model.py
+++ b/neurosis_amd/modules/diffusion/model.py
@@ -219,7 +219,7 @@
             self.quant_conv = nn.Identity()
 
     def fwd(self, x: Img) -> Img:
-        h = self.conv_in.fwd(x, need_dx=False)[0]
+        h = self.conv_in.fwd(x, need_dx=False, stats_groups=self.down[0].block[0].norm1.num_groups)[0]
         last_level = self.num_resolutions - 1
         for i_level in range(self.num_resolutions):
             level = self.down[i_level]
diff --git a/neurosis_amd/nn.py b/neurosis_amd/nn.py
--- a/neurosis_amd/nn.py
+++ b/neurosis_amd/nn.py
@@ -138,6 +138,7 @@
         if bp is not None:
             bp.grad = None
         out, b = ops.conv2d_fwd(x, wp, bp, self.stride, self.padding, upsample, rowvec, residual, need_dx, self.asym_pad,
+                                stats_groups=stats_groups if self.out_channels % 8 == 0 else None,
                                 cin_real=self.in_channels if self.in_channels in (3, 4) else None)
 
         def bwd(dy: Tensor):
diff --git a/neurosis_amd/ops.py b/neurosis_amd/ops.py
--- a/neurosis_amd/ops.py
+++ b/neurosis_amd/ops.py
@@ -169,6 +169,16 @@
 _wgrad_queue: Optional[WgradQueue] = None
 
 
+def fold_reduce(which: int = 1) -> bool:
+    e = os.environ.get("NK_FOLD_REDUCE")
+    if e is None:
+        return True
+    try:
+        return bool(int(e) & which)
+    except ValueError:
+        return False
+
+
 class batched_wgrads:
 
     def __init__(self, owner=None):
@@ -227,7 +237,16 @@
     N: int
     H: int
     W: int
-    sums: Optional[Tensor] = None
+    _sums: Optional[Tensor] = None
+    parts: Optional[Tensor] = None
+
+    @property
+    def sums(self) -> Optional[Tensor]:
+        if self._sums is None and self.parts is not None:
+            n, rows, g2 = self.parts.shape
+            self._sums = torch.empty(n, g2, dtype=torch.float32, device=self.parts.device)
+            call("nk_groupnorm_sums_from_parts", self.parts.data_ptr(), self._sums.data_ptr(), None, n, rows, g2 // 2, _stream())
+        return self._sums
 
     @property
     def C(self) -> int:
@@ -499,6 +518,21 @@
     return sums
 
 
+def _sums_of_parts(part: Tensor, N: int, tiles: int, groups: int):
+    dev = part.device
+    if fold_reduce():
+        rows = query("nk_groupnorm_parts_rows", tiles)
+        if rows != tiles:
+            l1 = torch.empty(N, rows, 2 * groups, dtype=torch.float32, device=dev)
+            call("nk_groupnorm_parts_l1", part.data_ptr(), l1.data_ptr(), N, tiles, groups, _stream())
+            part = l1
+        return None, part
+    sums = torch.empty(N, 2 * groups, dtype=torch.float32, device=dev)
+    ws = _ws(query("nk_groupnorm_sums_ws_floats", N, tiles, groups), dev)
+    call("nk_groupnorm_sums_from_parts", part.data_ptr(), sums.data_ptr(), ws.data_ptr(), N, tiles, groups, _stream())
+    return sums, None
+
+
 def conv2d_fwd(x: Img, weight: Tensor, bias: Optional[Tensor], stride: int = 1, padding=1, upsample: bool = False,
                rowvec: Optional[Tensor] = None, residual: Optional[Tensor] = None, need_dx: bool = True,
                asym_pad: bool = False, stats_groups: Optional[int] = None, cin_real: Optional[int] = None):
@@ -520,21 +554,26 @@
     if not x.t.is_contiguous():
         raise ValueError("conv2d: x must be dense channels-last")
     tiles = query("nk_conv2d_stats_tiles", C.byref(d), stats_groups) if stats_groups else 0
-    sums_out = None
+    sums_out = parts_out = None
     if tiles:
         dev = x.t.device
         part = torch.empty(x.N, tiles, 2 * stats_groups, dtype=torch.float32, device=dev)
         call("nk_conv2d_fwd_stats", C.byref(d), x.t.data_ptr(), w2d(weight).data_ptr(), _p(bias), _p(rowvec), _p(residual), y.data_ptr(),
              part.data_ptr(), stats_groups, _stream())
-        sums_out = torch.empty(x.N, 2 * stats_groups, dtype=torch.float32, device=dev)
-        ws = _ws(query("nk_groupnorm_sums_ws_floats", x.N, tiles, stats_groups), dev)
-        call("nk_groupnorm_sums_from_parts", part.data_ptr(), sums_out.data_ptr(), ws.data_ptr(), x.N, tiles, stats_groups, _stream())
+        sums_out, parts_out = _sums_of_parts(part, x.N, tiles, stats_groups)
     elif (cin_real in (3, 4) and Cin == 8 and KH == 3 and KW == 3 and stride == 1 and pad_t == 1 and not asym_pad and not upsample and rowvec is None
           and residual is None and Cout % 8 == 0):
-        call("nk_conv3x3_few_channels_fwd", x.t.data_ptr(), w2d(weight).data_ptr(), _p(bias), y.data_ptr(), x.N, x.H, x.W, Cout, cin_real, _stream())
+        rows = query("nk_conv3x3_few_channels_stats_rows", x.N, x.H, x.W, Cout, stats_groups) if stats_groups and fold_reduce(4) else 0
+        if rows:
+            part = torch.empty(x.N, rows, 2 * stats_groups, dtype=torch.float32, device=x.t.device)
+            call("nk_conv3x3_few_channels_fwd_stats", x.t.data_ptr(), w2d(weight).data_ptr(), _p(bias), y.data_ptr(), part.data_ptr(), x.N, x.H, x.W, Cout,
+                 cin_real, stats_groups, _stream())
+            sums_out, parts_out = _sums_of_parts(part, x.N, rows, stats_groups)
+        else:
+            call("nk_conv3x3_few_channels_fwd", x.t.data_ptr(), w2d(weight).data_ptr(), _p(bias), y.data_ptr(), x.N, x.H, x.W, Cout, cin_real, _stream())
     else:
         call("nk_conv2d_fwd", C.byref(d), x.t.data_ptr(), w2d(weight).data_ptr(), _p(bias), _p(rowvec), _p(residual), y.data_ptr(), _stream())
-    out = Img(y, x.N, Ho, Wo, sums_out)
+    out = Img(y, x.N, Ho, Wo, sums_out, parts_out)
 
     def bwd(dy: Tensor):
         _check2d(dy, "dy")
@@ -582,7 +621,10 @@
     mean = torch.empty(N, groups, dtype=torch.float32, device=x.t.device)
     rstd = torch.empty_like(mean)
     nws = query("nk_groupnorm_ws_floats", N, HW, Cc, groups)
-    if x.sums is not None and x.sums.shape == (N, 2 * groups):
+    if x._sums is None and x.parts is not None and x.parts.shape[0] == N and x.parts.shape[2] == 2 * groups and fold_reduce():
+        call("nk_groupnorm_apply_parts", x.t.data_ptr(), x.parts.data_ptr(), x.parts.shape[1], None, weight.data_ptr(), bias.data_ptr(), y.data_ptr(),
+             mean.data_ptr(), rstd.data_ptr(), N, HW, Cc, groups, float(eps), int(silu), _stream())
+    elif x.sums is not None and x.sums.shape == (N, 2 * groups):
         call("nk_groupnorm_apply", x.t.data_ptr(), x.sums.data_ptr(), weight.data_ptr(), bias.data_ptr(), y.data_ptr(), mean.data_ptr(),
              rstd.data_ptr(), N, HW, Cc, groups, float(eps), int(silu), _stream())
     else:
@@ -593,6 +635,17 @@
     def bwd(dy: Tensor, dx_add: Optional[Tensor] = None):
         dx = torch.empty_like(x.t)
         ws2 = _ws(nws, dy.device)
+        if fold_reduce():
+            rows = query("nk_groupnorm_part_rows", N, HW)
+            part = torch.empty(rows * 2 * Cc, dtype=torch.float32, device=dy.device)
+            call("nk_groupnorm_bwd_rows", dy.data_ptr(), x.t.data_ptr(), weight.data_ptr(), bias.data_ptr(), mean.data_ptr(), rstd.data_ptr(),
+                 _p(dx_add), dx.data_ptr(), part.data_ptr(), ws2.data_ptr(), N, HW, Cc, groups, int(silu), _stream())
+            entry = (part, grad_flat(weight), grad_flat(bias), rows, Cc, int(state_of(weight).grad_accumulate) | lib.NK_COLPART_ORDER16)
+            if _wgrad_queue is not None:
+                _wgrad_queue.add_colpart(*entry)
+            else:
+                on_wgrad_stream(lambda: colpart_reduce([entry]), part, owner=weight)
+            return dx
         call("nk_groupnorm_bwd", dy.data_ptr(), x.t.data_ptr(), weight.data_ptr(), bias.data_ptr(), mean.data_ptr(), rstd.data_ptr(),
              _p(dx_add), dx.data_ptr(), grad_flat(weight).data_ptr(), grad_flat(bias).data_ptr(), ws2.data_ptr(), N, HW, Cc, groups,
              int(silu), int(state_of(weight).grad_accumulate), _stream())
```
